# dojo-sim/ContactImplicitMPC.jl

Hardware: AMD Instinct MI355X
Metric: MPC steps/s (quadruped, H=40, fp64) (higher is better)
Workload: dtype f64

## Files before the change

contactimplicitmpc/jl_amd/csrc/cimpc_host.cpp:

```cpp
#include <hip/hip_runtime.h>

#include <algorithm>
#include <chrono>
#include <cmath>
#include <cstdio>
#include <cstdlib>
#include <cstring>
#include <string>
#include <vector>

#include "cimpc_internal.h"
#include "lin_table.h"
#include "newton_state.h"
#include "schedule_plan.h"

using namespace cimpc;

namespace {

thread_local std::string g_create_error;

enum ProfClass { PC_IP = 0, PC_KKT = 1, PC_RESID = 2, PC_OTHER = 3, PC_ASYNC = 4, PC_COUNT = 5 };

struct ProfRec {
// ... 385 lines not shown
    o->r_tol = 3.0e-4;
    o->beta_init = 1.0e-5;
    o->max_time = 0.0;
    o->kappa = 2.0e-4;
    o->max_iter = 5;
    o->kkt_backend = CIMPC_KKT_CONDENSED;
}

const char* cimpc_last_error(cimpc_handle h) { return h ? h->err.c_str() : g_create_error.c_str(); }

int cimpc_create(const cimpc_dims* dims, const cimpc_ip_opts* ip, const cimpc_newton_opts* nt,
                 int device, cimpc_handle* out) {
    if (!dims || !out) return fail(nullptr, CIMPC_ERR_INVALID, "null argument");
    *out = nullptr;
    const cimpc_dims& d = *dims;
    if (d.nq <= 0 || d.nu < 0 || d.nw < 0 || d.nc <= 0 || d.nb < 0 || d.H <= 0 || d.H_ref <= 0 ||
        d.B <= 0 || (d.mode != 0 && d.mode != 1))
        return fail(nullptr, CIMPC_ERR_INVALID, "invalid dimensions");
    int ndev = 0;
    if (hipGetDeviceCount(&ndev) != hipSuccess || ndev <= 0)
        return fail(nullptr, CIMPC_ERR_NO_DEVICE,
                    "no HIP device visible: this library has no CPU fallback");
    if (device < 0 || device >= ndev) return fail(nullptr, CIMPC_ERR_NO_DEVICE, "device index out of range");
    hipDeviceProp_t prop;
    if (hipGetDeviceProperties(&prop, device) != hipSuccess)
        return fail(nullptr, CIMPC_ERR_NO_DEVICE, "hipGetDeviceProperties failed");
    if (std::strncmp(prop.gcnArchName, "gfx950", 6) != 0)
        return fail(nullptr, CIMPC_ERR_NO_DEVICE,
                    std::string("device is ") + prop.gcnArchName + ", kernels are built for gfx950 only");
    if (hipSetDevice(device) != hipSuccess) return fail(nullptr, CIMPC_ERR_NO_DEVICE, "hipSetDevice failed");

    cimpc_ctx* h = new cimpc_ctx();
    h->dm = d;
    if (ip) h->ip = *ip; else cimpc_default_ip_opts(&h->ip);
    if (nt) h->nt = *nt; else cimpc_default_newton_opts(&h->nt);
    h->device = device;
    if (h->ip.max_time > 0.0 && h->ip.max_time < 1000.0) {
        if (h->ip.max_iter >= 128) { delete h; return fail(nullptr, CIMPC_ERR_INVALID, "ip max_time needs max_iter < 128 (the parked state packs both into one word)"); }
        int khz = 0;
        if (hipDeviceGetAttribute(&khz, hipDeviceAttributeWallClockRate, device) != hipSuccess || khz <= 0) {
            delete h;
            return fail(nullptr, CIMPC_ERR_HIP, "ip max_time: the device does not report hipDeviceAttributeWallClockRate");
        }
        h->ip_budget_ticks = std::max<long long>(1, (long long)std::llround(h->ip.max_time * 1.0e3 * (double)khz));
    }
    h->kn.read_environment();
    if (ip_kernel_info(&h->dm, &h->ki) != CIMPC_OK) {
        delete h;
        return fail(nullptr, CIMPC_ERR_INVALID,
                    "model dimensions outside the runtime-dimension kernel (nx, ny <= 64) and without a compiled set (built: pushbot, hopper_2D, hopper_3D, walledcartpole, particle, particle_2D, "
                    "quadruped, flamingo, centroidal_quadruped are built)");
    }
    h->nx = d.nq;
    h->ny = 2 * d.nc + d.nb;
    h->nz = d.nq + 4 * d.nc + 2 * d.nb;
    h->nth = 2 * d.nq + d.nu + d.nw + 2;
    h->nths = 2 * d.nq + d.nu;
    h->nd = d.mode ? d.nq + d.nc + d.nb : d.nq;
    h->nr = d.mode ? d.nq + d.nu + d.nc + d.nb : d.nq + d.nu;
    h->N = d.H * (h->nr + h->nd);
    if (hipStreamCreateWithFlags(&h->stream, hipStreamNonBlocking) != hipSuccess) {
        delete h;
        return fail(nullptr, CIMPC_ERR_HIP, "hipStreamCreate failed");
    }
    h->own_stream = true;
    h->knot_set.assign(d.H_ref, 0);
    h->h_tab.assign(h->ki.tab_size, 0.0);

    const size_t B = d.B, H = d.H;
    int rc = CIMPC_OK;
    {
        const size_t K = d.H_ref;
        const size_t evals = 1 + 7 * (size_t)std::max(1, h->nt.max_iter);
        h->a_cap = B * evals * ((H + K - 1) / K + 1);
        h->a_rq_cap = B * (2 + 3 * (size_t)std::max(1, h->nt.max_iter));
        h->a_kq_cap = B * (2 + 3 * (size_t)std::max(1, h->nt.max_iter));
        const size_t bytes = (K * h->a_cap + h->a_rq_cap + h->a_kq_cap) * sizeof(int);
        h->sched = plan_schedule(h->kn.sched, ScheduleFacts{d.B, d.H, d.H_ref, h->ki.G, newton_async_available(&d) && K <= 256 && bytes <= ((size_t)1 << 30)});
    }
    auto A = [&](auto** p, size_t n) { if (rc == CIMPC_OK) rc = dev_alloc(h, p, n); };
    A(&h->d_tab, (size_t)d.H_ref * h->ki.tab_size);
    {
        const size_t K = d.H_ref;
        const size_t cap = B * CS * ((H + K - 1) / K + 1);
        h->Q.K = (int)K; h->Q.cap = (int)cap; h->Q.par = 0;
        A(&h->Q.items, 2 * K * cap);
        h->ctl_ints = 3 * K * QPAD + 2 * 8 * CPAD;
        A(&h->Q.count, h->ctl_ints);
        if (rc == CIMPC_OK) { h->Q.head = h->Q.count + 2 * K * QPAD; h->d_ring = h->Q.count + 3 * K * QPAD; }
        A(&h->Q.done_count, B * CS);
        A(&h->d_window, B * (H + 2));
        h->Q.window = h->d_window;
    }
    A(&h->d_alt, B * d.nc);
    A(&h->d_zout, B * CS * H * h->nz);
    A(&h->d_Q, H * d.nq * d.nq);
    A(&h->d_R, H * d.nu * d.nu);
    A(&h->d_Qinv, H * d.nq * d.nq);
    A(&h->d_Rinv, H * d.nu * d.nu);
    A(&h->d_Cg, H * d.nc * d.nc);
    A(&h->d_Cb, H * d.nb * d.nb);
    A(&h->d_V, H * d.nq * d.nq);
    A(&h->d_qt, H * d.nq);
    A(&h->d_vt, H * d.nq);
    A(&h->d_q0, 2 * B * d.nq);
    if (rc == CIMPC_OK) h->d_q1 = h->d_q0 + B * d.nq;
    A(&h->d_result, 8 + B * (d.nu + 2));
    if (rc == CIMPC_OK && (hipHostMalloc((void**)&h->h_qin, (2 * B + 1) * d.nq * sizeof(double), hipHostMallocDefault) != hipSuccess ||
                           hipHostMalloc((void**)&h->h_result, (8 + B * (d.nu + 2)) * sizeof(double), hipHostMallocDefault) != hipSuccess))
        rc = CIMPC_ERR_HIP;
    A(&h->d_rhs, B * h->N);
    NewtonDev& S = h->S;
    S.dm = d;
    S.b0 = 0;
    S.nb_launch = d.B;
    S.nd = h->nd; S.nr = h->nr; S.nth = h->nth; S.nths = h->nths; S.N = h->N;
    const size_t BS = B * CS;
    for (TrajDev* T : {&S.traj, &S.cand, &S.ref}) {
        const size_t n = (T == &S.cand) ? BS : B;
        A(&T->q, n * (H + 2) * d.nq); A(&T->u, n * H * d.nu); A(&T->w, n * H * d.nw);
        A(&T->g, n * H * d.nc); A(&T->b, n * H * d.nb); A(&T->th, n * H * h->nth);
    }
    A(&S.nu, B * H * h->nd); A(&S.nu_cand, BS * H * h->nd); A(&S.d, BS * H * h->nd);
    A(&S.dz, BS * H * h->nths * h->nd); A(&S.dz_good, B * H * h->nths * h->nd); A(&h->d_good_src, B * H);
    S.dtn_ld = h->ki.generic ? 0 : h->ki.dtn_ld;
    if (S.dtn_ld > 0) A(&S.dtn, BS * H * (size_t)S.dtn_ld);
    A(&S.ip_status, BS * H); A(&S.ip_iters, BS * H); A(&S.pflag, BS * H); A(&S.cur_slot, B);
    A(&h->d_pstate, BS * H * (2 * (size_t)h->nx + 4 * (size_t)h->ny + 4));
    A(&S.res, B * h->N); A(&S.res_cand, BS * h->N); A(&S.delta, B * h->N);
    A(&S.r_norm, B); A(&S.r_cand, BS); A(&S.alpha, B); A(&S.beta, B);
    A(&S.ls_iter, B); A(&S.newton_l, B); A(&S.stage, B); A(&S.need_sweep, BS);
    A(&S.kkt_list, 2 * B);
    A(&S.slot_list, 2 * BS);
    A(&S.counters, 8 * CPAD);
    A(&S.stats, std::max<size_t>(B * 4, 64));
    A(&S.ro_sweeps, B); A(&S.ro_ip_iters, B); A(&S.ro_ip_fail, B); A(&S.nlog, B * NLOG * 4);
    A(&S.kkt_ws, B * H * (3 * (size_t)h->nd * h->nd + h->nd));
    A(&S.kkt_tw_xch, B * (3 * (size_t)h->nd * h->nd + 4 * h->nd));
    A(&S.kkt_tw_flags, B * 32);
    if (rc == CIMPC_OK && hipHostMalloc((void**)&h->h_counters, 8 * CPAD * sizeof(int)) != hipSuccess)
        rc = fail(h, CIMPC_ERR_HIP, "hipHostMalloc failed");
    if (rc != CIMPC_OK) {
        g_create_error = h->err;
        cimpc_destroy(h);
        return rc;
    }
    S.Q = h->d_Q; S.R = h->d_R; S.Qinv = h->d_Qinv; S.Rinv = h->d_Rinv; S.Cg = h->d_Cg; S.Cb = h->d_Cb;
    if (hipMemset(h->d_good_src, 0xFF, B * H * sizeof(int)) != hipSuccess || hipStreamSynchronize(nullptr) != hipSuccess) {
        g_create_error = "hipMemset failed"; cimpc_destroy(h); return CIMPC_ERR_HIP;
    }
    S.band_form = h->kn.banded_form;
    S.r_tol = h->nt.r_tol; S.beta_init = h->nt.beta_init; S.kappa = h->nt.kappa; S.max_iter = h->nt.max_iter;
    h->kp = h->kn.kkt;
    h->kp.kkt_overlap = h->sched.kkt_overlap;
    set_kkt_backend(h);
    S.spec_all = h->sched.spec_all; S.spec_first = h->sched.spec_first; S.spec_mid = h->sched.spec_mid;
    S.kkt_tw_nb = h->kn.kkt_tw_nb;
    S.kkt_tw_epoch = 0;
    S.kkt_tw_spins = h->kn.kkt_tw_spins > 0 ? h->kn.kkt_tw_spins : (1 << 21);
    {
        int* dv = nullptr;
        if (hipHostMalloc((void**)&h->h_twfail, 4 * sizeof(int), hipHostMallocMapped) != hipSuccess ||
            hipHostGetDevicePointer((void**)&dv, h->h_twfail, 0) != hipSuccess) {
            g_create_error = "mapped counter allocation failed"; cimpc_destroy(h); return CIMPC_ERR_HIP;
        }
        h->h_twfail[0] = 0;
        S.kkt_tw_fail = dv;
    }
    if (hipHostMalloc((void**)&h->h_ring, 32 * sizeof(int), hipHostMallocMapped) != hipSuccess ||
        hipHostGetDevicePointer((void**)&h->h_ring_dev, h->h_ring, 0) != hipSuccess) {
        g_create_error = "ring allocation failed"; cimpc_destroy(h); return CIMPC_ERR_HIP;
    }
    if (h->sched.async_on) {
        const size_t K = d.H_ref;
        if (dev_alloc(h, &h->a_items, K * h->a_cap) != CIMPC_OK || dev_alloc(h, &h->a_jobs, h->a_rq_cap + h->a_kq_cap) != CIMPC_OK ||
            dev_alloc(h, &h->a_ctrl, 2 * K * QPAD + 64 + 33 * 16) != CIMPC_OK || dev_alloc(h, &h->a_evals, B) != CIMPC_OK) {
            g_create_error = h->err; cimpc_destroy(h); return CIMPC_ERR_HIP;
        }
        if (h->kn.async_debug && dev_alloc(h, &h->a_dbg, 16) != CIMPC_OK) { g_create_error = h->err; cimpc_destroy(h); return CIMPC_ERR_HIP; }
        h->async_dirty = true;
    }
    {
        RoundStreams& r = h->rs;
        if (hipStreamCreateWithFlags(&r.st, hipStreamNonBlocking) != hipSuccess ||
            hipStreamCreateWithFlags(&r.st_kkt, hipStreamNonBlocking) != hipSuccess ||
            hipEventCreateWithFlags(&r.ev_join, hipEventDisableTiming) != hipSuccess ||
            hipEventCreateWithFlags(&r.ev_start, hipEventDisableTiming) != hipSuccess) {
            g_create_error = "stream creation failed"; cimpc_destroy(h); return CIMPC_ERR_HIP;
        }
    }
    *out = h;
    return CIMPC_OK;
}

int cimpc_destroy(cimpc_handle h) {
    if (!h) return CIMPC_ERR_INVALID;
    (void)hipSetDevice(h->device);
    if (h->stream) (void)hipStreamSynchronize(h->stream);
    for (auto& r : h->prof_recs) { (void)hipEventDestroy(r.a); (void)hipEventDestroy(r.b); }
    for (auto e : h->ev_pool) (void)hipEventDestroy(e);
    for (void* p : h->allocs) (void)hipFree(p);
    if (h->h_counters) (void)hipHostFree(h->h_counters);
    if (h->h_ring) (void)hipHostFree(h->h_ring);
    if (h->h_qin) (void)hipHostFree(h->h_qin);
    if (h->h_result) (void)hipHostFree(h->h_result);
    if (h->h_stage) (void)hipHostFree(h->h_stage);
    if (h->h_twfail) (void)hipHostFree(h->h_twfail);
    {
        RoundStreams& r = h->rs;
        if (r.st) { (void)hipStreamSynchronize(r.st); (void)hipStreamDestroy(r.st); }
        if (r.st_kkt) { (void)hipStreamSynchronize(r.st_kkt); (void)hipStreamDestroy(r.st_kkt); }
        if (r.ev_join) (void)hipEventDestroy(r.ev_join);
        if (r.ev_start) (void)hipEventDestroy(r.ev_start);
    }
    if (h->own_stream && h->stream) (void)hipStreamDestroy(h->stream);
    delete h;
    return CIMPC_OK;
}

int cimpc_set_stream(cimpc_handle h, void* hip_stream) {
    if (!h) return CIMPC_ERR_INVALID;
    (void)hipStreamSynchronize(h->stream);
    h->advance_pending = false;
// ... 187 lines not shown
static int rekey_out(cimpc_ctx* h) {
    if (h->dz_producer == 0 || !h->window_set) return CIMPC_OK;
    if (!h->d_dz_knot && dev_alloc(h, &h->d_dz_knot, (size_t)h->dm.B * h->dm.H_ref * h->nths * h->nd) != CIMPC_OK) return CIMPC_ERR_HIP;
    int rc = launch_dz_rekey(h->S, h->d_dz_knot, h->d_window, h->dz_producer == 1 ? 0 : 1, 0, h->stream);
    return rc == CIMPC_OK ? CIMPC_OK : fail(h, rc, "sensitivity archive launch failed");
}
static int rekey_in(cimpc_ctx* h) {
    if (h->dz_producer == 0 || !h->d_dz_knot) return CIMPC_OK;
    for (int which = 0; which < 2; ++which) {
        int rc = launch_dz_rekey(h->S, h->d_dz_knot, h->d_window, which, 1, h->stream);
        if (rc != CIMPC_OK) return fail(h, rc, "sensitivity restore launch failed");
    }
    return CIMPC_OK;
}

int cimpc_set_window(cimpc_handle h, const int* window) {
    if (!h || !window) return fail(h, CIMPC_ERR_INVALID, "null argument");
    const cimpc_dims& d = h->dm;
    const int B = d.B, H = d.H, K = d.H_ref;
    std::vector<int> w0((size_t)B * (H + 2));
    for (size_t k = 0; k < w0.size(); ++k) {
        const int t = window[k];
        if (t < 1 || t > K) return fail(h, CIMPC_ERR_INVALID, "window entry out of range (1-based knot index)");
        w0[k] = t - 1;
    }
    HIP_TRY(h, hipSetDevice(h->device));
    if (int dp = drain_pending(h); dp != CIMPC_OK) return dp;
    if (int rk = rekey_out(h); rk != CIMPC_OK) return rk;
    HIP_TRY(h, hipStreamSynchronize(h->stream));
    HIP_TRY(h, hipMemcpy(h->d_window, w0.data(), w0.size() * sizeof(int), hipMemcpyHostToDevice));
    if (int rk = rekey_in(h); rk != CIMPC_OK) return rk;
    HIP_TRY(h, hipStreamSynchronize(h->stream));
    h->window_set = true;
    h->gait_set = false;
    h->win_mirror = w0;
    return CIMPC_OK;
}

int cimpc_set_reference(cimpc_handle h, const double* q_ref, const double* u_ref,
                        const double* w_ref, const double* gamma_ref, const double* b_ref,
                        const double* theta_ref) {
    if (!h || !q_ref || !u_ref || !theta_ref) return fail(h, CIMPC_ERR_INVALID, "q_ref, u_ref, theta_ref are required");
    const cimpc_dims& d = h->dm;
    const size_t B = d.B, H = d.H;
    HIP_TRY(h, hipSetDevice(h->device));
    if (int dp = drain_pending(h); dp != CIMPC_OK) return dp;
    HIP_TRY(h, hipMemcpy(h->S.ref.q, q_ref, B * (H + 2) * d.nq * sizeof(double), hipMemcpyHostToDevice));
    HIP_TRY(h, hipMemcpy(h->S.ref.u, u_ref, B * H * d.nu * sizeof(double), hipMemcpyHostToDevice));
    if (w_ref) HIP_TRY(h, hipMemcpy(h->S.ref.w, w_ref, B * H * d.nw * sizeof(double), hipMemcpyHostToDevice));
    else {
        HIP_TRY(h, hipMemset(h->S.ref.w, 0, B * H * d.nw * sizeof(double)));
        HIP_TRY(h, hipStreamSynchronize(nullptr));
    }
    if (gamma_ref) HIP_TRY(h, hipMemcpy(h->S.ref.g, gamma_ref, B * H * d.nc * sizeof(double), hipMemcpyHostToDevice));
    if (b_ref) HIP_TRY(h, hipMemcpy(h->S.ref.b, b_ref, B * H * d.nb * sizeof(double), hipMemcpyHostToDevice));
    HIP_TRY(h, hipMemcpy(h->S.ref.th, theta_ref, B * H * h->nth * sizeof(double), hipMemcpyHostToDevice));
    h->reference_set = true;
    h->gait_set = false;
    return CIMPC_OK;
}

int cimpc_implicit_dynamics(cimpc_handle h, const double* q, const double* theta,
                            const double* gamma, const double* b, double* d_out, double* dz,
                            int* status, int* iters, double* z) {
    int rc = check_ready(h, false);
    if (rc != CIMPC_OK) return rc;
    if (!q || !theta) return fail(h, CIMPC_ERR_INVALID, "q and theta are required");
    const cimpc_dims& d = h->dm;
    const size_t B = d.B, H = d.H;
    if (d.mode == CIMPC_MODE_CONFIGURATIONFORCE && (!gamma || !b))
        return fail(h, CIMPC_ERR_INVALID, "gamma and b are required in configurationforce mode");
    HIP_TRY(h, hipSetDevice(h->device));
    if (int sy = sync_dz_stores(h, 2); sy != CIMPC_OK) return sy;
    h->dz_producer = 2;
    TrajDev& T = h->S.cand;
    auto up = [&](double* dst, const double* src, size_t row_doubles) {
        return hipMemcpy2DAsync(dst, CS * row_doubles * sizeof(double), src, row_doubles * sizeof(double),
                                row_doubles * sizeof(double), B, hipMemcpyHostToDevice, h->stream);
    };
    HIP_TRY(h, up(T.q, q, (H + 2) * d.nq));
    HIP_TRY(h, up(T.th, theta, H * h->nth));
    if (gamma) HIP_TRY(h, up(T.g, gamma, H * d.nc));
    if (b) HIP_TRY(h, up(T.b, b, H * d.nb));
    HIP_TRY(h, hipMemsetAsync(h->Q.count, 0, 2 * h->Q.K * QPAD * sizeof(int), h->stream));
    HIP_TRY(h, hipMemsetAsync(h->Q.head, 0, h->Q.K * QPAD * sizeof(int), h->stream));
    {
        NewtonDev Sk = h->S;
        Sk.WQ = h->Q; Sk.WQ.par = 0;
        rc = launch_enqueue_all(Sk, h->stream);
        if (rc != CIMPC_OK) return fail(h, rc, "enqueue launch failed");
    }
    for (int pass = 0; pass < 64; ++pass) {
        const int par = pass & 1;
        HIP_TRY(h, hipMemsetAsync(h->S.counters, 0, 8 * CPAD * sizeof(int), h->stream));
        rc = run_sweep(h, par, h->S.counters + 2 * CPAD, z ? h->d_zout : nullptr, h->stream);
        if (rc != CIMPC_OK) return rc;
        HIP_TRY(h, hipMemsetAsync(h->Q.count + (size_t)par * h->Q.K * QPAD, 0, h->Q.K * QPAD * sizeof(int), h->stream));
        HIP_TRY(h, hipMemsetAsync(h->Q.head, 0, h->Q.K * QPAD * sizeof(int), h->stream));
        HIP_TRY(h, hipMemcpyAsync(h->h_counters, h->S.counters + 2 * CPAD, sizeof(int), hipMemcpyDeviceToHost, h->stream));
        HIP_TRY(h, hipStreamSynchronize(h->stream));
        if (h->h_counters[0] == 0) break;
    }
    auto down = [&](void* dst, const void* src, size_t row_bytes) {
        return hipMemcpy2DAsync(dst, row_bytes, src, CS * row_bytes, row_bytes, B, hipMemcpyDeviceToHost, h->stream);
    };
    if (d_out) HIP_TRY(h, down(d_out, h->S.d, H * h->nd * sizeof(double)));
    if (dz) HIP_TRY(h, down(dz, h->S.dz, H * h->nths * h->nd * sizeof(double)));
    if (status) HIP_TRY(h, down(status, h->S.ip_status, H * sizeof(int)));
    if (iters) HIP_TRY(h, down(iters, h->S.ip_iters, H * sizeof(int)));
    if (z) HIP_TRY(h, down(z, h->d_zout, H * h->nz * sizeof(double)));
    HIP_TRY(h, hipStreamSynchronize(h->stream));
    return CIMPC_OK;
}

static int run_ip_callback(cimpc_handle h, int t, int n, int op, const double* z, const double* theta, const double* alt,
                           const double* r, double kappa, double reg, double* out) {
    if (!h || !z || !out || n <= 0) return fail(h, CIMPC_ERR_INVALID, "null argument");
    if (t < 1 || t > h->dm.H_ref) return fail(h, CIMPC_ERR_INVALID, "knot index out of range (1-based)");
    if (!h->knot_set[t - 1]) return fail(h, CIMPC_ERR_STATE, "set_linearization has not been called for this knot");
    if (h->ki.generic) return fail(h, CIMPC_ERR_INVALID, "B2 callbacks exist for the compiled lane-group models only");
    HIP_TRY(h, hipSetDevice(h->device));
    const size_t nz = h->nz, nth = h->nth, nc = h->dm.nc;
    const size_t naux = std::max(nz, nth);
    const size_t tot = (size_t)n * (2 * nz + naux + nc);
    double* buf = nullptr;
    HIP_TRY(h, hipMalloc((void**)&buf, tot * sizeof(double)));
    double* d_z = buf; double* d_out = buf + (size_t)n * nz; double* d_aux = d_out + (size_t)n * nz; double* d_alt = d_aux + (size_t)n * naux;
    auto done = [&](int rc) { (void)hipFree(buf); return rc; };
    if (hipMemcpy(d_z, z, (size_t)n * nz * sizeof(double), hipMemcpyHostToDevice) != hipSuccess) return done(fail(h, CIMPC_ERR_HIP, "upload failed"));
    const double* aux = op == 0 ? theta : r;
    if (!aux) return done(fail(h, CIMPC_ERR_INVALID, "null argument"));
    if (hipMemcpy(d_aux, aux, (size_t)n * (op == 0 ? nth : nz) * sizeof(double), hipMemcpyHostToDevice) != hipSuccess) return done(fail(h, CIMPC_ERR_HIP, "upload failed"));
    if (alt && hipMemcpy(d_alt, alt, (size_t)n * nc * sizeof(double), hipMemcpyHostToDevice) != hipSuccess) return done(fail(h, CIMPC_ERR_HIP, "upload failed"));
    IpCallbackArgs a{};
    a.tab = h->d_tab; a.knot = t - 1; a.n = n; a.op = op; a.z = d_z;
    a.theta = op == 0 ? d_aux : nullptr; a.alt = (op == 0 && alt) ? d_alt : nullptr; a.r = op == 1 ? d_aux : nullptr;
    a.kappa = kappa; a.reg = reg; a.out = d_out;
    (void)hipGetLastError();
    const int rc = launch_ip_callback(&h->dm, a, h->stream);
    if (rc != CIMPC_OK) return done(fail(h, rc, "callback launch failed"));
    if (hipStreamSynchronize(h->stream) != hipSuccess ||
        hipMemcpy(out, d_out, (size_t)n * nz * sizeof(double), hipMemcpyDeviceToHost) != hipSuccess) return done(fail(h, CIMPC_ERR_HIP, "callback kernel failed"));
    return done(CIMPC_OK);
}

int cimpc_ip_residual(cimpc_handle h, int t, int n, const double* z, const double* theta, const double* alt, double kappa, double* r) {
    return run_ip_callback(h, t, n, 0, z, theta, alt, nullptr, kappa, 0.0, r);
}

int cimpc_ip_linear_solve(cimpc_handle h, int t, int n, const double* z, const double* r, double reg, double* delta) {
    return run_ip_callback(h, t, n, 1, z, nullptr, nullptr, r, 0.0, reg, delta);
}

int cimpc_kkt_solve(cimpc_handle h, const double* r, double beta, double* delta) {
    int rc = check_ready(h, true);
    if (rc != CIMPC_OK) return rc;
    if (!r || !delta) return fail(h, CIMPC_ERR_INVALID, "null argument");
    const size_t n = (size_t)h->dm.B * h->N;
    HIP_TRY(h, hipSetDevice(h->device));
    HIP_TRY(h, hipMemcpyAsync(h->d_rhs, r, n * sizeof(double), hipMemcpyHostToDevice, h->stream));
    if ((rc = ensure_kkt_ws(h)) != CIMPC_OK) return rc;
    for (int attempt = 0; attempt < 2; ++attempt) {
        h->S.kkt_tw_epoch += 1;
        const int fails0 = *(volatile int*)h->h_twfail;
        prof_begin(h, PC_KKT);
        rc = run_kkt_stage(h, h->S, kkt_raw_args(h->d_rhs, beta, h->S.delta), KktSite{.kind = KktSite::Seam, .attempt = attempt, .B = h->dm.B},
                           nullptr, h->S.nb_launch, nullptr, h->stream);
        prof_end(h);
        if (rc != CIMPC_OK) return fail(h, rc, "kkt launch failed");
        HIP_TRY(h, hipMemcpyAsync(delta, h->S.delta, n * sizeof(double), hipMemcpyDeviceToHost, h->stream));
        HIP_TRY(h, hipStreamSynchronize(h->stream));
        const int fails1 = *(volatile int*)h->h_twfail;
        if (fails1 == fails0) break;
        h->n_kkt_tw_fallbacks += fails1 - fails0;
        h->twfail_seen = fails1;
    }
    return CIMPC_OK;
}

int cimpc_kkt_solve_rho(cimpc_handle h, const double* r, double rho, double* delta) {
    if (!h) return CIMPC_ERR_INVALID;
    if (!(rho >= 0.0) || !(h->nt.kappa > 0.0)) return fail(h, CIMPC_ERR_INVALID, "rho must be >= 0 (and kappa > 0)");
    const double Hk = (double)h->dm.H, kap = h->nt.kappa;
    auto f = [&](double b) { return Hk * b * kap; };
    double beta = rho / (Hk * kap), err = std::fabs(f(beta) - rho), lo = beta, hi = beta;
    for (int k = 0; k < 4 && err != 0.0; ++k) {
        lo = std::nextafter(lo, -HUGE_VAL); hi = std::nextafter(hi, HUGE_VAL);
        for (double c : {lo, hi}) { const double e = std::fabs(f(c) - rho); if (e < err) { err = e; beta = c; } }
    }
    return cimpc_kkt_solve(h, r, beta, delta);
}

int cimpc_newton_solve_dev(cimpc_handle h, const double* q0_dev, const double* q1_dev, int warm_start) {
    int rc = check_ready(h, true);
    if (rc != CIMPC_OK) return rc;
    if (!q0_dev || !q1_dev) return fail(h, CIMPC_ERR_INVALID, "null argument");
    HIP_TRY(h, hipSetDevice(h->device));
    if (int sy = sync_dz_stores(h, 1); sy != CIMPC_OK) return sy;
    h->dz_producer = 1;
    NewtonDev& S = h->S;
    const int tw_fail0 = *(volatile int*)h->h_twfail;
    h->twfail_seen = tw_fail0;
    const auto t0 = std::chrono::steady_clock::now();
    auto over_budget = [&]() {
        if (h->nt.max_time <= 0.0) return false;
        const double el = std::chrono::duration<double>(std::chrono::steady_clock::now() - t0).count();
        return el >= h->nt.max_time;
    };
    if (!h->external_stream) {
        HIP_TRY(h, hipEventRecord(h->rs.ev_start, h->stream));
        HIP_TRY(h, hipStreamWaitEvent(h->rs.st, h->rs.ev_start, 0));
    }
    HIP_TRY(h, hipMemsetAsync(S.stats, 0, (size_t)h->dm.B * 4 * sizeof(long long), h->external_stream ? h->stream : h->rs.st));
    auto finish_results = [&](hipStream_t st) -> int {
        if (launch_dz_commit(S, st) != CIMPC_OK) return fail(h, CIMPC_ERR_HIP, "sensitivity flush launch failed");
        int rf = launch_solve_finish(S, h->d_result, st);
        if (rf != CIMPC_OK) return fail(h, rf, "result kernel launch failed");
        HIP_TRY(h, hipMemcpyAsync(h->h_result, h->d_result, (8 + (size_t)h->dm.B * (h->dm.nu + 2)) * sizeof(double), hipMemcpyDeviceToHost, st));
        return CIMPC_OK;
    };
    auto run_async = [&](bool from_reset, long long rounds_before, int next_par = -1) -> int {
        IpQueues LQ = h->Q; LQ.par = next_par >= 0 ? next_par : (int)(rounds_before & 1);
        hipStream_t st = h->external_stream ? h->stream : h->rs.st;
        const size_t K = h->Q.K;
        if (h->async_dirty) {
            HIP_TRY(h, hipMemsetAsync(h->a_items, 0xFF, K * h->a_cap * sizeof(int), st));
            HIP_TRY(h, hipMemsetAsync(h->a_jobs, 0xFF, (h->a_rq_cap + h->a_kq_cap) * sizeof(int), st));
            h->async_dirty = false;
        }
        HIP_TRY(h, hipMemsetAsync(h->a_ctrl, 0, (2 * K * QPAD + 64 + 33 * 16) * sizeof(int), st));
        volatile int* hm = (volatile int*)h->h_ring;
        hm[3] = 0;
        NewtonDev Sk = S;
        Sk.b0 = 0; Sk.nb_launch = h->dm.B; Sk.counters = h->d_ring; Sk.counters_next = h->d_ring + 8 * CPAD;
        Sk.host_flag = h->h_ring_dev;
        if (!from_reset) Sk.spec_all = h->sched.spec_tail;
        Sk.WQ = h->Q; Sk.WQ.par = 0;
        Sk.WQ.items = h->a_items; Sk.WQ.cap = (int)h->a_cap;
        Sk.WQ.count = h->a_ctrl; Sk.WQ.head = h->a_ctrl + K * QPAD;
        AsyncQ& A = Sk.A;
        A.on = 1;
        int* c = h->a_ctrl + 2 * K * QPAD;
        A.rq_items = h->a_jobs; A.rq_head = c + 0; A.rq_tail = c + 16;
        A.kq_items = h->a_jobs + h->a_rq_cap; A.kq_head = c + 32; A.kq_tail = c + 48;
        A.n_done = c + 8;
        A.epoch = c + 64;
        A.evals_left = h->a_evals;
        A.abort_flag = (volatile int*)(h->h_ring_dev + 3);
        const int a_grid = from_reset ? h->sched.async_grid : h->sched.tail_grid;
        A.n_service = from_reset ? h->sched.async_service : h->sched.tail_service;
        A.idle_sleep = async_idle_sleep; A.idle_spins = async_idle_spins; A.wake_fan = async_wake_fan;
        A.dbg = h->a_dbg;
        if (h->a_dbg) HIP_TRY(h, hipMemsetAsync(h->a_dbg, 0, 16 * sizeof(long long), st));
        A.B = h->dm.B;
        const KktSite site{.kind = from_reset ? KktSite::Persistent : KktSite::HybridTail, .tw_off = *(volatile int*)h->h_twfail != tw_fail0,
                           .B = h->dm.B, .async_tail = h->sched.async_tail, .waves = std::min(h->sched.waves, 4)};
        A.kkt_tw = plan_kkt_stage(h, site) == KktForm::AsyncTwoJob ? 1 : 0;
        S.kkt_tw_epoch += h->nt.max_iter + 2;
        prof_begin(h, PC_OTHER, st);
        int rc2 = from_reset ? launch_reset(Sk, q0_dev, q1_dev, warm_start, st) : launch_async_handoff(Sk, LQ, st);
        prof_end(h, st);
        if (rc2 != CIMPC_OK) return fail(h, rc2, "reset / hand-off launch failed");
        IpParams p = make_ip_params(h, S.cand, 0, h->d_ring + 2 * CPAD, nullptr);
        if (S.dtn != nullptr) { p.nu = S.nu_cand; p.dtn = S.dtn; }
        p.Q = Sk.WQ;
        p.iter_cap = h->ip.max_iter + 1;
        p.A = A;
        long long solved_before = 0;
        if (h->prof_on && !from_reset) { long long sv[4]; if (int rs = read_stats(h, sv); rs != CIMPC_OK) return rs; solved_before = sv[1]; }
        prof_begin(h, PC_ASYNC, st);
        rc2 = launch_newton_async(&h->dm, p, Sk, std::min(h->sched.waves, 4), a_grid, st);
        prof_end(h, st);
        if (rc2 != CIMPC_OK) return fail(h, rc2, "asynchronous newton launch failed");
        if (int rf = finish_results(st); rf != CIMPC_OK) return rf;
        const double watchdog_s = h->kn.watchdog_s;
        const bool budget = h->nt.max_time > 0.0 && h->nt.max_time < 1.0e6;
        bool timed_out = false;
        const auto tw = std::chrono::steady_clock::now();
        long long polls = 0;
        while (hipStreamQuery(st) == hipErrorNotReady) {
            if (budget && over_budget()) { hm[3] = 1; h->async_dirty = true; break; }
            if ((++polls & 0x3FF) == 0 &&
                std::chrono::duration<double>(std::chrono::steady_clock::now() - tw).count() > watchdog_s) {
                hm[3] = 1; h->async_dirty = true; timed_out = true; break;
            }
        }
        HIP_TRY(h, hipStreamSynchronize(st));
        if (const int twf = *(volatile int*)h->h_twfail; twf != h->twfail_seen) { h->n_kkt_tw_fallbacks += twf - h->twfail_seen; h->twfail_seen = twf; }
        if (timed_out) return fail(h, CIMPC_ERR_HIP, "asynchronous solve: watchdog expired (no completion within CIMPC_ASYNC_WATCHDOG_S)");
        if (h->a_dbg) {
            long long dv[16];
            HIP_TRY(h, hipMemcpy(dv, h->a_dbg, sizeof(dv), hipMemcpyDeviceToHost));
            fprintf(stderr, "[cimpc async] WG-ms: other %.2f kkt %.2f resid %.2f ip %.2f | jobs: kkt %lld resid %lld serve %lld | grid %d service %d | group-trips %.2fM active %.1f%% | group-ms pop %.1f fence %.1f | pop: cas %lld spins %lld claim-ms %.1f wait-ms %.1f\n",
                    dv[0] * 1e-5, dv[1] * 1e-5, dv[2] * 1e-5, dv[3] * 1e-5, dv[9], dv[10], dv[11], h->sched.async_grid, h->sched.async_service, dv[5] * 1e-6, dv[5] ? 100.0 * dv[4] / dv[5] : 0.0, dv[6] * 1e-5, dv[7] * 1e-5, dv[12], dv[13], dv[14] * 1e-5, dv[15] * 1e-5);
        }
        const long long stv[4] = {(long long)h->h_result[0], (long long)h->h_result[1], (long long)h->h_result[2], (long long)h->h_result[3]};
        h->last_stats.sweeps = stv[0];
        h->last_stats.ip_solves = stv[1];
        h->last_stats.ip_iters = stv[2];
        h->last_stats.ip_failures = stv[3];
        h->last_stats.rounds = rounds_before + 1;
        h->last_stats.newton_iters = (long long)h->h_result[4];
        h->prof_ip_problems += solved_before;
        h->prof_async_problems += stv[1] - solved_before;
        if (from_reset) h->prof_kkt_systems += h->last_stats.newton_iters;
        return CIMPC_OK;
    };
    if ((rc = ensure_kkt_ws(h)) != CIMPC_OK) return rc;
    const SolvePath path = choose_solve_path(h->sched, h->kb);
    if (path == SolvePath::Persistent) return run_async(true, 0);
    const bool hybrid = path == SolvePath::Hybrid;
    const int round_limit = max_rounds(h->kn.sched, h->nt.max_iter, h->ip.max_iter);
    RoundStreams sb = h->rs;
    if (h->external_stream) sb.st = h->stream;
    long long launched = 0, completed = 0, rounds = 0;
    const bool dbg_rounds = h->kn.debug_rounds;
    int last_kkt = 0, last_sweep = h->dm.B, last_slots = h->dm.B, last_parked = 0, last_new_slots = h->dm.B;
    const bool ahead = round_ahead(h->sched, h->kb, warm_start != 0, h->nt.max_time > 0.0 && h->nt.max_time < 1.0e6);
    auto launch_round = [&](long long r, bool blind) -> int {
        const int slot = (int)(r & 1), par = (int)(r & 1);
        int* d_cnt = h->d_ring + 8 * CPAD * slot;
        S.kkt_tw_epoch += 1;
        const int tw_fails = *(volatile int*)h->h_twfail;
        if (tw_fails != h->twfail_seen) { h->n_kkt_tw_fallbacks += tw_fails - h->twfail_seen; h->twfail_seen = tw_fails; }
        const bool tw_off = tw_fails != tw_fail0;
        NewtonDev Sk = S;
        Sk.b0 = 0; Sk.nb_launch = h->dm.B; Sk.counters = d_cnt;
        Sk.counters_next = h->d_ring + 8 * CPAD * (slot ^ 1);
        Sk.host_flag = h->h_ring_dev + 8 * slot;
        Sk.A.n_done = hybrid ? h->a_ctrl + 2 * (size_t)h->Q.K * QPAD + 8 : nullptr;
        Sk.round_stamp = (int)(r + 1);
        Sk.WQ = h->Q; Sk.WQ.par = par;
        const bool kkt = (r > 0) && (blind || last_kkt > 0);
        const int n_kkt = blind ? h->dm.B : last_kkt;
        const int* n_kkt_dev = blind ? h->d_ring + 8 * CPAD * (slot ^ 1) + 1 * CPAD : nullptr;
        if (kkt) {
            const bool ov = h->kp.kkt_overlap;
            const KktSite site{.kind = ov ? KktSite::Overlapped : KktSite::Round, .n_kkt = n_kkt, .blind = blind,
                               .sweep_problems = (long long)last_new_slots * h->dm.H, .tw_off = tw_off, .B = h->dm.B};
            hipStream_t kst = ov ? sb.st_kkt : sb.st;
            if (!ov) Sk.kkt_same_round = 1;
            prof_begin(h, PC_KKT, kst);
            int rk = run_kkt_stage(h, Sk, kkt_newton_args(Sk), site, Sk.kkt_list + (size_t)(par ^ 1) * h->dm.B,
                                   ov ? last_kkt : n_kkt, ov ? nullptr : n_kkt_dev, kst);
            prof_end(h, kst);
            if (rk != CIMPC_OK) return fail(h, rk, "kkt launch failed");
            if (ov && hipEventRecord(sb.ev_join, sb.st_kkt) != hipSuccess) return fail(h, CIMPC_ERR_HIP, "join record failed");
        }
        const RoundPlan rp = plan_round(h->kn.sched, h->sched, h->ip.max_iter, kkt, blind, last_sweep, last_slots);
        const long long hint = blind ? -1 : (long long)last_slots * h->dm.H + last_parked;
        if (dbg_rounds && !blind) {
            std::vector<int> qc((size_t)h->Q.K * QPAD);
            (void)hipStreamSynchronize(sb.st); (void)hipStreamSynchronize(sb.st_kkt);
            if (hipMemcpy(qc.data(), h->Q.count + (size_t)par * h->Q.K * QPAD, qc.size() * sizeof(int), hipMemcpyDeviceToHost) == hipSuccess) {
                long long tot = 0;
                for (int k = 0; k < h->Q.K; ++k) tot += qc[(size_t)k * QPAD];
                fprintf(stderr, "[cimpc round %lld] sweep launch: %lld problems queued (host hint %lld)\n", r, tot, hint);
            }
        }
        int rr = run_sweep(h, par, d_cnt + 2 * CPAD, nullptr, sb.st, rp.cap, d_cnt + 3 * CPAD, true, hint);
        if (rr != CIMPC_OK) return rr;
        prof_begin(h, PC_RESID, sb.st);
        if (rp.split_join) {
            rr = launch_resid_decide(Sk, sb.st, rp.n_slots, 1);
            if (rr != CIMPC_OK) return fail(h, rr, "residual launch failed");
        }
        if (kkt && h->kp.kkt_overlap && hipStreamWaitEvent(sb.st, sb.ev_join, 0) != hipSuccess) return fail(h, CIMPC_ERR_HIP, "join failed");
        rr = launch_resid_decide(Sk, sb.st, rp.n_slots, rp.split_join ? 2 : 0);
        prof_end(h, sb.st);
        if (rr != CIMPC_OK) return fail(h, rr, "residual launch failed");
        return CIMPC_OK;
    };
    HIP_TRY(h, hipMemsetAsync(h->Q.count, 0, h->ctl_ints * sizeof(int), sb.st));
    if (hybrid) HIP_TRY(h, hipMemsetAsync(h->a_ctrl + 2 * (size_t)h->Q.K * QPAD, 0, 64 * sizeof(int), sb.st));
    ((volatile int*)h->h_ring)[2] = 0;
    ((volatile int*)h->h_ring)[10] = 0;
    {
        NewtonDev Sk = S;
        Sk.b0 = 0; Sk.nb_launch = h->dm.B; Sk.counters = h->d_ring;
        Sk.WQ = h->Q; Sk.WQ.par = 0;
        prof_begin(h, PC_OTHER, sb.st);
        rc = launch_reset(Sk, q0_dev, q1_dev, warm_start, sb.st);
        prof_end(h, sb.st);
        if (rc != CIMPC_OK) return fail(h, rc, "reset launch failed");
    }
    while (true) {
        if (completed >= round_limit) {
            (void)hipStreamSynchronize(sb.st); (void)hipStreamSynchronize(sb.st_kkt);
            return fail(h, CIMPC_ERR_STATE, "newton_solve: round limit reached with unfinished rollouts");
        }
        while (launched <= completed + (ahead ? 1 : 0)) {
            rc = launch_round(launched, launched > completed);
            if (rc != CIMPC_OK) return rc;
            ++launched;
        }
        {
            volatile int* hm = (volatile int*)h->h_ring + 8 * (completed & 1);
            const int want = (int)(completed + 1);
            long long spins = 0;
            while (hm[2] != want) {
                if ((++spins & 0xFFFFF) == 0 && hipStreamQuery(sb.st) != hipErrorNotReady && hm[2] != want)
                    return fail(h, CIMPC_ERR_HIP, "round finished without publishing its counters");
            }
        }
        volatile int* hr = (volatile int*)h->h_ring + 8 * (completed & 1);
        const int n_sweep = hr[0];
        last_sweep = n_sweep;
        last_kkt = hr[1];
        last_slots = hr[6];
        last_new_slots = hr[7];
        last_parked = hr[4];
        if (dbg_rounds) fprintf(stderr, "[cimpc round %lld] t %.3f ms: next sweep %d rollouts (%d evaluation slots), next kkt %d, parked %d, finished %d\n", completed,
                                1e3 * std::chrono::duration<double>(std::chrono::steady_clock::now() - t0).count(), n_sweep, last_slots, last_kkt, hr[4], hr[5]);
        h->prof_kkt_systems += last_kkt;
        ++completed;
        rounds = completed;
        if ((n_sweep == 0 && last_kkt == 0) || over_budget()) break;
        if (hybrid) {
            if (hand_over(h->sched, h->dm.B - hr[5])) {
                HIP_TRY(h, hipStreamSynchronize(sb.st));
                HIP_TRY(h, hipStreamSynchronize(sb.st_kkt));
                return run_async(false, rounds, (int)(rounds & 1));
            }
        }
    }
    HIP_TRY(h, hipStreamSynchronize(sb.st_kkt));
    if (int rf = finish_results(sb.st); rf != CIMPC_OK) return rf;
    HIP_TRY(h, hipStreamSynchronize(sb.st));
    const long long st[4] = {(long long)h->h_result[0], (long long)h->h_result[1], (long long)h->h_result[2], (long long)h->h_result[3]};
    h->last_stats.sweeps = st[0];
    h->last_stats.ip_solves = st[1];
    h->last_stats.ip_iters = st[2];
    h->last_stats.ip_failures = st[3];
    h->last_stats.rounds = rounds;
    h->last_stats.newton_iters = (long long)h->h_result[4];
    h->prof_ip_problems += st[1];
    return CIMPC_OK;
}

// ... 341 lines not shown
```

contactimplicitmpc/jl_amd/csrc/cimpc_internal.h:

```cpp
#pragma once
#include <hip/hip_runtime.h>
#include <stdint.h>

#include "../../../include/cimpc.h"

namespace cimpc {

constexpr int QPAD = 32;
constexpr int CPAD = 32;

struct IpQueues {
    int* items;
    int* count;
    int* head;
    int* done_count;
    const int* window;
    int cap, K, par;
};

struct AsyncQ {
    int on;
    int* rq_items;
    int* rq_head;
    int* rq_tail;
    int* kq_items;
    int* kq_head;
    int* kq_tail;
    int* evals_left;
    int* n_done;
    int* epoch;
    volatile int* abort_flag;
    long long* dbg;
    int n_service;
    int flags;
    int idle_sleep;
    int idle_spins;
    int wake_fan;
    int B;
    int kkt_tw;
};
constexpr int KJOB_SHIFT = 24, KJOB_MASK = (1 << KJOB_SHIFT) - 1;

__device__ __forceinline__ void xfence(int ) { __threadfence(); }
template <bool X>
__device__ __forceinline__ double xld(const double* p) { return *p; }
template <bool X>
__device__ __forceinline__ void xst(double* p, double v) { *p = v; }
template <bool X>
__device__ __forceinline__ void xst(int* p, int v) { *p = v; }

__device__ __forceinline__ int aload(const int* p) { return __hip_atomic_load(p, __ATOMIC_RELAXED, __HIP_MEMORY_SCOPE_AGENT); }
__device__ __forceinline__ void astore(int* p, int v) { __hip_atomic_store(p, v, __ATOMIC_RELAXED, __HIP_MEMORY_SCOPE_AGENT); }

__device__ __forceinline__ void aq_push(int* items, int* tail, int v) {
    const int pos = atomicAdd(tail, 1);
    astore(items + pos, v);
}
__device__ __forceinline__ int aq_pop(int* items, int* head, const int* tail, long long* dbg = nullptr,
                                      volatile int* abort_flag = nullptr) {
    const long long t0 = dbg ? wall_clock64() : 0;
    int h = aload(head);
    int cas = 0;
    while (true) {
        if (h >= aload(tail)) { if (dbg) { dbg[0] += cas; dbg[2] += wall_clock64() - t0; } return -1; }
        const int old = atomicCAS(head, h, h + 1);
        ++cas;
        if (old == h) break;
        h = old;
    }
    const long long t1 = dbg ? wall_clock64() : 0;
    int v, spins = 0;
    while ((v = aload(items + h)) < 0) {
        __builtin_amdgcn_s_sleep(1);
        if ((++spins & 0xFFFF) == 0 && abort_flag != nullptr && *abort_flag != 0) return -1;
    }
    astore(items + h, -1);
    if (dbg) { dbg[0] += cas; dbg[1] += spins; dbg[2] += t1 - t0; dbg[3] += wall_clock64() - t1; }
    return v;
}

__device__ __forceinline__ void wake_ip(const AsyncQ& A, int b) {
    for (int k = 0; k < A.wake_fan; ++k) atomicAdd(A.epoch + ((b + k * (16 / A.wake_fan)) & 15) * 16, 1);
}
__device__ __forceinline__ void wake_job(const AsyncQ& A, int b) {
    atomicAdd(A.epoch + 32 * 16, 1);
    atomicAdd(A.epoch + (16 + (b & 15)) * 16, 1);
}
__device__ __forceinline__ void push_kkt_job(const AsyncQ& A, int b) {
    if (A.kkt_tw) {
        const int pos = atomicAdd(A.kq_tail, 2);
        astore(A.kq_items + pos, b | (2 << KJOB_SHIFT));
        astore(A.kq_items + pos + 1, b | (1 << KJOB_SHIFT));
        atomicAdd(A.epoch + 32 * 16, 1);
        atomicAdd(A.epoch + (16 + (b & 15)) * 16, 1);
        atomicAdd(A.epoch + (16 + ((b + 1) & 15)) * 16, 1);
    } else {
        aq_push(A.kq_items, A.kq_tail, b);
        wake_job(A, b);
    }
}
__device__ __forceinline__ void wake_all(const AsyncQ& A) { for (int k = 0; k <= 32; ++k) atomicAdd(A.epoch + k * 16, 1); }

__device__ __forceinline__ int* qcount(const IpQueues& Q, int par, int k) { return Q.count + ((size_t)par * Q.K + k) * QPAD; }
__device__ __forceinline__ int* qhead(const IpQueues& Q, int k) { return Q.head + (size_t)k * QPAD; }

struct IpParams {
    const double* tab;
    IpQueues Q;
    int wpk;
    const double* q;
    const double* theta;
    const double* gam;
    const double* bfr;
    const double* alt;
    double* d;
    double* dz;
    const double* nu;
    double* dtn;
    int dtn_ld;
    int* status;
    int* iters;
    double* zout;
    int* pflag;
    double* pstate;
    int* pending_count;
    int iter_cap;
    int* drain_count;
    int drain_thresh, drain_min;
    int slots;
    int H;
    cimpc_ip_opts o;
    double kc_floor;
    double tau_floor;
    double reg_floor;
    long long budget_ticks;
    int generic_static;
    int direct;
    AsyncQ A;
};

struct IpCallbackArgs {
    const double* tab;
    int knot, n, op;
    const double* z;
    const double* theta;
    const double* alt;
    const double* r;
    double kappa, reg;
    double* out;
};

struct KernelInfo {
    int G;
    int lds_table;
    int lds_group;
    int tab_size;
    int dtn_ld;
    int adj;
    int generic;
};

struct LdsOptIn { size_t set[16] = {0}; };
inline int lds_opt_in(LdsOptIn& cache, const void* kernel, size_t lds) {
    if (lds <= 64 * 1024) return CIMPC_OK;
    int dev = 0;
    if (hipGetDevice(&dev) != hipSuccess) return CIMPC_ERR_HIP;
    dev &= 15;
    if (lds <= cache.set[dev]) return CIMPC_OK;
    if (hipFuncSetAttribute(kernel, hipFuncAttributeMaxDynamicSharedMemorySize, (int)lds) != hipSuccess) return CIMPC_ERR_HIP;
    cache.set[dev] = lds;
    return CIMPC_OK;
}
template <class Kern, class... Args>
int launch_lds(LdsOptIn& cache, Kern kernel, dim3 grid, dim3 block, size_t lds, hipStream_t s, Args... args) {
    if (lds_opt_in(cache, (const void*)kernel, lds) != CIMPC_OK) return CIMPC_ERR_HIP;
    hipLaunchKernelGGL(kernel, grid, block, lds, s, args...);
    return hipGetLastError() == hipSuccess ? CIMPC_OK : CIMPC_ERR_HIP;
}

int ip_kernel_info(const cimpc_dims* dm, KernelInfo* info);
int launch_ip_sweep(const cimpc_dims* dm, const IpParams& p, int waves, hipStream_t s);
int launch_ip_callback(const cimpc_dims* dm, const IpCallbackArgs& a, hipStream_t s);
bool ip_generic_available(const cimpc_dims* dm);
void ip_generic_info(const cimpc_dims* dm, KernelInfo* info);
int launch_ip_generic(const cimpc_dims* dm, const IpParams& p, hipStream_t s);

}
// ... 1 lines not shown
```

contactimplicitmpc/jl_amd/csrc/ip_generic.hip:

```cpp
#include <algorithm>
#include <cstdio>

#include "cimpc_internal.h"
#include "lin_table.h"
#include "newton_state.h"

namespace cimpc {

namespace {

constexpr int GW = 64;

__device__ __forceinline__ void wfence() {
    __builtin_amdgcn_fence(__ATOMIC_ACQ_REL, "wavefront");
    __builtin_amdgcn_wave_barrier();
}
__device__ __forceinline__ double uniform(double v) {
    const unsigned lo = (unsigned)__builtin_amdgcn_readfirstlane(__double2loint(v));
    const unsigned hi = (unsigned)__builtin_amdgcn_readfirstlane(__double2hiint(v));
    return __hiloint2double((int)hi, (int)lo);
}
__device__ __forceinline__ double wmax(double v) {
#pragma unroll
    for (int m = 32; m >= 1; m >>= 1) v = fmax(v, __shfl_xor(v, m, 64));
// ... 95 lines not shown
            wfence();
            if (l == k) { t = c / Rm[k * ld + k]; buf[0] = t; }
            wfence();
            const double xk = buf[0];
            if (vy && l < k) c = fma(-Rm[l * ld + k], xk, c);
        }
        return t;
    }

    __device__ double schur_solve(double u, double v, double& xs) {
        const double bq = matvec(L.oCAi, nx, vx ? u : 0.0);
        const double t = qr_solve(vy ? bq - v : 0.0);
        const double w = matvec(L.oDy1, ny, vy ? t : 0.0);
        const double ww = vx ? u + w : 0.0;
        xs = matvec(L.oAi, nx, ww);
        return t;
    }
    __device__ void linear_solve() {
        const double u = rdyn;
        const double v = vy ? (rrst - ry2 * rbil / y1r) : 0.0;
        const double t = schur_solve(u, v, Dx_);
        Dy1_ = vy ? -t : 0.0;
        Dy2_ = vy ? ((rbil - y2r * Dy1_) / y1r) : 0.0;
    }
    __device__ double step_length(double tau) const {
        double a = 1.0;
        if (vy && Dy1_ > 0.0) a = fmin(a, tau * y1 / Dy1_);
        if (vy && Dy2_ > 0.0) a = fmin(a, tau * y2 / Dy2_);
        return wmin(a);
    }
    __device__ bool iterate(const cimpc_ip_opts& o, double& reg, double& r_vio, double& k_vio) {
        reg = (k_vio < o.kappa_reg) ? k_vio * o.gamma_reg : 0.0;
        factorize(reg);
        linear_solve();
        const double a_aff = step_length(1.0);
        const double mu = wsum(vy ? y1 * y2 : 0.0) / (double)ny;
        const double mu_aff = wsum(vy ? (y1 - a_aff * Dy1_) * (y2 - a_aff * Dy2_) : 0.0) / (double)ny;
        double sg = fmin(fmax(mu_aff / mu, 0.0), 1.0);
        sg = sg * sg * sg;
        const double kc = fmax(sg * mu, o.kappa_tol / o.undercut);
        rbil = vy ? ((y1 * y2 - kc) + Dy1_ * Dy2_) : 0.0;
        linear_solve();
        const double vm = fmax(r_vio, k_vio);
        const double tau = fmax(1.0 - o.eps_min, 1.0 - vm * vm);
        const double alpha = step_length(tau);
        if (alpha < o.stall_alpha) return true;
        x -= alpha * Dx_;
        y1 = vy ? (y1 - alpha * Dy1_) : 1.0;
        y2 = vy ? (y2 - alpha * Dy2_) : 1.0;
        double k_c = 0.0, r_c = 0.0, back = alpha;
        for (int s = 1; s <= o.max_ls; ++s) {
            residual(0.0);
            k_c = k_violation();
            r_c = r_violation();
            if (r_c <= r_vio || k_c <= k_vio) break;
            back *= o.ls_scale;
            x += back * Dx_;
            y1 = vy ? (y1 + back * Dy1_) : 1.0;
            y2 = vy ? (y2 + back * Dy2_) : 1.0;
        }
        k_vio = k_c;
        r_vio = r_c;
        return false;
    }
};

struct GenDims { int nq, nu, nw, nc, nb, mode; };

}

__global__ __launch_bounds__(64) void ip_generic_kernel(IpParams p, GenDims gd) {
    extern __shared__ __attribute__((aligned(16))) double sm[];
    const int l = (int)threadIdx.x;
    const int nx = gd.nq, ny = 2 * gd.nc + gd.nb, nth = 2 * gd.nq + gd.nu + gd.nw + 2, nths = 2 * gd.nq + gd.nu;
    const int nz = gd.nq + 4 * gd.nc + 2 * gd.nb, nd = gd.mode ? gd.nq + gd.nc + gd.nb : gd.nq;
    Gen S(nx, ny, nth);
    S.nx = nx; S.ny = ny; S.nth = nth; S.nths = nths; S.nd = nd; S.nc = gd.nc; S.nb = gd.nb; S.nq = gd.nq; S.mode = gd.mode;
    S.ld = ny | 1;
    S.Qm = sm; S.Rm = sm + ny * S.ld; S.buf = S.Rm + ny * S.ld;
    double* dth = S.buf + GW;
    S.l = l; S.vx = l < nx; S.vy = l < ny;
    const LinLayout& L = S.L;
    const cimpc_ip_opts o = p.o;
    const int K = p.Q.K, par = p.Q.par, cap = p.Q.cap;
    const int PS = 2 * nx + 4 * ny + 4;
    for (int kk = 0; kk < K; ++kk) {
        const int knot = ((int)blockIdx.x + kk) % K;
        const int n = *qcount(p.Q, par, knot);
        if (n == 0) continue;
        const int* items = p.Q.items + ((size_t)par * K + knot) * cap;
        S.tab = p.tab + (size_t)knot * L.size;
        const double* tVec = S.tab + L.oVec;
        S.ry2 = tVec[LinLayout::V_RY2 * GW + l]; S.ry1d = tVec[LinLayout::V_RY1D * GW + l]; S.caibd = tVec[LinLayout::V_CAIBD * GW + l];
        S.rdyn0 = tVec[LinLayout::V_RDYN0 * GW + l]; S.rrst0 = tVec[LinLayout::V_RRST0 * GW + l];
        S.x0 = tVec[LinLayout::V_X0 * GW + l]; S.y10 = tVec[LinLayout::V_Y10 * GW + l]; S.y20 = tVec[LinLayout::V_Y20 * GW + l];
        int* head = qhead(p.Q, knot);
        const int G0 = (int)gridDim.x;
        int idx = p.generic_static ? (int)blockIdx.x : __builtin_amdgcn_readfirstlane(atomicAdd(head, l == 0 ? 1 : 0));
        for (; idx < n; idx = p.generic_static ? idx + G0 : __builtin_amdgcn_readfirstlane(atomicAdd(head, l == 0 ? 1 : 0))) {
            const int prob = items[idx];
            const int sb = prob / p.H, i = prob - sb * p.H;
            const size_t pi = (size_t)prob;
            wfence();
            for (int k = l; k < nth; k += GW) dth[k] = p.theta[pi * nth + k] - S.tab[L.oTh0 + k];
            wfence();
            {
                double a = 0.0, c = 0.0;
                for (int k = 0; k < nth; ++k) { const double dv = dth[k]; a = fma(S.T(L.oRthDyn, k), dv, a); c = fma(S.T(L.oRthRst, k), dv, c); }
                S.tthdyn = a; S.tthrst = c;
            }
            S.altl = (p.alt != nullptr && l < gd.nc) ? p.alt[(size_t)(sb / p.slots) * gd.nc + l] : 0.0;
            const double qinit = S.vx ? p.q[((size_t)sb * (p.H + 2) + (i + 2)) * gd.nq + l] : 0.0;
            S.x = qinit; S.y1 = 1.0; S.y2 = 1.0;
            S.residual(0.0);
            double r_vio = S.r_violation(), k_vio = S.k_violation(), reg = 0.0;
            int iters = 0;
            bool stalled = false;
            const long long t_solve0 = p.budget_ticks > 0 ? (long long)wall_clock64() : 0;
            while (!stalled && !(r_vio < o.r_tol && k_vio < o.kappa_tol) && iters < o.max_iter &&
                   !(p.budget_ticks > 0 && (long long)wall_clock64() - t_solve0 >= p.budget_ticks)) {
                ++iters;
                stalled = S.iterate(o, reg, r_vio, k_vio);
            }
            const int code = (!stalled && r_vio < o.r_tol && k_vio < o.kappa_tol) ? 1 : 0;
            if (l == 0) { p.status[pi] = code; p.iters[pi] = iters; p.pflag[pi] = 0; }
            if (S.vx) p.d[pi * nd + l] = S.x - qinit;
            if (gd.mode == CIMPC_MODE_CONFIGURATIONFORCE) {
                if (l < gd.nc) p.d[pi * nd + nx + l] = S.y1 - p.gam[pi * gd.nc + l];
                else if (l < gd.nc + gd.nb) p.d[pi * nd + nx + l] = S.y1 - p.bfr[pi * gd.nb + (l - gd.nc)];
            }
            if (p.zout != nullptr) {
                double* zo = p.zout + pi * nz;
                if (S.vx) zo[l] = S.x;
                if (S.vy) { zo[nx + l] = S.y1; zo[nx + ny + l] = S.y2; }
            }
            if (l == 0) {
                double* ps = p.pstate + pi * PS;
                ps[PS - 2] = reg;
            }
            if (code == 1) {
                S.factorize(fmax(reg, o.kappa_tol * o.gamma_reg));
                double* dzo = p.dz + pi * (size_t)(nths * nd);
                for (int c = 0; c < nths; ++c) {
                    const double u = S.vx ? S.T(L.oRthDyn, c) : 0.0;
                    const double v = S.vy ? S.T(L.oRthRst, c) : 0.0;
                    double xs;
                    const double t = S.schur_solve(u, v, xs);
                    if (S.vx) dzo[c * nd + l] = -xs;
                    if (gd.mode == CIMPC_MODE_CONFIGURATIONFORCE && l < gd.nc + gd.nb) dzo[c * nd + nx + l] = t;
                }
            }
            if (l == 0) atomicAdd(&p.Q.done_count[sb], 1);
        }
    }
}

bool ip_generic_available(const cimpc_dims* dm) {
    const int nx = dm->nq, ny = 2 * dm->nc + dm->nb;
    return nx >= 1 && ny >= 1 && nx <= GW && ny <= GW;
}
void ip_generic_info(const cimpc_dims* dm, KernelInfo* info) {
    const LinLayout L(dm->nq, 2 * dm->nc + dm->nb, 2 * dm->nq + dm->nu + dm->nw + 2, GW);
    info->G = GW;
    info->lds_table = 0;
    info->lds_group = 0;
    info->tab_size = L.size;
}
int launch_ip_generic(const cimpc_dims* dm, const IpParams& p, hipStream_t s) {
    if (!ip_generic_available(dm)) return CIMPC_ERR_INVALID;
    const int ny = 2 * dm->nc + dm->nb, nth = 2 * dm->nq + dm->nu + dm->nw + 2, ld = ny | 1;
    const size_t lds = (size_t)(2 * ny * ld + GW + nth + 8) * sizeof(double);
    static LdsOptIn optin;
    if (lds_opt_in(optin, (const void*)ip_generic_kernel, lds) != CIMPC_OK) return CIMPC_ERR_HIP;
    const int per_cu = (int)std::max<size_t>(1, std::min<size_t>(8, (160 * 1024) / std::max<size_t>(lds, 1)));
    const long long nprob = (long long)dm->B * CS * dm->H;
    const int grid = (int)std::max<long long>(1, std::min<long long>(nprob, 256ll * per_cu));
    const GenDims gd{dm->nq, dm->nu, dm->nw, dm->nc, dm->nb, dm->mode};
    hipLaunchKernelGGL(ip_generic_kernel, dim3(grid), dim3(64), lds, s, p, gd);
    return hipGetLastError() == hipSuccess ? CIMPC_OK : CIMPC_ERR_HIP;
}

}
```

contactimplicitmpc/jl_amd/csrc/ip_kernel_impl.h:

```cpp
#pragma once
#include "cimpc_internal.h"
#include "lane_group.h"
#include "lin_table.h"

#define CIMPC_SWEEP_PRIO 0

namespace cimpc {

#ifdef CIMPC_SWEEP_PROF
static __device__ unsigned long long g_sweep_prof[16];
#define SPROF_T() ((long long)__builtin_amdgcn_s_memtime())
#else
#define SPROF_T() 0ll
#endif

template <int NQ_, int NU_, int NW_, int NC_, int NB_, int MODE_, int WIDE_ = 0>
struct Model {
    static constexpr int NQ = NQ_, NU = NU_, NW = NW_, NC = NC_, NB = NB_, MODE = MODE_;
    static constexpr bool WIDE = WIDE_ != 0;
    using Wide = Model<NQ_, NU_, NW_, NC_, NB_, MODE_, 1>;
    static constexpr int NX = NQ, NY = 2 * NC + NB, NZ = NQ + 4 * NC + 2 * NB;
    static constexpr int NTH = 2 * NQ + NU + NW + 2, NTHS = 2 * NQ + NU;
    static constexpr int ND = MODE ? NQ + NC + NB : NQ;
    static constexpr int G = (NX <= 16 && NY <= 16) ? 16 : (NX <= 32 && NY <= 32) ? 32 : 64;
// ... 663 lines not shown
                        constexpr int j = decltype(jc)::value;
                        const double g0 = g[j * G + (l & 15)], g1 = g[j * G + 16 + ((l & 15) < NY - 16 ? (l & 15) : 0)];
                        Dpp16::chain2<16, 0, 8>(a[j], g0, [&](auto kc) { return A2[decltype(kc)::value]; });
                        Dpp16::chain2<NY - 16, 0, 8>(a[j], g1, [&](auto kc) { return A2[16 + decltype(kc)::value]; });
                    });
                } else
                static_for<0, NY>([&](auto kc) {
                    constexpr int k = decltype(kc)::value;
                    static_for<0, N>([&](auto jc) { constexpr int j = decltype(jc)::value; a[j][k & 1] = fma(A2[k], g[j * G + k], a[j][k & 1]); });
                });
                static_for<0, N>([&](auto jc) {
                    constexpr int j = decltype(jc)::value;
                    const double mx = -(a[j][0] + a[j][1]);
                    if (vx) xst<ASYNC>(dzo + (c0 + cc + j) * ND + lg, mx);
                    if (want && vx) scr[(cc + j) * ND + l] = mx;
                });
            };
            int cc = 0;
#pragma unroll 1
            for (; cc + CB <= n; cc += CB) columns(std::integral_constant<int, CB>{}, cc);
#pragma unroll 1
            for (; cc < n; ++cc) columns(std::integral_constant<int, 1>{}, cc);
            if (want) {
                wave_lds_fence();
                const double* col = scr + (l < n ? l : 0) * ND;
                double s_ = 0.0;
                static_for<0, NX>([&](auto kc) { constexpr int k = decltype(kc)::value; s_ = fma(col[k], LG::template bcast<k>(nux), s_); });
                if (l < n) xst<ASYNC>(p.dtn + pi * (size_t)M::DTN_LD + c0 + lg, s_);
                wave_lds_fence();
            }
        }
        problem_done<ASYNC>(p, prob / p.H, l, part == 0);
        return;
    }
    constexpr int ILP2 = ILP > 2 ? ILP - 1 : 1;
    const bool narrow = nparts > 1 && (hi - lo) % ILP != 0;
#pragma unroll 1
    for (int c0 = lo; c0 < hi; c0 += CH) {
        const int n = hi - c0 < CH ? hi - c0 : CH;
        int cc = 0;
        if (!narrow) {
#pragma unroll 1
            for (; cc + ILP <= n; cc += ILP) {
                if constexpr (G != 16) column_n(c0 + cc, cc);
                else static_for<0, ILP>([&](auto jc) { column(c0 + cc + decltype(jc)::value, cc + decltype(jc)::value); });
            }
        }
        if constexpr (ILP2 > 1) {
#pragma unroll 1
            for (; cc + ILP2 <= n; cc += ILP2) {
                static_for<0, ILP2>([&](auto jc) { column(c0 + cc + decltype(jc)::value, cc + decltype(jc)::value); });
            }
        }
        if constexpr (ILP2 > 2) {
            if (cc + ILP2 - 1 <= n) {
                static_for<0, ILP2 - 1>([&](auto jc) { column(c0 + cc + decltype(jc)::value, cc + decltype(jc)::value); });
                cc += ILP2 - 1;
            }
        }
        for (; cc < n; ++cc) column(c0 + cc, cc);
        if (want) {
            wave_lds_fence();
            const double* col = scr + (l < n ? l : 0) * ND;
            double s_ = 0.0;
            static_for<0, NX>([&](auto kc) { constexpr int k = decltype(kc)::value; s_ = fma(col[k], LG::template bcast<k>(nux), s_); });
            if constexpr (M::MODE == CIMPC_MODE_CONFIGURATIONFORCE)
                static_for<0, NC + NB>([&](auto kc) { constexpr int k = decltype(kc)::value; s_ = fma(col[NX + k], LG::template bcast<k>(nuy), s_); });
            if (l < n) xst<ASYNC>(p.dtn + pi * (size_t)M::DTN_LD + c0 + lg, s_);
            wave_lds_fence();
        }
    }
    problem_done<ASYNC>(p, prob / p.H, l, part == 0);
}

#define CIMPC_PICK_MAXK 256
constexpr int PICK_MAXK = CIMPC_PICK_MAXK;
__device__ __forceinline__ int pick_knot(const IpParams& p, int* s_rem, int* s_total, int* s_knot, int tid, int wg, int nwg) {
    const int K = p.Q.K, par = p.Q.par;
    if (tid == 0) *s_total = 0;
    __syncthreads();
    {
        int part = 0;
        for (int k = tid; k < K; k += (int)blockDim.x) {
            int rem = aload(qcount(p.Q, par, k)) - aload(qhead(p.Q, k));
            rem = rem > 0 ? rem : 0;
            if (k < PICK_MAXK) s_rem[k] = rem;
            part += rem;
        }
        if (part > 0) atomicAdd(s_total, part);
    }
    __syncthreads();
    if (tid == 0) {
        const int total = *s_total;
        int pick = -1;
        if (total > 0) {
            const long long target = ((long long)wg * total) / (long long)nwg;
            long long acc = 0;
            for (int k = 0; k < K; ++k) {
                const int rem = k < PICK_MAXK ? s_rem[k] : max(0, aload(qcount(p.Q, par, k)) - aload(qhead(p.Q, k)));
                if (rem > 0) { pick = k; acc += rem; if (acc > target) break; }
            }
        }
        *s_knot = pick;
    }
    __syncthreads();
    return *s_knot;
}

template <class M, bool ASYNC>
__device__ __forceinline__ void serve_knot(const IpParams& p, double* smem, int knot, int tid, [[maybe_unused]] long long* sp = nullptr) {
    constexpr int NX = M::NX, NY = M::NY, NTH = M::NTH, ND = M::ND, G = M::G;
    constexpr int NC = M::NC, NB = M::NB;
    constexpr LinLayout L(NX, NY, NTH, G, M::NTHS, M::ADJ);
    constexpr int PS = 2 * NX + 4 * NY + 4;
    double* tab = smem;
    const int K = p.Q.K, cap = p.Q.cap, par = p.Q.par;
    const int grp = tid / G;
    const int l = tid % G;
    double* Rst = smem + L.hot + (size_t)grp * M::LDS_GROUP;
    double* dth = Rst;
    constexpr int GPW = 64 / G;
    static_assert(M::SENS_MAX >= 2 * GPW, "the wave's list holds a trip's worth of problems plus one trip of new arrivals");
    const int gw = (tid & 63) / G;
    int* backlog = reinterpret_cast<int*>(smem + L.hot + (size_t)(grp - gw) * M::LDS_GROUP + M::TILE);
    int nback = 0;
    const bool vx = l < NX, vy = l < NY;
    const cimpc_ip_opts o = p.o;
    long long* tbase = reinterpret_cast<long long*>(smem + L.hot + (size_t)grp * M::LDS_GROUP + M::TILE + M::SENS_MAX / 2);
    const bool timed = p.budget_ticks > 0;

    [[maybe_unused]] const long long sp_t0 = SPROF_T();
    const int n = ASYNC ? 1 : *qcount(p.Q, par, knot);
    stage_table<M>(tab, p.tab, knot, tid);
    __syncthreads();
#ifdef CIMPC_SWEEP_PROF
    if (sp) sp[2] += SPROF_T() - sp_t0;
#endif
    const int* items = p.Q.items + ((size_t)par * K + knot) * cap;
    int* head = qhead(p.Q, knot);
    [[maybe_unused]] const int* tailp = qcount(p.Q, par, knot);
    IpSolver<M> S;
    const double* ctab = (L.hot == L.size) ? tab : p.tab + (size_t)knot * L.size;
    S.bind(tab, Rst, l, ctab);
    bool have = false, exhausted = false, stalled = false;
    int prob = 0, iters = 0, done_here = 0;
    [[maybe_unused]] int idle_trips = 0, dbg_trips = 0, dbg_act = 0;
    [[maybe_unused]] long long dbg_tpop = 0, dbg_tfence = 0;
    [[maybe_unused]] long long dbg_pop[4] = {0, 0, 0, 0};
    [[maybe_unused]] const bool dbg_on = ASYNC && p.A.dbg != nullptr;
    double reg = 0.0, r_vio = 0.0, k_vio = 0.0, qinit = 0.0;
    [[maybe_unused]] int drain_raw = 0;

    while (true) {
        [[maybe_unused]] const long long sp_a = SPROF_T();
        [[maybe_unused]] bool draining = false;
        int lg = l;
        asm volatile("" : "+v"(lg));
        if constexpr (!ASYNC) {
            if (p.drain_count != nullptr) {
                draining = __builtin_amdgcn_readfirstlane(drain_raw) >= p.drain_thresh;
                drain_raw = aload(p.drain_count);
            }
        }
        bool push = false;
        long long t_used = 0;
        if (timed) t_used = (long long)wall_clock64() - *tbase;
        if (have) {
            int code = -1;
            if (stalled) code = 0;
            else if (r_vio < o.r_tol && k_vio < o.kappa_tol) code = 1;
            else if (iters >= o.max_iter || (timed && t_used >= p.budget_ticks)) code = 0;
            else if (done_here >= p.iter_cap || (!ASYNC && draining && done_here >= p.drain_min)) code = 2;
            if (code >= 0) {
                const size_t pi = (size_t)prob;
                const int sb = prob / p.H;
                double* ps = p.pstate + pi * PS;
                if (code == 2) {
                    if (vx) { ps[lg] = S.x; ps[NX + 2 * NY + lg] = S.rdyn; }
                    if (vy) { ps[NX + lg] = S.y1; ps[NX + NY + lg] = S.y2; ps[2 * NX + 2 * NY + lg] = S.rrst; ps[2 * NX + 3 * NY + lg] = S.rbil; }
                    if (l == 0) {
                        ps[PS - 4] = r_vio; ps[PS - 3] = k_vio; ps[PS - 2] = reg; ps[PS - 1] = (double)((long long)iters + (timed ? t_used * 128 : 0));
                        p.pflag[pi] = 1;
                        const int pos = atomicAdd(qcount(p.Q, par ^ 1, knot), 1);
                        p.Q.items[((size_t)(par ^ 1) * K + knot) * cap + pos] = prob;
                        atomicAdd(p.pending_count, 1);
                    }
                } else {
                    if (l == 0) { xst<ASYNC>(p.status + pi, code); xst<ASYNC>(p.iters + pi, iters); }
                    if (vx) xst<ASYNC>(p.d + pi * ND + lg, S.x - qinit);
                    if constexpr (M::MODE == CIMPC_MODE_CONFIGURATIONFORCE) {
                        if (l < NC) xst<ASYNC>(p.d + pi * ND + NX + lg, S.y1 - xld<ASYNC>(p.gam + pi * NC + lg));
                        else if (l < NC + NB) xst<ASYNC>(p.d + pi * ND + NX + lg, S.y1 - xld<ASYNC>(p.bfr + pi * NB + (lg - NC)));
                    }
                    if (p.zout != nullptr) {
                        double* zo = p.zout + pi * M::NZ;
                        if (vx) zo[lg] = S.x;
                        if (vy) { zo[NX + lg] = S.y1; zo[NX + NY + lg] = S.y2; }
                    }
                    if (code == 1) {
                        if (vx) ps[lg] = S.x;
                        if (vy) { ps[NX + lg] = S.y1; ps[NX + NY + lg] = S.y2; }
                        if (l == 0) ps[PS - 2] = reg;
                        push = true;
                    } else {
                        {
                            const long long t0 = dbg_on ? wall_clock64() : 0;
                            problem_done<ASYNC>(p, sb, l);
                            if (dbg_on) dbg_tfence += wall_clock64() - t0;
                        }
                    }
                }
                have = false;
            }
        }
        {
            const unsigned long long pm = __ballot((push && l == 0) ? 1 : 0);
            if (pm != 0ull) {
                if (push && l == 0) backlog[nback + __popcll(pm & ((1ull << (tid & 63)) - 1ull))] = prob;
                nback += __popcll(pm);
            }
        }
        [[maybe_unused]] const long long sp_b = SPROF_T();
        if (!have && (!exhausted || (ASYNC && (++idle_trips & 7) == 0))) {
            int idx = 0, item = 0;
            if constexpr (ASYNC) {
                const long long tq0 = dbg_on ? wall_clock64() : 0;
                if (l == 0) item = aq_pop(const_cast<int*>(items), head, tailp, p.A.dbg ? dbg_pop : nullptr, p.A.abort_flag);
                item = group_bcast0<G>(item);
                idx = item < 0 ? n : 0;
                const long long tq1 = dbg_on ? wall_clock64() : 0;
                if (item >= 0) xfence(p.A.flags);
                if (dbg_on) { dbg_tpop += tq1 - tq0; dbg_tfence += wall_clock64() - tq1; }
            } else {
                if (l == 0) idx = atomicAdd(head, 1);
                idx = group_bcast0<G>(idx);
            }
            if (idx < n) {
                prob = ASYNC ? item : items[idx];
                const int sb = prob / p.H, i = prob - sb * p.H;
                const size_t pi = (size_t)prob;
                const double* th = p.theta + pi * NTH;
                constexpr int NTC = (NTH + G - 1) / G;
                double thv[NTC];
                static_for<0, NTC>([&](auto jc) {
                    constexpr int j = decltype(jc)::value;
                    const int k = lg + j * G;
                    thv[j] = xld<ASYNC>(th + (k < NTH ? k : 0));
                });
                const double alt_in = (p.alt != nullptr && l < NC) ? p.alt[(size_t)(sb / p.slots) * NC + lg] : 0.0;
                const double* qrow = p.q + ((size_t)sb * (p.H + 2) + (i + 2)) * M::NQ;
                const double q_in = vx ? xld<ASYNC>(qrow + lg) : 0.0;
                const int parked_in = p.pflag[pi];
                static_for<0, NTC>([&](auto jc) {
                    constexpr int j = decltype(jc)::value;
                    const int k = l + j * G;
                    if (k < NTH) dth[k] = thv[j] - ctab[L.oTh0 + k];
                });
                wave_lds_fence();
                {
                    double a0 = 0.0, a1 = 0.0, c0 = 0.0, c1 = 0.0;
                    if constexpr (G == 16) {
                        constexpr int CHK = 8;
                        static_for<0, (NTH + CHK - 1) / CHK>([&](auto cc) {
                            constexpr int k0 = decltype(cc)::value * CHK, n = NTH - k0 < CHK ? NTH - k0 : CHK;
                            double dv[n], od[n], orr[n];
                            static_for<0, n>([&](auto jc) {
                                constexpr int j = decltype(jc)::value;
                                dv[j] = dth[k0 + j]; od[j] = ctab[L.oRthDyn + (k0 + j) * G + l]; orr[j] = ctab[L.oRthRst + (k0 + j) * G + l];
                            });
                            pin_values(dv); pin_values(od); pin_values(orr);
                            static_for<0, n>([&](auto jc) {
                                constexpr int j = decltype(jc)::value;
                                if constexpr (((k0 + j) & 1) == 0) { a0 = fma(od[j], dv[j], a0); c0 = fma(orr[j], dv[j], c0); }
                                else { a1 = fma(od[j], dv[j], a1); c1 = fma(orr[j], dv[j], c1); }
                            });
                        });
                    } else {
                        int k = 0;
                        for (; k + 1 < NTH; k += 2) {
                            const double d0 = dth[k], d1 = dth[k + 1];
                            a0 = fma(ctab[L.oRthDyn + k * G + l], d0, a0);
                            c0 = fma(ctab[L.oRthRst + k * G + l], d0, c0);
                            a1 = fma(ctab[L.oRthDyn + (k + 1) * G + l], d1, a1);
                            c1 = fma(ctab[L.oRthRst + (k + 1) * G + l], d1, c1);
                        }
                        for (; k < NTH; ++k) {
                            const double d0 = dth[k];
                            a0 = fma(ctab[L.oRthDyn + k * G + l], d0, a0);
                            c0 = fma(ctab[L.oRthRst + k * G + l], d0, c0);
                        }
                    }
                    S.tthdyn = a0 + a1;
                    S.tthrst = c0 + c1;
                }
                S.altl = alt_in;
                qinit = q_in;
                const double* ps = p.pstate + pi * PS;
                if (parked_in == 1) {
                    S.x = vx ? ps[lg] : 0.0;
                    S.y1 = vy ? ps[NX + lg] : 1.0;
                    S.y2 = vy ? ps[NX + NY + lg] : 1.0;
                    S.rdyn = vx ? ps[NX + 2 * NY + lg] : 0.0;
                    S.rrst = vy ? ps[2 * NX + 2 * NY + lg] : 0.0;
                    S.rbil = vy ? ps[2 * NX + 3 * NY + lg] : 0.0;
                    r_vio = ps[PS - 4]; k_vio = ps[PS - 3]; reg = ps[PS - 2];
                    const long long it_word = (long long)ps[PS - 1];
                    iters = timed ? (int)(it_word & 127) : (int)it_word;
                    if (timed && l == 0) *tbase = (long long)wall_clock64() - (it_word >> 7);
                    wave_lds_fence();
                    if (l == 0) p.pflag[pi] = 0;
                } else {
                    S.x = qinit; S.y1 = 1.0; S.y2 = 1.0;
                    S.residual(0.0);
                    r_vio = S.r_violation();
                    k_vio = S.k_violation();
                    iters = 0;
                    reg = 0.0;
                    if (timed && l == 0) *tbase = (long long)wall_clock64();
                }
                if (timed) wave_lds_fence();
                done_here = 0;
                stalled = false;
                have = true;
#ifdef CIMPC_SWEEP_PROF
                if (sp) sp[8] += 1;
#endif
            } else {
                exhausted = true;
            }
        }
        [[maybe_unused]] const long long sp_c = SPROF_T();
#ifdef CIMPC_SWEEP_PROF
        if (sp) { sp[3] += sp_b - sp_a; sp[4] += sp_c - sp_b; }
#endif
        if (dbg_on) { dbg_trips += 1; dbg_act += have ? 1 : 0; }
        const bool any_ip = __any(have ? 1 : 0);
        if (!any_ip && nback == 0) break;
        const bool sens_trip = !any_ip || nback >= GPW || (ASYNC && nback > 0 && __any(have ? 0 : 1));
        if (!sens_trip) {
            if (have && !(r_vio < o.r_tol && k_vio < o.kappa_tol) && iters < o.max_iter && done_here < p.iter_cap) {
                ++done_here;
                ++iters;
                stalled = S.iterate(o, p.kc_floor, p.tau_floor, reg, r_vio, k_vio);
            }
        } else {
            int take, part = 0, nparts = 1;
            if (nback >= GPW) { take = nback - 1 - gw; nback -= GPW; }
            else {
                if (nback == 1) { take = 0; part = gw; nparts = GPW; }
                else if (GPW == 4 && nback == 2) { take = gw >> 1; part = gw & 1; nparts = 2; }
                else take = gw < nback ? gw : -1;
                nback = 0;
            }
            wave_lds_fence();
            if (take >= 0) {
                const double sx = S.x, sy1 = S.y1, sy2 = S.y2, sd = S.rdyn, sr = S.rrst, sb_ = S.rbil, st = S.tthdyn, su = S.tthrst, sa = S.altl;
                const int pr = backlog[take];
                sensitivities<M, ASYNC>(p, S, tab, pr, l, part, nparts);
                S.x = sx; S.y1 = sy1; S.y2 = sy2; S.rdyn = sd; S.rrst = sr; S.rbil = sb_; S.tthdyn = st; S.tthrst = su; S.altl = sa;
            }
        }
#ifdef CIMPC_SWEEP_PROF
        if (sp) { const long long sp_d = SPROF_T(); if (sens_trip) { sp[6] += sp_d - sp_c; sp[10] += 1; } else { sp[5] += sp_d - sp_c; sp[9] += 1; } }
#endif
    }
    if constexpr (ASYNC) {
        if (p.A.dbg != nullptr && l == 0) {
            atomicAdd((unsigned long long*)p.A.dbg + 4, (unsigned long long)dbg_act);
            atomicAdd((unsigned long long*)p.A.dbg + 5, (unsigned long long)dbg_trips);
            atomicAdd((unsigned long long*)p.A.dbg + 6, (unsigned long long)dbg_tpop);
            atomicAdd((unsigned long long*)p.A.dbg + 7, (unsigned long long)dbg_tfence);
            for (int k = 0; k < 4; ++k) atomicAdd((unsigned long long*)p.A.dbg + 12 + k, (unsigned long long)dbg_pop[k]);
        }
    }
}

#define CIMPC_SWEEP_OCC 2
#define CIMPC_SWEEP_THREADS 256
template <class M>
__global__ __launch_bounds__(M::G == 16 ? CIMPC_SWEEP_THREADS : (M::WIDE ? 512 : 256), M::G == 16 ? CIMPC_SWEEP_OCC : 1) void ip_queue_kernel(IpParams p) {
    extern __shared__ __attribute__((aligned(16))) double smem[];
    __shared__ int s_knot, s_total, s_rem[PICK_MAXK];
    const int tid = (int)threadIdx.x;
    __builtin_amdgcn_s_setprio(CIMPC_SWEEP_PRIO);
    [[maybe_unused]] long long sp[12] = {0, 0, 0, 0, 0, 0, 0, 0, 0, 0, 0, 0};
    [[maybe_unused]] const long long sp_life = SPROF_T();
    if (p.direct) {
        const int knot = (int)blockIdx.x;
        if (knot < p.Q.K && aload(qcount(p.Q, p.Q.par, knot)) > 0) serve_knot<M, false>(p, smem, knot, tid, sp);
        return;
    }
    while (true) {
        [[maybe_unused]] const long long sp_t = SPROF_T();
        __syncthreads();
        const int knot = pick_knot(p, s_rem, &s_total, &s_knot, tid, (int)blockIdx.x, (int)gridDim.x);
#ifdef CIMPC_SWEEP_PROF
        sp[1] += SPROF_T() - sp_t;
#endif
        if (knot < 0) {
            if (tid == 0 && p.drain_count != nullptr) atomicAdd(p.drain_count, 1);
            break;
        }
        serve_knot<M, false>(p, smem, knot, tid, sp);
    }
#ifdef CIMPC_SWEEP_PROF
    if ((tid & 63) == 0) {
        sp[0] = SPROF_T() - sp_life; sp[7] = 1;
        for (int k = 0; k < 11; ++k) atomicAdd(&g_sweep_prof[k], (unsigned long long)sp[k]);
    }
#endif
}

template <class M>
__global__ __launch_bounds__(64) void ip_callback_kernel(IpCallbackArgs a) {
    constexpr int NX = M::NX, NY = M::NY, NTH = M::NTH, G = M::G;
    constexpr LinLayout L(NX, NY, NTH, G, M::NTHS, M::ADJ);
    extern __shared__ __attribute__((aligned(16))) double smem[];
    const int tid = (int)threadIdx.x, grp = tid / G, l = tid % G;
    double* tab = smem;
    double* Rst = smem + L.size + (size_t)grp * M::LDS_GROUP;
    stage_table<M>(tab, a.tab, a.knot, tid);
    __syncthreads();
    const int prob = (int)blockIdx.x * (64 / G) + grp;
    const bool live = prob < a.n;
    const size_t pi = (size_t)(live ? prob : 0);
    IpSolver<M> S;
    S.bind(tab, Rst, l);
    const bool vx = S.vx, vy = S.vy;
    const double* z = a.z + pi * M::NZ;
    S.x = vx ? z[l] : 0.0;
    S.y1 = vy ? z[NX + l] : 1.0;
    S.y2 = vy ? z[NX + NY + l] : 1.0;
    double* out = a.out + pi * M::NZ;
    if (a.op == 0) {
        const double* th = a.theta + pi * NTH;
        double td[2] = {0.0, 0.0}, tr[2] = {0.0, 0.0};
        for (int k = 0; k < NTH; ++k) {
            const double dk = th[k] - tab[L.oTh0 + k];
            td[k & 1] = fma(tab[L.oRthDyn + k * G + l], dk, td[k & 1]);
            tr[k & 1] = fma(tab[L.oRthRst + k * G + l], dk, tr[k & 1]);
        }
        S.tthdyn = td[0] + td[1]; S.tthrst = tr[0] + tr[1];
        S.altl = (a.alt != nullptr && l < M::NC) ? a.alt[pi * M::NC + l] : 0.0;
        S.residual(a.kappa);
        if (live && vx) out[l] = S.rdyn;
        if (live && vy) { out[NX + l] = S.rrst; out[NX + NY + l] = S.rbil; }
    } else {
        const double* r = a.r + pi * M::NZ;
        S.rdyn = vx ? r[l] : 0.0;
        S.rrst = vy ? r[NX + l] : 0.0;
        S.rbil = vy ? r[NX + NY + l] : 0.0;
        S.factorize(a.reg);
        S.linear_solve();
        if (live && vx) out[l] = S.Dx_;
        if (live && vy) { out[NX + l] = S.Dy1_; out[NX + NY + l] = S.Dy2_; }
    }
}

template <class M>
int launch_callback(const IpCallbackArgs& a, hipStream_t s) {
    constexpr LinLayout L(M::NX, M::NY, M::NTH, M::G, M::NTHS, M::ADJ);
    const int ppw = 64 / M::G;
    const size_t lds = (size_t)(L.size + ppw * M::LDS_GROUP) * sizeof(double);
    static LdsOptIn optin;
    if (lds_opt_in(optin, (const void*)ip_callback_kernel<M>, lds) != CIMPC_OK) return CIMPC_ERR_HIP;
    hipLaunchKernelGGL((ip_callback_kernel<M>), dim3((a.n + ppw - 1) / ppw), dim3(64), lds, s, a);
    return hipGetLastError() == hipSuccess ? CIMPC_OK : CIMPC_ERR_HIP;
}

template <class M>
int launch_model(const IpParams& p, int waves, hipStream_t s) {
    constexpr LinLayout L(M::NX, M::NY, M::NTH, M::G, M::NTHS, M::ADJ);
    if (waves < 1 || waves > (M::G == 16 ? CIMPC_SWEEP_THREADS : 512) / 64 || waves == 3) return CIMPC_ERR_INVALID;
    const int ppw = 64 / M::G;
    const size_t lds = (size_t)(L.hot + waves * ppw * M::LDS_GROUP) * sizeof(double);
    const int grid = p.wpk;
    if constexpr (M::G == 64) { if (waves > 4) return CIMPC_ERR_INVALID; }
    if constexpr (M::G == 32) {
        if (waves > 4) {
            using MW = typename M::Wide;
            constexpr LinLayout LW(MW::NX, MW::NY, MW::NTH, MW::G, MW::NTHS, MW::ADJ);
            const size_t lds_w = (size_t)(LW.size + waves * ppw * MW::LDS_GROUP) * sizeof(double);
            static LdsOptIn optin_w;
            if (lds_opt_in(optin_w, (const void*)ip_queue_kernel<MW>, lds_w) != CIMPC_OK) return CIMPC_ERR_HIP;
            hipLaunchKernelGGL((ip_queue_kernel<MW>), dim3(grid), dim3(64 * waves), lds_w, s, p);
            return hipGetLastError() == hipSuccess ? CIMPC_OK : CIMPC_ERR_HIP;
// ... 93 lines not shown
```

contactimplicitmpc/jl_amd/csrc/newton_async_impl.h:

```cpp
#pragma once
#include <algorithm>
#include <cstddef>
#include <map>
#include "ip_kernel_impl.h"
#ifdef CIMPC_KKT_PROF
#undef CIMPC_KKT_PROF
#endif
#include "newton_impl.h"

namespace cimpc {

struct AsyncArgs {
    IpParams p;
    NewtonDev S;
};

template <class T, size_t OFFSET>
__device__ __forceinline__ T uniform_arg(unsigned long long v) {
    T out;
#if defined(__HIP_DEVICE_COMPILE__)
    const unsigned lo = __builtin_amdgcn_readfirstlane((unsigned)v);
    const unsigned hi = __builtin_amdgcn_readfirstlane((unsigned)(v >> 32));
    const unsigned long long u = (((unsigned long long)hi << 32) | lo) + OFFSET;
    __builtin_memcpy(&out, (const __attribute__((address_space(4))) T*)u, sizeof(T));
#else
    (void)v;
#endif
    return out;
}
__device__ __forceinline__ NewtonDev uniform_state(unsigned long long v) { return uniform_arg<NewtonDev, offsetof(AsyncArgs, S)>(v); }
template <int NQ, int NU>
__device__ __noinline__ void async_kkt_job(unsigned long long ka, int b, double* smem, int tid) {
    const NewtonDev S = uniform_state(ka);
    if ((int)blockDim.x >= 192) {
        if (tid < 192) {
            const KktArgs K{S.res, S.delta, S.beta, 0.0, S.stage, 0};
            kkt_body<NQ, NU, WaveSync, 3>(S, K, b, smem, tid & 63, tid >> 6);
        } else {
            for (int k = 0; k < S.dm.H + 4; ++k) __syncthreads();
        }
        __threadfence_block();
        __syncthreads();
        start_line_search<BlockSync>(S, b, 2, tid, (int)blockDim.x);
    } else if ((int)blockDim.x >= 128) {
        const KktArgs K{S.res, S.delta, S.beta, 0.0, S.stage, 2};
        kkt_body<NQ, NU, WaveSync, 2>(S, K, b, smem, tid & 63, tid >> 6);
    } else if (tid < 64) {
        const KktArgs K{S.res, S.delta, S.beta, 0.0, S.stage, 2};
        kkt_body<NQ, NU, WaveSync>(S, K, b, smem, tid);
    }
}
template <int NQ, int NU, int TW>
__device__ __noinline__ void async_kkt_tw_job(unsigned long long ka, int b, double* smem, int tid) {
    NewtonDev S = uniform_state(ka);
    S.kkt_tw_epoch += 1 + __builtin_amdgcn_readfirstlane(S.newton_l[b]);
    constexpr int TL = kkt_tld<NQ, NU>();
    const int H = S.dm.H;
    const int msp = kkt_tw_split(H, S.kkt_tw_nb, TL > 16, false);
    const int NS = TW == 1 ? msp + 2 : (H - msp - 2) + 2;
    if (tid < 192) {
        const KktArgs K{S.res, S.delta, S.beta, 0.0, S.stage, 0};
        kkt_body<NQ, NU, WaveSync, 3, false, TW>(S, K, b, smem, tid & 63, tid >> 6);
    } else {
        for (int k = 0; k < NS + 8; ++k) __syncthreads();
    }
    __syncthreads();
    const int last = (int)smem[KKT_TW_TILES * TL * TL + 11 * (TL <= 16 ? 16 : 32)];
    if (last == 0) return;
    __threadfence();
    int* xfl = S.kkt_tw_flags + (size_t)b * KKT_TW_FLAGS;
    if (__builtin_amdgcn_readfirstlane(aload(xfl + 3)) == S.kkt_tw_epoch) {
        if (tid == 0) { aq_push(S.A.kq_items, S.A.kq_tail, b | (3 << KJOB_SHIFT)); wake_job(S.A, b); }
        return;
    }
    start_line_search<BlockSync>(S, b, 2, tid, (int)blockDim.x);
}
template <int NQ, int NU>
__device__ __noinline__ void async_resid_job(unsigned long long ka, int b, double* red, double* rc, int* sh) {
    const NewtonDev S = uniform_state(ka);
    resid_decide_body<NQ, NU, false, true>(S, b, red, rc, sh);
}

template <class M>
__device__ __noinline__ void async_serve_job(unsigned long long ka, double* smem, int knot, int tid) {
    const IpParams p = uniform_arg<IpParams, offsetof(AsyncArgs, p)>(ka);
    serve_knot<M, true>(p, smem, knot, tid);
}

template <class M>
__global__ __launch_bounds__(256, (M::G == 16 ? 2 : 1)) void newton_async_kernel(AsyncArgs args) {
    const IpParams& p = args.p;
    const unsigned long long ka = (unsigned long long)__builtin_amdgcn_kernarg_segment_ptr();
    static_assert(M::MODE == CIMPC_MODE_CONFIGURATION, "the KKT stage implements :configuration");
    constexpr int NQ = M::NQ, NU = M::NU;
    extern __shared__ __attribute__((aligned(16))) double smem[];
    __shared__ int s_knot, s_total, s_rem[PICK_MAXK], s_job[2], s_epoch[2];
    __shared__ double rc[CS];
    __shared__ int sh[4];
    const int tid = (int)threadIdx.x;
    const AsyncQ& A = p.A;
    const bool service = (int)blockIdx.x < A.n_service;
    const int nwork = max(1, (int)gridDim.x - A.n_service), wg = max(0, (int)blockIdx.x - A.n_service);
    unsigned trip = 0;
    long long tk = wall_clock64();
    auto account = [&](int slot) {
        if (tid == 0 && A.dbg != nullptr) {
            const long long tn = wall_clock64();
            atomicAdd((unsigned long long*)A.dbg + slot, (unsigned long long)(tn - tk));
            atomicAdd((unsigned long long*)A.dbg + 8 + slot, 1ull);
            tk = tn;
        }
    };
    while (true) {
        __syncthreads();
        if (tid == 0) {
            int type = 0, job = -1;
            s_epoch[0] = aload(A.epoch + ((int)blockIdx.x & 15) * 16);
            s_epoch[1] = aload(A.epoch + (service ? 32 : 16 + ((int)blockIdx.x & 15)) * 16);
            if ((trip++ & 31u) == 31u && *A.abort_flag != 0) {
                type = 3;
            } else if ((job = aq_pop(A.kq_items, A.kq_head, A.kq_tail, nullptr, A.abort_flag)) >= 0) {
                type = 1;
            } else if ((job = aq_pop(A.rq_items, A.rq_head, A.rq_tail, nullptr, A.abort_flag)) >= 0) {
                type = 2;
            }
            s_job[0] = type; s_job[1] = job;
        }
        __syncthreads();
        const int type = s_job[0], job = s_job[1];
        if (type == 3) break;
        if (type == 1) {
            xfence(A.flags);
            account(0);
            const int kind = job >> KJOB_SHIFT, jb = job & KJOB_MASK;
            if constexpr (kkt_tld<NQ, NU>() == 16) {
                if ((kind == 1 || kind == 2) && (int)blockDim.x >= 256) {
                    if (kind == 2) async_kkt_tw_job<NQ, NU, 2>(ka, jb, smem, tid);
                    else async_kkt_tw_job<NQ, NU, 1>(ka, jb, smem, tid);
                    __syncthreads();
                    account(1);
                    continue;
                }
            }
            async_kkt_job<NQ, NU>(ka, jb, smem, tid);
            __syncthreads();
            account(1);
            continue;
        }
        if (type == 2) {
            xfence(A.flags);
            account(0);
            async_resid_job<NQ, NU>(ka, job, smem, rc, sh);
            __syncthreads();
            account(2);
            continue;
        }
        if (!service) {
            const int knot = pick_knot(p, s_rem, &s_total, &s_knot, tid, wg, nwork);
            if (knot >= 0) {
                account(0);
                async_serve_job<M>(ka, smem, knot, tid);
                __syncthreads();
                account(3);
                continue;
            }
        }
        if (tid == 0) {
            int leave = aload(A.n_done) >= A.B;
            const int* wi = A.epoch + ((int)blockIdx.x & 15) * 16;
// ... 53 lines not shown
```

contactimplicitmpc/jl_amd/csrc/newton_impl.h:

```cpp
#pragma once
#include "lane_group.h"
#include "newton_state.h"

namespace cimpc {

struct BlockSync { static __device__ __forceinline__ void sync() { __syncthreads(); } };
struct WaveSync {
    static __device__ __forceinline__ void sync() {
        __builtin_amdgcn_fence(__ATOMIC_SEQ_CST, "workgroup");
        __builtin_amdgcn_wave_barrier();
    }
};

__device__ __forceinline__ void theta_update(const NewtonDev& S, const TrajDev& T, int b, int i,
                                             int tid, int nthreads) {
    const cimpc_dims& m = S.dm;
    double* th = T.th + ((size_t)b * m.H + i) * S.nth;
    const double* q = T.q + ((size_t)b * (m.H + 2) + i) * m.nq;
    const double* u = T.u + ((size_t)b * m.H + i) * m.nu;
    const double* w = T.w + ((size_t)b * m.H + i) * m.nw;
    for (int k = tid; k < 2 * m.nq; k += nthreads) th[k] = q[k];
    for (int k = tid; k < m.nu; k += nthreads) th[2 * m.nq + k] = u[k];
    for (int k = tid; k < m.nw; k += nthreads) th[2 * m.nq + m.nu + k] = w[k];
}

__device__ __forceinline__ void copy_n(double* dst, const double* src, int n, int tid, int nt) {
    for (int k = tid; k < n; k += nt) dst[k] = src[k];
}

__device__ __forceinline__ double ls_alpha(int iter) { return ldexp(1.0, -iter); }

__device__ __forceinline__ void list_slot(const NewtonDev& S, size_t sb, int par, int pos = -1) {
    if (S.slot_list == nullptr) return;
    if (pos < 0) pos = atomicAdd(&S.counters[4 * CPAD], 1);
    if (pos >= S.dm.B * CS) __builtin_trap();
    S.slot_list[(size_t)par * S.dm.B * CS + pos] = (int)sb;
}

__device__ __forceinline__ void enqueue_eval(const NewtonDev& S, size_t sb, int b, int par, int tid, int nt, int list_pos = -1) {
    const int H = S.dm.H, K = S.WQ.K;
    for (int k = tid; k < H; k += nt) {
        const int t = S.WQ.window[(size_t)b * (H + 2) + k];
        const int pos = atomicAdd(qcount(S.WQ, par, t), 1);
        S.WQ.items[((size_t)par * K + t) * S.WQ.cap + pos] = (int)(sb * H + k);
    }
    if (tid == 0) {
        S.WQ.done_count[sb] = 0;
        S.need_sweep[sb] = 1;
        list_slot(S, sb, par, list_pos);
    }
}

__device__ __forceinline__ void enqueue_evals(const NewtonDev& S, size_t sb, int n, int b, int par, int tid, int nt, int mark = 1) {
    const int H = S.dm.H, K = S.WQ.K;
    for (int k = tid; k < H; k += nt) {
        const int t = S.WQ.window[(size_t)b * (H + 2) + k];
        const int pos = atomicAdd(qcount(S.WQ, par, t), n);
        int* it = S.WQ.items + ((size_t)par * K + t) * S.WQ.cap + pos;
        for (int c = 0; c < n; ++c) it[c] = (int)((sb + c) * H + k);
    }
    if (tid == 0) {
        int pos = 0;
        if (S.slot_list != nullptr) pos = atomicAdd(&S.counters[4 * CPAD], n);
        atomicAdd(&S.counters[5 * CPAD], n);
        if (pos + n > S.dm.B * CS) __builtin_trap();
        for (int c = 0; c < n; ++c) {
            S.WQ.done_count[sb + c] = 0;
            S.need_sweep[sb + c] = mark;
            if (S.slot_list != nullptr) S.slot_list[(size_t)par * S.dm.B * CS + pos + c] = (int)(sb + c);
        }
    }
}

template <class Sync>
__device__ __forceinline__ void enqueue_eval_async(const NewtonDev& S, size_t sb0, int first, int nslots, int b, int tid, int nt) {
    const int H = S.dm.H;
    if (tid == 0) {
        for (int c = 0; c < CS; ++c) {
            const bool on = c >= first && c < first + nslots;
            if (on) S.WQ.done_count[sb0 + c] = 0;
            S.need_sweep[sb0 + c] = on;
        }
        astore(S.A.evals_left + b, nslots);
    }
    xfence(S.A.flags);
    Sync::sync();
    for (int e = tid; e < nslots * H; e += nt) {
        const int c = first + e / H, k = e % H;
        const int t = S.WQ.window[(size_t)b * (H + 2) + k];
        aq_push(S.WQ.items + (size_t)t * S.WQ.cap, qcount(S.WQ, 0, t), (int)((sb0 + c) * H + k));
    }
    Sync::sync();
    if (tid == 0) wake_ip(S.A, b);
}

template <class Sync>
__device__ __forceinline__ void apply_step(const NewtonDev& S, const TrajDev& dst, double* nu_dst_base, size_t di, int b,
                           double alpha, int tid, int nt) {
    const cimpc_dims& m = S.dm;
    const int H = m.H, nq = m.nq, nu = m.nu, nr = S.nr, nd = S.nd;
    const double* D = S.delta + (size_t)b * S.N;
    const bool cf = m.mode == CIMPC_MODE_CONFIGURATIONFORCE;
    const int oq_in_block = cf ? nu + m.nc + m.nb : nu;
    for (int k = tid; k < H * nq; k += nt) {
        const int t = k / nq, c = k - t * nq;
        dst.q[(di * (H + 2) + t + 2) * nq + c] =
            S.traj.q[((size_t)b * (H + 2) + t + 2) * nq + c] - alpha * D[t * nr + oq_in_block + c];
    }
    for (int k = tid; k < 2 * nq; k += nt)
        dst.q[di * (H + 2) * nq + k] = S.traj.q[(size_t)b * (H + 2) * nq + k];
    for (int k = tid; k < H * nu; k += nt) {
        const int t = k / nu, c = k - t * nu;
        dst.u[(di * H + t) * nu + c] = S.traj.u[((size_t)b * H + t) * nu + c] - alpha * D[t * nr + c];
    }
    if (cf) {
        for (int k = tid; k < H * m.nc; k += nt) {
            const int t = k / m.nc, c = k - t * m.nc;
            dst.g[(di * H + t) * m.nc + c] = S.traj.g[((size_t)b * H + t) * m.nc + c] - alpha * D[t * nr + nu + c];
        }
        for (int k = tid; k < H * m.nb; k += nt) {
            const int t = k / m.nb, c = k - t * m.nb;
            dst.b[(di * H + t) * m.nb + c] = S.traj.b[((size_t)b * H + t) * m.nb + c] - alpha * D[t * nr + nu + m.nc + c];
        }
    }
    for (int k = tid; k < H * nd; k += nt)
        nu_dst_base[di * H * nd + k] = S.nu[(size_t)b * H * nd + k] - alpha * D[H * nr + k];
    Sync::sync();
    {
        const int nth = S.nth, nw = m.nw;
        for (int k = tid; k < H * nth; k += nt) {
            const int t = k / nth, c = k - t * nth;
            double v;
            if (c < 2 * nq) v = dst.q[(di * (H + 2) + t) * nq + c];
            else if (c < 2 * nq + nu) v = dst.u[(di * H + t) * nu + (c - 2 * nq)];
            else if (c < 2 * nq + nu + nw) v = S.traj.w[((size_t)b * H + t) * nw + (c - 2 * nq - nu)];
            else v = S.traj.th[((size_t)b * H + t) * nth + c];
            dst.th[(di * H + t) * nth + c] = v;
        }
    }
    Sync::sync();
}

template <int UN>
__device__ __forceinline__ void copy_rows(double* __restrict__ dst, const double* __restrict__ src, int n, int tid, int nt) {
    for (int e0 = tid; e0 < n; e0 += UN * nt) {
        double v[UN];
        static_for<0, UN>([&](auto jc) { constexpr int j = decltype(jc)::value; const int e = e0 + j * nt; v[j] = src[e < n ? e : 0]; });
// ... 18 lines not shown
template <class Sync>
__device__ __forceinline__ void apply_steps(const NewtonDev& S, size_t sb_first, int it_first, int count, int b, int tid, int nt) {
    const cimpc_dims& m = S.dm;
    const int H = m.H, nq = m.nq, nu = m.nu, nw = m.nw, nr = S.nr, nd = S.nd, nth = S.nth;
    const bool cf = m.mode == CIMPC_MODE_CONFIGURATIONFORCE;
    const int oq = cf ? nu + m.nc + m.nb : nu;
    const double* __restrict__ D = S.delta + (size_t)b * S.N;
    const double* __restrict__ tq = S.traj.q + (size_t)b * (H + 2) * nq;
    const double* __restrict__ tu = S.traj.u + (size_t)b * H * nu;
    const double* __restrict__ tw = S.traj.w + (size_t)b * H * nw;
    const double* __restrict__ tth = S.traj.th + (size_t)b * H * nth;
    const double* __restrict__ tnu = S.nu + (size_t)b * H * nd;
    double* __restrict__ cq = S.cand.q + sb_first * (H + 2) * nq;
    double* __restrict__ cu = S.cand.u + sb_first * H * nu;
    double* __restrict__ cth = S.cand.th + sb_first * H * nth;
    double* __restrict__ cnu = S.nu_cand + sb_first * H * nd;
    auto put = [&](double* dst, size_t stride, int k, double base, double dl, bool moves) {
        for (int c = 0; c < count; ++c) dst[(size_t)c * stride + k] = moves ? fma(-ls_alpha(it_first + c), dl, base) : base;
    };
    auto rows = [&](auto unc, int n, auto&& src, auto&& sink) {
        constexpr int UN = decltype(unc)::value;
        for (int e0 = tid; e0 < n; e0 += UN * nt) {
            double base[UN], dl[UN]; bool mv[UN];
            static_for<0, UN>([&](auto jc) { constexpr int j = decltype(jc)::value; const int e = e0 + j * nt; src(e < n ? e : 0, base[j], dl[j], mv[j]); });
            static_for<0, UN>([&](auto jc) { constexpr int j = decltype(jc)::value; const int e = e0 + j * nt; if (e < n) sink(e, base[j], dl[j], mv[j]); });
        }
    };
    const size_t sth = (size_t)H * nth;
    rows(std::integral_constant<int, 3>{}, (H + 2) * nq, [&](int k, double& base, double& dl, bool& mv) {
        const int j = k / nq, c = k - j * nq;
        base = tq[k]; mv = j >= 2; dl = D[mv ? (j - 2) * nr + oq + c : 0];
    }, [&](int k, double base, double dl, bool mv) {
        const int j = k / nq, c = k - j * nq;
        put(cq, (size_t)(H + 2) * nq, k, base, dl, mv);
        if (j < H) put(cth, sth, j * nth + c, base, dl, mv);
        if (j >= 1 && j <= H) put(cth, sth, (j - 1) * nth + nq + c, base, dl, mv);
    });
    rows(std::integral_constant<int, 2>{}, H * nu, [&](int k, double& base, double& dl, bool& mv) {
        const int t = k / nu, c = k - t * nu;
        base = tu[k]; dl = D[t * nr + c]; mv = true;
    }, [&](int k, double base, double dl, bool mv) {
        const int t = k / nu, c = k - t * nu;
        put(cu, (size_t)H * nu, k, base, dl, mv);
        put(cth, sth, t * nth + 2 * nq + c, base, dl, mv);
    });
    if (cf) {
        const double* __restrict__ tg = S.traj.g + (size_t)b * H * m.nc;
        const double* __restrict__ tb = S.traj.b + (size_t)b * H * m.nb;
        for (int k = tid; k < H * m.nc; k += nt) { const int t = k / m.nc, c = k - t * m.nc; put(S.cand.g + sb_first * H * m.nc, (size_t)H * m.nc, k, tg[k], D[t * nr + nu + c], true); }
        for (int k = tid; k < H * m.nb; k += nt) { const int t = k / m.nb, c = k - t * m.nb; put(S.cand.b + sb_first * H * m.nb, (size_t)H * m.nb, k, tb[k], D[t * nr + nu + m.nc + c], true); }
    }
    rows(std::integral_constant<int, 3>{}, H * nd, [&](int k, double& base, double& dl, bool& mv) { base = tnu[k]; dl = D[H * nr + k]; mv = true; },
         [&](int k, double base, double dl, bool mv) { put(cnu, (size_t)H * nd, k, base, dl, mv); });
    const int o_w = 2 * nq + nu, o_c = o_w + nw, n_c = nth - o_c;
    rows(std::integral_constant<int, 1>{}, H * nw, [&](int k, double& base, double& dl, bool& mv) { base = tw[k]; dl = 0.0; mv = false; },
         [&](int k, double base, double dl, bool mv) { const int t = k / nw; put(cth, sth, t * nth + o_w + (k - t * nw), base, dl, mv); });
    if (n_c > 0)
        rows(std::integral_constant<int, 1>{}, H * n_c, [&](int k, double& base, double& dl, bool& mv) { const int t = k / n_c; base = tth[t * nth + o_c + (k - t * n_c)]; dl = 0.0; mv = false; },
             [&](int k, double base, double dl, bool mv) { const int t = k / n_c; put(cth, sth, t * nth + o_c + (k - t * n_c), base, dl, mv); });
    Sync::sync();
}

template <class Sync>
__device__ __forceinline__ void start_line_search(const NewtonDev& S, int b, int mode, int lane, int nt) {
    const size_t sb0 = (size_t)b * CS;
    int n = 1;
    {
        const int prev = S.ls_iter[b];
        if (S.newton_l[b] == 0) n = S.spec_first;
        else if (prev >= S.spec_all) n = 7;
        else if (prev >= S.spec_mid) n = 3;
        n = (n >= 7) ? 7 : (n >= 3) ? 3 : 1;
    }
    Sync::sync();
    apply_steps<Sync>(S, sb0, 0, n, b, lane, nt);
    if (lane == 0) { S.alpha[b] = 1.0; S.ls_iter[b] = 0; S.stage[b] = (n == 7) ? STAGE_LS7 : (n == 3) ? STAGE_LS3 : STAGE_LS0; }
    if (mode == 2) {
        enqueue_eval_async<Sync>(S, sb0, 0, n, b, lane, nt);
    } else {
        const int par = (S.kkt_same_round == 1) ? S.WQ.par : (S.WQ.par ^ 1);
        enqueue_evals(S, sb0, n, b, par, lane, nt, S.kkt_same_round == 0 ? 2 : 1);
        if (lane == 0) {
            for (int c = n; c < CS; ++c) S.need_sweep[sb0 + c] = 0;
            if (S.kkt_same_round == 0) atomicAdd(&S.counters[0 * CPAD], 1);
        }
    }
}


__device__ __forceinline__ const double* dz_eff(const NewtonDev& S, int b, int it, int i) {
    const int H = S.dm.H;
    const size_t sb0 = (size_t)b * CS, blk = (size_t)S.nths * S.nd;
    int s = it;
    while (s >= 0 && S.ip_status[(sb0 + s) * H + i] == 0) --s;
    return s >= 0 ? S.dz + ((sb0 + s) * H + i) * blk : S.dz_good + ((size_t)b * H + i) * blk;
}

template <int NQ, int NU, bool CF>
__device__ double slot_residual(const NewtonDev& S, size_t sb, int b, const int* eff, int tid, int nt, double* absr = nullptr) {
    const cimpc_dims& m = S.dm;
    const int nq = NQ > 0 ? NQ : m.nq, nu = NQ > 0 ? NU : m.nu;
    constexpr bool cf = CF;
    const int H = m.H, nc = m.nc, nb = m.nb, nr = S.nr;
    const int nd = cf ? nq + nc + nb : nq;
    const int oq_in_block = cf ? nu + nc + nb : nu;
    double* r = S.res_cand + sb * S.N;
    const double* nuc = S.nu_cand + sb * H * nd;
    const int it = (int)(sb - (size_t)b * CS);
    const size_t blk = (size_t)(2 * nq + nu) * nd, sb0 = (size_t)b * CS;
    auto dzp = [&](int i) -> const double* {
        if (eff == nullptr) return dz_eff(S, b, it, i);
        const int s_ = eff[i];
        return s_ >= 0 ? S.dz + ((sb0 + s_) * H + i) * blk : S.dz_good + ((size_t)b * H + i) * blk;
    };
    if constexpr (NQ > 0 && !CF) {
        if (absr != nullptr && S.V == nullptr) {
            constexpr int nrc = NQ + NU, JM = NQ > NU ? NQ : NU;
            const double* dtn = S.dtn; const int dld = S.dtn_ld;
            const double* cu = S.cand.u + sb * H * NU; const double* ru = S.ref.u + (size_t)b * H * NU;
            const double* cqp = S.cand.q + sb * (H + 2) * NQ; const double* rqp = S.ref.q + (size_t)b * (H + 2) * NQ;
            const double* dd = S.d + sb * H * NQ;
            for (int j = tid; j < H * JM; j += nt) {
                const bool on_u = j < H * NU;
                const int ju = on_u ? j : 0, iu = ju / NU, cu_ = ju - iu * NU;
                const double* Rm = S.R + (size_t)iu * NU * NU + cu_; const double* uu = cu + iu * NU; const double* ur = ru + iu * NU;
                const bool ownu = dtn != nullptr && eff != nullptr && eff[iu] == it;
                const double* A0 = dzp(iu) + (size_t)(2 * NQ + cu_) * NQ; const double* nv = nuc + iu * NQ;
                const bool on_q = j < H * NQ;
                const int jq = on_q ? j : 0, i = jq / NQ, cq = jq - i * NQ;
                const int i1 = min(i + 1, H - 1), i2 = min(i + 2, H - 1);
                const double* Qm = S.Q + (size_t)i * NQ * NQ + cq; const double* qq = cqp + (i + 2) * NQ; const double* qr = rqp + (i + 2) * NQ;
                const bool own1 = dtn != nullptr && eff != nullptr && eff[i1] == it, own2 = dtn != nullptr && eff != nullptr && eff[i2] == it;
                const double* A1 = dzp(i1) + (size_t)(NQ + cq) * NQ; const double* n1 = nuc + i1 * NQ;
                const double* A2 = dzp(i2) + (size_t)cq * NQ; const double* n2 = nuc + i2 * NQ;
                double rv[NU], du_[NU], qv[NQ], dq_[NQ];
#pragma unroll
                for (int k = 0; k < NU; ++k) { rv[k] = Rm[k * NU]; du_[k] = uu[k] - ur[k]; }
#pragma unroll
                for (int k = 0; k < NQ; ++k) { qv[k] = Qm[k * NQ]; dq_[k] = qq[k] - qr[k]; }
                const double nui = nuc[i * NQ + cq];
                const double dv = dd[jq];
                double su, s1, s2;
                if (dtn != nullptr) {
                    su = dtn[((size_t)sb * H + iu) * dld + 2 * NQ + cu_]; s1 = dtn[((size_t)sb * H + i1) * dld + NQ + cq]; s2 = dtn[((size_t)sb * H + i2) * dld + cq];
                }
                auto dot = [&](const double* A, const double* n_) { double a_ = 0.0;
#pragma unroll
                    for (int k = 0; k < NQ; ++k) a_ = fma(A[k], n_[k], a_);
                    return a_; };
                if (!ownu) su = dot(A0, nv);
                if (!own1) s1 = dot(A1, n1);
                if (!own2) s2 = dot(A2, n2);
                double vu = 0.0, vq = 0.0;
#pragma unroll
                for (int k = 0; k < NU; ++k) vu = fma(rv[k], du_[k], vu);
                vu += su;
#pragma unroll
                for (int k = 0; k < NQ; ++k) vq = fma(qv[k], dq_[k], vq);
                vq -= nui;
                if (i + 1 < H) vq += s1;
                if (i + 2 < H) vq += s2;
                if (on_u) { r[iu * nrc + cu_] = vu; absr[iu * nrc + cu_] = fabs(vu); }
                if (on_q) { r[i * nrc + NU + cq] = vq; absr[i * nrc + NU + cq] = fabs(vq); r[H * nrc + jq] = dv; absr[H * nrc + jq] = fabs(dv); }
            }
            return 0.0;
        }
    }
// ... 32 lines not shown
                    for (int k = 0; k < nq; ++k)
                        v = fma(Vi[cq + k * nq], qq[k] - qq[k - nq] - (cf ? 0.0 : vt[k]), v);
                    if (i + 1 < H) {
                        const double* Vn = Vi + nq * nq;
                        for (int k = 0; k < nq; ++k)
                            v = fma(-Vn[cq + k * nq], qq[k + nq] - qq[k] - (cf ? 0.0 : vt[k + nq]), v);
                    }
                }
                v -= nuc[i * nd + cq];
                if (i + 1 < H) {
                    const double* A1 = dzp(i + 1) + (size_t)(nq + cq) * nd;
                    double s = 0.0;
#pragma unroll
                    for (int k = 0; k < nq; ++k) s = fma(A1[k], nuc[(i + 1) * nd + k], s);
                    for (int k = nq; k < nd; ++k) s = fma(A1[k], nuc[(i + 1) * nd + k], s);
                    v += s;
                }
                if (i + 2 < H) {
                    const double* A2 = dzp(i + 2) + (size_t)cq * nd;
                    double s = 0.0;
#pragma unroll
                    for (int k = 0; k < nq; ++k) s = fma(A2[k], nuc[(i + 2) * nd + k], s);
                    for (int k = nq; k < nd; ++k) s = fma(A2[k], nuc[(i + 2) * nd + k], s);
                    v += s;
                }
            } else if (c < nu + nc) {
                const int cg = c - nu;
                const double* Cm = S.Cg + (size_t)i * nc * nc;
                const double* gg = S.cand.g + (sb * H + i) * nc;
                const double* gr = S.ref.g + ((size_t)b * H + i) * nc;
                for (int k = 0; k < nc; ++k) v = fma(Cm[cg + k * nc], gg[k] - gr[k], v);
                v -= nuc[i * nd + nq + cg];
            } else {
                const int cb = c - nu - nc;
                const double* Cm = S.Cb + (size_t)i * nb * nb;
                const double* bb = S.cand.b + (sb * H + i) * nb;
                const double* br = S.ref.b + ((size_t)b * H + i) * nb;
                for (int k = 0; k < nb; ++k) v = fma(Cm[cb + k * nb], bb[k] - br[k], v);
                v -= nuc[i * nd + nq + nc + cb];
            }
        }
        r[e] = v;
        if (absr != nullptr) absr[e] = fabs(v);
        else part += fabs(v);
    }
    return part;
}

#ifdef CIMPC_RESID_PROF
static __device__ unsigned long long g_resid_prof[4][16];
struct ResidProf {
    long long t0, t, acc[13]; int k;
    __device__ ResidProf(int k_) : k(k_) { t0 = t = wall_clock64(); for (int j = 0; j < 13; ++j) acc[j] = 0; }
    __device__ void mark(int j) { const long long n = wall_clock64(); acc[j] += n - t; t = n; }
    __device__ ~ResidProf() {
        if (threadIdx.x != 0) return;
        const long long te = wall_clock64();
        atomicAdd(&g_resid_prof[k][0], 1ull);
        for (int j = 1; j < 13; ++j) if (acc[j]) atomicAdd(&g_resid_prof[k][j], (unsigned long long)acc[j]);
        atomicAdd(&g_resid_prof[k][13], (unsigned long long)(te - t0));
        atomicMax(&g_resid_prof[k][14], (unsigned long long)(te - t0));
        if (te - t0 > 3000) {
            atomicAdd(&g_resid_prof[2 + k][0], 1ull);
            for (int j = 1; j < 13; ++j) if (acc[j]) atomicAdd(&g_resid_prof[2 + k][j], (unsigned long long)acc[j]);
            atomicAdd(&g_resid_prof[2 + k][13], (unsigned long long)(te - t0));
        }
    }
};
#define RPROF_BEGIN(k) ResidProf rprof_(k);
#define RPROF(j) rprof_.mark(j);
#else
#define RPROF_BEGIN(k)
#define RPROF(j)
#endif
constexpr int SLOT_ABS_MAX = 6144;
template <int NQ, int NU, bool CF, bool ASYNC, int SPLIT = 0>
__device__ __forceinline__ void resid_decide_body(const NewtonDev& S, int b, double* red, double* rc, int* sh) {
    const cimpc_dims& m = S.dm;
    const int tid = threadIdx.x, nt = blockDim.x;
    const int H = m.H;
    const size_t sb0 = (size_t)b * CS;
    if (!ASYNC && blockIdx.x == 0) {
        const int K = S.WQ.K, par = S.WQ.par;
        for (int k = tid; k < K; k += nt) { *qcount(S.WQ, par, k) = 0; *qhead(S.WQ, k) = 0; }
        if (tid < 8) S.counters_next[tid * CPAD] = 0;
    }
    RPROF_BEGIN(1)
    int pre_dc = H, pre_ns = 0;
    double pre_rc = 0.0;
    if constexpr (SPLIT == 2) {
        if (tid < CS) { pre_dc = S.WQ.done_count[sb0 + tid]; pre_ns = S.need_sweep[sb0 + tid]; pre_rc = S.r_cand[sb0 + tid]; }
    }
    const int stage = S.stage[b];
    if (stage == STAGE_DONE || stage == STAGE_KKT) return;
    const int ncand = (stage == STAGE_LS1) ? 2 : (stage == STAGE_LS2) ? 4 : (stage == STAGE_LS7) ? 7 : (stage == STAGE_LS3) ? 3 : 1;
    const int it0 = (stage == STAGE_LS1) ? 1 : (stage == STAGE_LS2) ? 3 : 0;
    if constexpr (SPLIT == 2) {
        const bool mine = tid >= it0 && tid < it0 + ncand;
        if (!__syncthreads_or(tid == it0 && pre_ns != 0)) return;
        if (__syncthreads_or(tid == it0 && pre_ns == 2)) {
            if (mine) S.need_sweep[sb0 + tid] = 1;
            return;
        }
        if (__syncthreads_or(mine && pre_dc < H)) {
            if (tid == 0) atomicAdd(&S.counters[0 * CPAD], 1);
            if (mine) list_slot(S, sb0 + tid, S.WQ.par ^ 1);
            return;
        }
        if (mine) rc[tid - it0] = pre_rc;
    } else {
        if (S.need_sweep[sb0 + it0] == 0) return;
        if constexpr (!ASYNC) {
            if (S.need_sweep[sb0 + it0] == 2) {
                __syncthreads();
                if (tid < ncand) S.need_sweep[sb0 + it0 + tid] = 1;
                return;
            }
        }
        if constexpr (!ASYNC) {
            int pend = 0;
            if (tid < ncand) pend = (S.WQ.done_count[sb0 + it0 + tid] < H);
            if (__syncthreads_or(pend)) {
                if (tid == 0) atomicAdd(&S.counters[0 * CPAD], 1);
                return;
            }
        }
    }
    int& s_act = sh[0]; int& s_slot = sh[1]; int& s_iter = sh[2];
    constexpr int EFF_H = 128;
    __shared__ int eff[(SPLIT ? 1 : CS) * EFF_H];
    const bool use_eff = H <= EFF_H;
    auto resolve_eff = [&](int c, int* row) {
        for (int i = tid; i < H && use_eff; i += nt) {
            int s_ = it0 + c;
            while (s_ >= 0 && S.ip_status[(sb0 + s_) * H + i] == 0) --s_;
            row[i] = s_;
        }
    };
    if constexpr (SPLIT == 2) {
        __syncthreads();
    } else {
        constexpr int CT = 256;
        for (int c = 0; c < ncand; ++c) resolve_eff(c, eff + c * EFF_H);
        __syncthreads();
        double* absr = red + CS * CT;
        for (int c = 0; c < ncand; ++c) {
            slot_residual<NQ, NU, CF>(S, sb0 + it0 + c, b, use_eff ? eff + c * EFF_H : nullptr, tid, nt, absr);
            __syncthreads();
            for (int j = tid; j < CT; j += nt) {
                double part = 0.0;
                for (int e = j; e < S.N; e += CT) part += absr[e];
                red[c * CT + j] = part;
            }
            __syncthreads();
        }
        for (int st = CT / 2; st > 0; st >>= 1) {
            for (int j = tid; j < st; j += nt)
                for (int c = 0; c < ncand; ++c) red[c * CT + j] += red[c * CT + j + st];
            __syncthreads();
        }
        if (tid < ncand) { rc[tid] = red[tid * CT]; S.r_cand[sb0 + it0 + tid] = red[tid * CT]; }
        __syncthreads();
    }
    RPROF(1)
    if (tid == 0) {
        int act = 2, slot = 0, iter = 0;
        if (stage == STAGE_INIT) {
            act = 0;
        } else {
            const double rn2 = S.r_norm[b] * S.r_norm[b];
            for (int c = 0; c < ncand; ++c) {
                const double a = ls_alpha(it0 + c);
                if (!(rc[c] * rc[c] >= (1.0 - 0.001 * a) * rn2)) { act = 1; slot = c; iter = it0 + c; break; }
            }
            if (act == 2 && (stage == STAGE_LS2 || stage == STAGE_LS7)) {
                act = 1; slot = ncand - 1; iter = 7;
            }
        }
        s_act = act; s_slot = slot; s_iter = iter;
    }
    __syncthreads();
    RPROF(2)
    {
        const int nref = (s_act == 1 && s_iter <= 6) ? s_slot + 1 : ncand;
        int its = 0, fails = 0, its_ref = 0, fails_ref = 0;
        for (int k = tid; k < ncand * H; k += nt) {
            const int it = S.ip_iters[(sb0 + it0) * H + k], fl = (S.ip_status[(sb0 + it0) * H + k] == 0);
            its += it; fails += fl;
            if (k < nref * H) { its_ref += it; fails_ref += fl; }
        }
        for (int o = 32; o > 0; o >>= 1) {
            its += __shfl_xor(its, o, 64); fails += __shfl_xor(fails, o, 64);
            its_ref += __shfl_xor(its_ref, o, 64); fails_ref += __shfl_xor(fails_ref, o, 64);
        }
        if ((tid & 63) == 0) {
            double* w = red + 4 * (tid >> 6);
            w[0] = (double)its; w[1] = (double)fails; w[2] = (double)its_ref; w[3] = (double)fails_ref;
        }
        __syncthreads();
        if (tid == 0) {
            long long t_its = 0, t_fails = 0, t_its_ref = 0, t_fails_ref = 0;
            for (int w = 0; w < (nt + 63) / 64; ++w) {
                t_its += (long long)red[4 * w]; t_fails += (long long)red[4 * w + 1];
                t_its_ref += (long long)red[4 * w + 2]; t_fails_ref += (long long)red[4 * w + 3];
            }
            S.ro_sweeps[b] += nref;
            S.ro_ip_iters[b] += (int)t_its_ref;
            S.ro_ip_fail[b] += (int)t_fails_ref;
            long long* st = S.stats + (size_t)b * 4;
            st[0] += ncand; st[1] += (long long)ncand * H; st[2] += (long long)t_its; st[3] += t_fails;
        }
    }
    __syncthreads();
    RPROF(3)
    const int act = s_act, slot = s_slot, iter = s_iter;
    if (act == 2) {
        const int nstage = (stage == STAGE_LS0) ? STAGE_LS1 : STAGE_LS2;
        const int it1 = (nstage == STAGE_LS1) ? 1 : 3, nn = (nstage == STAGE_LS1) ? 2 : 4;
        if constexpr (ASYNC) {
            apply_steps<BlockSync>(S, sb0 + it1, it1, nn, b, tid, nt);
            if (tid == 0) S.stage[b] = nstage;
            enqueue_eval_async<BlockSync>(S, sb0, it1, nn, b, tid, nt);
            return;
        }
        if (tid == 0) for (int c = 0; c < CS; ++c) S.need_sweep[sb0 + c] = 0;
        __syncthreads();
        apply_steps<BlockSync>(S, sb0 + it1, it1, nn, b, tid, nt);
        RPROF(4)
        enqueue_evals(S, sb0 + it1, nn, b, S.WQ.par ^ 1, tid, nt);
        RPROF(5)
        if (tid == 0) {
            S.stage[b] = nstage;
            atomicAdd(&S.counters[0 * CPAD], 1);
        }
        return;
    }
    const double alpha = ls_alpha(iter);
    if (act == 1) {
        if (iter <= 6) accept_candidate<BlockSync>(S, sb0 + it0 + slot, b, tid, nt);
        else apply_step<BlockSync>(S, S.traj, S.nu, (size_t)b, b, alpha, tid, nt);
    }
    RPROF(6)
    {
        double* rr = S.res + (size_t)b * S.N;
        const double* r = S.res_cand + (sb0 + it0 + slot) * S.N;
        for (int e = tid; e < S.N; e += nt) rr[e] = r[e];
    }
    RPROF(7)
    {
        const int blk = S.nths * S.nd, ita = it0 + slot;
        double* good = S.dz_good + (size_t)b * H * blk;
        {
        if constexpr (SPLIT == 2) {
            resolve_eff(slot, eff);
            __syncthreads();
        }
        bool lazy_commit = false;
        if constexpr (!ASYNC) lazy_commit = S.good_src != nullptr && use_eff;
        if (lazy_commit) {
            const int* ef = eff + (SPLIT ? 0 : slot * EFF_H);
            for (int i = tid; i < H; i += nt) S.good_src[(size_t)b * H + i] = ef[i];
        } else if (use_eff && (blk & 1) == 0) {
            const int* ef = eff + (SPLIT ? 0 : slot * EFF_H);
            const int hb = blk / 2;
            constexpr int UN = 13;
            for (int e0 = tid; e0 < H * hb; e0 += UN * nt) {
                typedef double v2d __attribute__((ext_vector_type(2)));
                v2d v[UN]; int dst[UN];
                static_for<0, UN>([&](auto jc) {
                    constexpr int j = decltype(jc)::value;
                    const int e = e0 + j * nt, ec = e < H * hb ? e : 0, i = ec / hb, s_ = ef[i];
                    dst[j] = (e < H * hb && s_ >= 0) ? i * blk + 2 * (ec - i * hb) : -1;
                    v[j] = reinterpret_cast<const v2d*>(S.dz + ((sb0 + (s_ >= 0 ? s_ : 0)) * H + i) * (size_t)blk)[ec - i * hb];
                });
                static_for<0, UN>([&](auto jc) {
                    constexpr int j = decltype(jc)::value;
                    if (dst[j] >= 0) *reinterpret_cast<v2d*>(good + dst[j]) = v[j];
                });
            }
        } else {
            for (int e = tid; e < H * blk; e += nt) {
                const int i = e / blk;
                good[e] = dz_eff(S, b, ita, i)[e - i * blk];
            }
        }
        }
    }
    RPROF(8)
    if (tid == 0) {
        const double rn = rc[slot];
        if (act == 1 && S.nlog != nullptr && S.newton_l[b] < NLOG) {
            double* e = S.nlog + ((size_t)b * NLOG + S.newton_l[b]) * 4;
            e[0] = alpha; e[1] = S.r_norm[b] / (double)S.N; e[2] = rn / (double)S.N; e[3] = (double)iter;
        }
        S.r_norm[b] = rn;
        S.cur_slot[b] = it0 + slot;
        S.alpha[b] = alpha;
        S.ls_iter[b] = iter;
        int l = S.newton_l[b];
        if (act == 1) {
            l += 1;
            S.newton_l[b] = l;
            const double be = S.beta[b];
            S.beta[b] = (iter > 6) ? fmin(be * 1.3, 1.0e2) : fmax(1.0e1, be / 1.3);
        }
        const bool done = (l >= S.max_iter) || (rn / (double)S.N < S.r_tol);
        for (int c = 0; c < CS; ++c) S.need_sweep[sb0 + c] = 0;
        if (done) {
            S.stage[b] = STAGE_DONE;
            if (!ASYNC && S.A.n_done != nullptr) atomicAdd(S.A.n_done, 1);
        } else {
            S.stage[b] = STAGE_KKT;
            if constexpr (!ASYNC) {
                const int pos = atomicAdd(&S.counters[1 * CPAD], 1);
                if (S.kkt_list != nullptr) S.kkt_list[(size_t)S.WQ.par * m.B + pos] = b;
            }
// ... 4 lines not shown
        xfence(S.A.flags);
        __syncthreads();
        if (tid == 0) {
            if (sh[3]) {
                if (atomicAdd(S.A.n_done, 1) == S.A.B - 1) wake_all(S.A);
            } else {
                push_kkt_job(S.A, b);
            }
        }
    }
}

#define CIMPC_KKT_PRIO 2
#define CIMPC_RESID_THREADS 256
#define CIMPC_SLOT_THREADS 256
template <int NQ, int NU, bool CF>
__global__ __launch_bounds__(CIMPC_SLOT_THREADS) void resid_slot_kernel(NewtonDev S, const int* list) {
    constexpr int CT = 256, EFF_H = 128;
    extern __shared__ __attribute__((aligned(16))) double red[];
    __shared__ int eff[EFF_H];
    const int tid = threadIdx.x, nt = blockDim.x, H = S.dm.H;
    RPROF_BEGIN(0)
    int my, b;
    if (list != nullptr) {
        const int e = list[blockIdx.x];
        b = e / CS; my = e - b * CS;
    } else {
        my = (int)blockIdx.x / S.nb_launch; b = (int)blockIdx.x - my * S.nb_launch + S.b0;
    }
    const size_t sb0 = (size_t)b * CS, sb = sb0 + my;
    const bool use_eff = H <= EFF_H;
    const int ns_my = S.need_sweep[sb];
    const int stage = S.stage[b];
    const int dc = tid < CS ? S.WQ.done_count[sb0 + tid] : H;
    const int nsl = tid < CS ? S.need_sweep[sb0 + tid] : 0;
    int eff_i = -1;
    if (use_eff && tid < H) {
#pragma unroll
        for (int s_ = 0; s_ < CS; ++s_) {
            const int ok = (s_ <= my) ? S.ip_status[(sb0 + s_) * H + tid] : 0;
            if (ok != 0) eff_i = s_;
        }
    }
    if (ns_my != 1 || stage == STAGE_DONE || stage == STAGE_KKT) return;
    const int ncand = (stage == STAGE_LS1) ? 2 : (stage == STAGE_LS2) ? 4 : (stage == STAGE_LS7) ? 7 : (stage == STAGE_LS3) ? 3 : 1;
    const int it0 = (stage == STAGE_LS1) ? 1 : (stage == STAGE_LS2) ? 3 : 0;
    if (my < it0 || my >= it0 + ncand) return;
    const bool mine = tid >= it0 && tid < it0 + ncand;
    if (__syncthreads_or((tid == it0 && nsl != 1) || (mine && dc < H))) return;
    if (use_eff && tid < H) eff[tid] = eff_i;
    __syncthreads();
    RPROF(1)
    if (S.N <= SLOT_ABS_MAX) {
        double* absr = red + CT;
        slot_residual<NQ, NU, CF>(S, sb, b, use_eff ? eff : nullptr, tid, nt, absr);
        __syncthreads();
        RPROF(2)
        if (tid < CT) {
            double part = 0.0;
            for (int e = tid; e < S.N; e += CT) part += absr[e];
            red[tid] = part;
        }
    } else {
        const double part = tid < CT ? slot_residual<NQ, NU, CF>(S, sb, b, use_eff ? eff : nullptr, tid, CT) : 0.0;
        if (tid < CT) red[tid] = part;
    }
    __syncthreads();
    for (int st = CT / 2; st > 0; st >>= 1) {
        if (tid < st) red[tid] += red[tid + st];
        __syncthreads();
    }
    if (tid == 0) S.r_cand[sb] = red[0];
    RPROF(3)
}
template <int NQ, int NU, bool CF, bool SINGLE = false>
__global__ __launch_bounds__(CIMPC_RESID_THREADS) void resid_decide_kernel(NewtonDev S) {
    extern __shared__ __attribute__((aligned(16))) double red[];
    __shared__ double rc[CS];
    __shared__ int sh[4];
    resid_decide_body<NQ, NU, CF, false, SINGLE ? 0 : 2>(S, (int)blockIdx.x + S.b0, red, rc, sh);
    __syncthreads();
    if (threadIdx.x == 0) {
        __threadfence();
        const int ticket = atomicAdd(&S.counters[7 * CPAD], 1);
        if (ticket == (int)gridDim.x - 1) {
            const int n_sweep = atomicAdd(&S.counters[0 * CPAD], 0), n_kkt = atomicAdd(&S.counters[1 * CPAD], 0);
            volatile int* hm = S.host_flag;
            hm[0] = n_sweep;
            hm[1] = n_kkt;
            hm[4] = atomicAdd(&S.counters[2 * CPAD], 0);
            hm[6] = atomicAdd(&S.counters[4 * CPAD], 0);
            hm[7] = atomicAdd(&S.counters[5 * CPAD], 0);
            hm[5] = S.A.n_done != nullptr ? atomicAdd(S.A.n_done, 0) : 0;
            __threadfence_system();
            hm[2] = S.round_stamp;
            __threadfence_system();
        }
    }
}

__device__ __forceinline__ const double* kkt_dz(const NewtonDev& S, const KktArgs& K, int b, int H, int nths, int nd) {
    if (K.dz_override) return K.dz_override + (size_t)b * H * nths * nd;
    return K.stage ? S.dz_good + (size_t)b * H * nths * nd : S.dz + (size_t)b * CS * H * nths * nd;
}

__device__ __forceinline__ void lds_sync() { __syncthreads(); }

constexpr int KKT_TILES = 21;

template <int NQ, int NU>
__global__ __launch_bounds__(64) void kkt_kernel_scalar(NewtonDev S, KktArgs K) {
    constexpr int LD = ((NQ > NU ? NQ : NU) + 3) & ~3;
    const cimpc_dims& m = S.dm;
    const int b = blockIdx.x + S.b0, lane = threadIdx.x;
    if (K.stage != nullptr && K.stage[b] != STAGE_KKT) return;
    constexpr int nq = NQ, nu = NU, nd = NQ, nr = NQ + NU, nths = 2 * NQ + NU;
    const int H = m.H;
    constexpr int T2D = LD * LD;
    extern __shared__ __attribute__((aligned(16))) double sm[];
    double* A0 = sm;
    double* A1 = A0 + T2D;
    double* A2 = A1 + T2D;
    double* A1p = A2 + T2D;
    double* T0 = A1p + T2D;
    double* T1 = T0 + T2D;
    double* T2 = T1 + T2D;
    double* Y0 = T2 + T2D;
    double* Y1 = Y0 + T2D;
    double* Y2 = Y1 + T2D;
    double* Lc = Y2 + T2D;
    double* Lbuf[3] = {Lc + T2D, Lc + 2 * T2D, Lc + 3 * T2D};
    double* L1buf[2] = {Lc + 4 * T2D, Lc + 5 * T2D};
    double* L2c = Lc + 6 * T2D;
    double* Qbuf[3] = {Lc + 7 * T2D, Lc + 8 * T2D, Lc + 9 * T2D};
    double* Ri = Lc + 10 * T2D;
    double* vec = sm + KKT_TILES * T2D;
    double* bet = vec;
    double* ybuf[3] = {vec + LD, vec + 2 * LD, vec + 3 * LD};
    double* rpu = vec + 4 * LD;
    double* rpq[3] = {vec + 5 * LD, vec + 6 * LD, vec + 7 * LD};
    double* tv = vec + 8 * LD;
    const double* rb = K.r + (size_t)b * S.N;
    const double beta = K.beta ? K.beta[b] : K.beta_scalar;
    const double rho = (double)H * beta * S.kappa;
    const double* dzb = kkt_dz(S, K, b, H, nths, nd);
    constexpr int n2 = nd * nd;
    double* ws = S.kkt_ws + (size_t)b * H * (3 * n2 + nd);
    const int oq = nu;

    constexpr int PF_DZ = (nd * nths + 63) / 64, PF_Q = (nq * nq + 63) / 64, PF_R = (nu * nu + 63) / 64;
    double pf_dz[PF_DZ], pf_q[PF_Q], pf_r[PF_R], pf_rp = 0.0, pf_rd = 0.0;
    auto prefetch = [&](int i) {
        if (i >= H) return;
        const double* dzi = dzb + (size_t)i * nths * nd;
#pragma unroll
        for (int j = 0; j < PF_DZ; ++j) { const int k = lane + 64 * j; pf_dz[j] = (k < nd * nths) ? dzi[k] : 0.0; }
#pragma unroll
        for (int j = 0; j < PF_Q; ++j) { const int k = lane + 64 * j; pf_q[j] = (k < nq * nq) ? S.Qinv[(size_t)i * nq * nq + k] : 0.0; }
#pragma unroll
        for (int j = 0; j < PF_R; ++j) { const int k = lane + 64 * j; pf_r[j] = (k < nu * nu) ? S.Rinv[(size_t)i * nu * nu + k] : 0.0; }
        pf_rp = (lane < nr) ? rb[i * nr + lane] : 0.0;
        pf_rd = (lane < nd) ? rb[H * nr + i * nd + lane] : 0.0;
    };
#ifdef CIMPC_KKT_PROF
    long long pt[16] = {0}; long long tp = clock64();
#define KPROF(j) { const long long tn = clock64(); pt[j] += tn - tp; tp = tn; }
#else
#define KPROF(j)
#endif
    prefetch(0);
    for (int i = 0; i < H; ++i) {
        double* Li = Lbuf[i % 3];      double* Li1 = Lbuf[(i + 2) % 3];  double* Li2 = Lbuf[(i + 1) % 3];
        double* L1c = L1buf[i % 2];    double* L1p = L1buf[(i + 1) % 2];
        double* Qi0 = Qbuf[i % 3];     double* Qi1 = Qbuf[(i + 2) % 3];  double* Qi2 = Qbuf[(i + 1) % 3];
        double* yc = ybuf[i % 3];      double* y1 = ybuf[(i + 2) % 3];   double* y2 = ybuf[(i + 1) % 3];
// ... 1185 lines not shown
```

contactimplicitmpc/jl_amd/csrc/newton_kernels.hip:

```cpp
#include <cstdlib>
#ifdef CIMPC_KKT_PROF
#define CIMPC_KKT_WPROF
#endif
#include "newton_impl.h"

namespace cimpc {

__global__ __launch_bounds__(256) void reset_kernel(NewtonDev S, const double* q0,
                                                    const double* q1, int warm) {
    const cimpc_dims& m = S.dm;
    const int b = blockIdx.x + S.b0, tid = threadIdx.x, nt = blockDim.x;
    const int H = m.H;
    const size_t oq = (size_t)b * (H + 2) * m.nq;
    const size_t sb0 = (size_t)b * CS;
    if (!warm) {
        for (int k = tid; k < H * S.nd; k += nt) {
            S.nu[(size_t)b * H * S.nd + k] = 0.0;
        }
        copy_n(S.traj.q + oq, S.ref.q + oq, (H + 2) * m.nq, tid, nt);
        copy_n(S.traj.u + (size_t)b * H * m.nu, S.ref.u + (size_t)b * H * m.nu, H * m.nu, tid, nt);
        copy_n(S.traj.w + (size_t)b * H * m.nw, S.ref.w + (size_t)b * H * m.nw, H * m.nw, tid, nt);
        copy_n(S.traj.g + (size_t)b * H * m.nc, S.ref.g + (size_t)b * H * m.nc, H * m.nc, tid, nt);
        copy_n(S.traj.b + (size_t)b * H * m.nb, S.ref.b + (size_t)b * H * m.nb, H * m.nb, tid, nt);
        copy_n(S.traj.th + (size_t)b * H * S.nth, S.ref.th + (size_t)b * H * S.nth, H * S.nth, tid, nt);
// ... 146 lines not shown
    double* D = K.delta + (size_t)b * N;
    const double* r = K.r + (size_t)b * N;
    if (M.corr != nullptr) {
        const double* c = M.corr + (size_t)b * N;
        for (int e = tid; e < N; e += nt) D[e] += c[e];
        __syncthreads();
    }
    const double beta = K.beta ? K.beta[b] : K.beta_scalar;
    const double rho = (double)H * beta * S.kappa;
    const double* dzb = kkt_dz(S, K, b, H, S.nths, S.nd);
    double* res = M.res + (size_t)b * N;
    double mr = 0.0, mres = 0.0;
    for (int e = tid; e < N; e += nt) {
        const double v = r[e] - kkt_apply_row(S, dzb, D, rho, e);
        res[e] = v;
        mr = fmax(mr, fabs(r[e]));
        mres = (v == v) ? fmax(mres, fabs(v)) : HUGE_VAL;
    }
    red[tid] = mr; red[256 + tid] = mres;
    __syncthreads();
    for (int st = nt / 2; st > 0; st >>= 1) {
        if (tid < st) { red[tid] = fmax(red[tid], red[tid + st]); red[256 + tid] = fmax(red[256 + tid], red[256 + tid + st]); }
        __syncthreads();
    }
    const bool ok = red[256] <= M.tol * fmax(1.0, red[0]);
    __syncthreads();
    if (ok) {
        if (tid == 0) M.flag[b] = 0;
        if (K.finish) {
            __threadfence_block();
            start_line_search<BlockSync>(S, b, 1, tid, nt);
        }
    } else if (M.last && tid == 0 && M.n_fallback != nullptr) {
        atomicAdd(M.n_fallback, 1);
    }
}
size_t kkt_mixed_workspace_doubles(const NewtonDev& S) { return 2 * (size_t)S.dm.B * S.N + (size_t)S.dm.B; }
bool kkt_mixed_available(const NewtonDev& S) {
    return S.dm.mode == CIMPC_MODE_CONFIGURATION && S.V == nullptr && S.dm.nq <= 24 && S.dm.nu <= 24 && S.dm.H <= 96;
}
static int launch_kkt_mixed(const NewtonDev& S, const KktArgs& K0, double* ws, int* n_fallback, hipStream_t s) {
    const size_t BN = (size_t)S.dm.B * S.N;
    double* corr = ws; double* res = ws + BN;
    int* flag = reinterpret_cast<int*>(ws + 2 * BN);
    hipLaunchKernelGGL(kkt_mixed_init_kernel, dim3((S.nb_launch + 255) / 256), dim3(256), 0, s, S, K0, flag);
    KktArgs P = K0; P.finish = 0; P.only_flag = flag;
    int rc = launch_kkt_condensed(S, P, KktForm::PerRollout, true, nullptr, S.nb_launch, nullptr, s);
    if (rc != CIMPC_OK) return rc;
    constexpr int CORRECTIONS = 4;
    for (int k = 0; k <= CORRECTIONS; ++k) {
        MixArgs M{flag, k == 0 ? nullptr : corr, res, 1.0e-9, k == CORRECTIONS ? 1 : 0, n_fallback};
        hipLaunchKernelGGL(kkt_mixed_check_kernel, dim3(S.nb_launch), dim3(256), 0, s, S, K0, M);
        if (k == CORRECTIONS) break;
        KktArgs Pk = P; Pk.r = res; Pk.delta = corr;
        rc = launch_kkt_condensed(S, Pk, KktForm::PerRollout, true, nullptr, S.nb_launch, nullptr, s);
        if (rc != CIMPC_OK) return rc;
    }
    KktArgs F = K0; F.only_flag = flag;
    rc = launch_kkt_condensed(S, F, KktForm::PerRollout, false, nullptr, S.nb_launch, nullptr, s);
    if (rc != CIMPC_OK) return rc;
    return hipGetLastError() == hipSuccess ? CIMPC_OK : CIMPC_ERR_HIP;
}

#ifdef CIMPC_RESID_PROF
extern "C" int cimpc_debug_resid_prof(unsigned long long* out32) {
    unsigned long long z[64] = {0};
    if (hipMemcpyFromSymbol(out32, HIP_SYMBOL(cimpc::g_resid_prof), sizeof(z)) != hipSuccess) return -1;
    return hipMemcpyToSymbol(HIP_SYMBOL(cimpc::g_resid_prof), z, sizeof(z)) == hipSuccess ? 0 : -1;
}
#endif
__global__ __launch_bounds__(64) void enqueue_all_kernel(NewtonDev S) {
    const int b = blockIdx.x + S.b0;
    enqueue_eval(S, (size_t)b * CS, b, S.WQ.par, threadIdx.x, 64, b - S.b0);
    if (threadIdx.x == 0) S.cur_slot[b] = 0;
    for (int k = threadIdx.x; k < S.dm.H; k += 64) S.pflag[(size_t)b * CS * S.dm.H + k] = 0;
}
int launch_enqueue_all(const NewtonDev& S, hipStream_t s) {
    hipLaunchKernelGGL(enqueue_all_kernel, dim3(S.nb_launch), dim3(64), 0, s, S);
    return hipGetLastError() == hipSuccess ? CIMPC_OK : CIMPC_ERR_HIP;
}
__global__ __launch_bounds__(64) void async_handoff_kernel(NewtonDev S, IpQueues LQ) {
    const int i = blockIdx.x, tid = threadIdx.x;
    if (i < S.WQ.K) {
        const int n = *qcount(LQ, LQ.par, i);
        const int* src = LQ.items + ((size_t)LQ.par * LQ.K + i) * LQ.cap;
        int* dst = S.WQ.items + (size_t)i * S.WQ.cap;
        for (int k = tid; k < n; k += 64) dst[k] = src[k];
        if (tid == 0) *qcount(S.WQ, 0, i) = n;
    }
    if (i < S.dm.B && tid == 0) {
        const int b = i, stage = S.stage[b];
        if (stage == STAGE_DONE) {
            atomicAdd(S.A.n_done, 1);
        } else if (stage == STAGE_KKT) {
            push_kkt_job(S.A, b);
        } else {
            const size_t sb0 = (size_t)b * CS;
            int n = 0;
            for (int c = 0; c < CS; ++c) n += (S.need_sweep[sb0 + c] != 0 && S.WQ.done_count[sb0 + c] < S.dm.H);
            S.A.evals_left[b] = n;
        }
    }
}
int launch_async_handoff(const NewtonDev& S, const IpQueues& LQ, hipStream_t s) {
    const int grid = S.dm.B > S.WQ.K ? S.dm.B : S.WQ.K;
    hipLaunchKernelGGL(async_handoff_kernel, dim3(grid), dim3(64), 0, s, S, LQ);
    return hipGetLastError() == hipSuccess ? CIMPC_OK : CIMPC_ERR_HIP;
}
__global__ __launch_bounds__(64) void mpc_advance_kernel(NewtonDev S, int* window, const double* stride, int H_ref) {
    const cimpc_dims& m = S.dm;
    const int b = blockIdx.x, c = threadIdx.x, H = m.H, nq = m.nq, nth = S.nth;
    auto rot = [&](double* a, int rows, int n) {
        if (c >= n) return;
        const double first = a[c];
        for (int t = 0; t + 1 < rows; ++t) a[(size_t)t * n + c] = a[(size_t)(t + 1) * n + c];
        a[(size_t)(rows - 1) * n + c] = first;
    };
    double* q = S.ref.q + (size_t)b * (H + 2) * nq;
    double* th = S.ref.th + (size_t)b * H * nth;
    rot(q, H + 2, nq);
    rot(S.ref.u + (size_t)b * H * m.nu, H, m.nu);
    rot(S.ref.w + (size_t)b * H * m.nw, H, m.nw);
    rot(S.ref.g + (size_t)b * H * m.nc, H, m.nc);
    rot(S.ref.b + (size_t)b * H * m.nb, H, m.nb);
    rot(th, H, nth);
    __syncthreads();
    if (c < nq) {
        q[(size_t)H * nq + c] = q[c] + stride[c];
        q[(size_t)(H + 1) * nq + c] = q[nq + c] + stride[c];
    }
    __syncthreads();
    if (c < nq) {
        for (int tau = H - 2; tau <= H; ++tau) {
            if (tau < 1) continue;
            th[(size_t)(tau - 1) * nth + c] = q[(size_t)(tau - 1) * nq + c];
            th[(size_t)(tau - 1) * nth + nq + c] = q[(size_t)tau * nq + c];
        }
    }
    for (int i = c; i < H + 2; i += 64) {
        int* w = window + (size_t)b * (H + 2) + i;
        *w = (*w + 1) % H_ref;
    }
}
__global__ __launch_bounds__(128) void gait_window_kernel(NewtonDev S, GaitDev G, int* window, int advance) {
    const cimpc_dims& m = S.dm;
    const int b = blockIdx.x, tid = threadIdx.x, nt = blockDim.x, H = m.H, nq = m.nq, nth = S.nth, Hr = G.H_ref;
    const int k = G.phase[b] + advance;
    __syncthreads();
    if (tid == 0) G.phase[b] = k;
    double* q = S.ref.q + (size_t)b * (H + 2) * nq;
    double* th = S.ref.th + (size_t)b * H * nth;
    for (int e = tid; e < (H + 2) * nq; e += nt) {
        const int i = e / nq, c = e - i * nq, a = k + i;
        const int lap = a >= 1 ? (a - 1) / Hr : 0, j = a >= 1 ? (a - 1) - lap * Hr + 1 : 0;
        q[e] = (k == 0 && a == Hr + 1) ? G.q[(size_t)a * nq + c]
                                       : (lap ? G.q[(size_t)j * nq + c] + (double)lap * G.stride[c] : G.q[(size_t)j * nq + c]);
    }
    auto rows = [&](double* dst, const double* src, int n) {
        for (int e = tid; e < H * n; e += nt) {
            const int i = e / n, c = e - i * n;
            dst[e] = src[(size_t)((k + i) % Hr) * n + c];
        }
    };
    rows(S.ref.u + (size_t)b * H * m.nu, G.u, m.nu);
    rows(S.ref.w + (size_t)b * H * m.nw, G.w, m.nw);
    rows(S.ref.g + (size_t)b * H * m.nc, G.g, m.nc);
    rows(S.ref.b + (size_t)b * H * m.nb, G.b, m.nb);
    rows(th, G.th, nth);
    __syncthreads();
    for (int e = tid; e < H * 2 * nq; e += nt) {
// ... 29 lines not shown
    const size_t stride_b = which == 0 ? H * blk : (size_t)CS * H * blk;
    hipLaunchKernelGGL(dz_rekey_kernel, dim3(S.dm.B * S.dm.H), dim3(128), 0, s, base, stride_b, blk, knot, window, S.dm.H, S.dm.H_ref, (int)blk, dir);
    return hipGetLastError() == hipSuccess ? CIMPC_OK : CIMPC_ERR_HIP;
}
int launch_reset(const NewtonDev& S, const double* q0, const double* q1, int warm, hipStream_t s) {
    hipLaunchKernelGGL(reset_kernel, dim3(S.nb_launch), dim3(256), 0, s, S, q0, q1, warm);
    return hipGetLastError() == hipSuccess ? CIMPC_OK : CIMPC_ERR_HIP;
}
template <int NQ, int NU, bool CF>
static int launch_resid_m(const NewtonDev& S, hipStream_t s, int n_slots, int phase) {
    const size_t lds2 = (size_t)2 * CIMPC_RESID_THREADS * sizeof(double);
    if (n_slots == -1) {
        const size_t lds1 = (size_t)(CS * 256 + S.N) * sizeof(double);
        if (lds1 <= 64 * 1024) {
            if (phase == 1) return CIMPC_OK;
            hipLaunchKernelGGL((resid_decide_kernel<NQ, NU, CF, true>), dim3(S.nb_launch), dim3(CIMPC_RESID_THREADS), lds1, s, S);
            return hipGetLastError() == hipSuccess ? CIMPC_OK : CIMPC_ERR_HIP;
        }
    }
    const int* list = (n_slots >= 0 && S.slot_list != nullptr) ? S.slot_list + (size_t)S.WQ.par * S.dm.B * CS : nullptr;
    const int grid = list != nullptr ? n_slots : S.nb_launch * CS;
    const size_t lds = (size_t)(256 + (S.N <= SLOT_ABS_MAX ? S.N : 0)) * sizeof(double);
    if (grid > 0 && phase != 2) hipLaunchKernelGGL((resid_slot_kernel<NQ, NU, CF>), dim3(grid), dim3(CIMPC_SLOT_THREADS), lds, s, S, list);
    if (phase != 1) hipLaunchKernelGGL((resid_decide_kernel<NQ, NU, CF, false>), dim3(S.nb_launch), dim3(CIMPC_RESID_THREADS), lds2, s, S);
    return hipGetLastError() == hipSuccess ? CIMPC_OK : CIMPC_ERR_HIP;
}
template <int NQ, int NU>
static int launch_resid_t(const NewtonDev& S, hipStream_t s, int n_slots, int phase) {
    return S.dm.mode == CIMPC_MODE_CONFIGURATIONFORCE ? launch_resid_m<NQ, NU, true>(S, s, n_slots, phase) : launch_resid_m<NQ, NU, false>(S, s, n_slots, phase);
}
__global__ __launch_bounds__(256) void solve_finish_kernel(NewtonDev S, double* out) {
    __shared__ double red[5][256];
    const int tid = threadIdx.x, B = S.dm.B, H = S.dm.H, nu = S.dm.nu, w = nu + 2;
    double acc[5] = {0.0, 0.0, 0.0, 0.0, 0.0};
    for (int b = tid; b < B; b += 256) {
        for (int k = 0; k < 4; ++k) acc[k] += (double)S.stats[(size_t)b * 4 + k];
        acc[4] += (double)S.newton_l[b];
        double* o = out + 8 + (size_t)b * w;
        for (int k = 0; k < nu; ++k) o[k] = S.traj.u[(size_t)b * H * nu + k];
        o[nu] = (double)S.newton_l[b];
        o[nu + 1] = S.r_norm[b];
    }
    for (int k = 0; k < 5; ++k) red[k][tid] = acc[k];
    __syncthreads();
    for (int st = 128; st > 0; st >>= 1) {
        if (tid < st) for (int k = 0; k < 5; ++k) red[k][tid] += red[k][tid + st];
        __syncthreads();
    }
    if (tid < 5) out[tid] = red[tid][0];
}
__global__ __launch_bounds__(256) void dz_commit_kernel(NewtonDev S) {
    const int b = blockIdx.x, i = blockIdx.y, tid = threadIdx.x, H = S.dm.H;
    const int blk = S.nths * S.nd;
    const int s_ = S.good_src[(size_t)b * H + i];
    if (s_ < 0) return;
    double* good = S.dz_good + ((size_t)b * H + i) * blk;
    const double* slot = S.dz + (((size_t)b * CS + s_) * H + i) * blk;
    for (int e = tid; e < blk; e += 256) good[e] = slot[e];
    __syncthreads();
    if (tid == 0) S.good_src[(size_t)b * H + i] = -1;
}
int launch_dz_commit(const NewtonDev& S, hipStream_t s) {
    if (S.good_src == nullptr) return CIMPC_OK;
    hipLaunchKernelGGL(dz_commit_kernel, dim3(S.dm.B, S.dm.H), dim3(256), 0, s, S);
    return hipGetLastError() == hipSuccess ? CIMPC_OK : CIMPC_ERR_HIP;
}
bool kkt_mfma_available(const NewtonDev& S) {
    const int nq = S.dm.nq, nu = S.dm.nu;
    if (S.dm.mode != CIMPC_MODE_CONFIGURATION || nq > 24 || nu > 24) return false;
#define X(q, u) if (nq == q && nu == u) return S.dm.H <= kkt_max_h<q, u>();
    CIMPC_NQNU(X)
#undef X
    return false;
}
bool kkt_packed_available(const NewtonDev& S) {
    return S.dm.mode == CIMPC_MODE_CONFIGURATION && S.kkt_list != nullptr && S.dm.nq <= 24 && S.dm.nu <= 24 && S.dm.H <= 96 && kkt_condensed_available(S);
}
int launch_solve_finish(const NewtonDev& S, double* out, hipStream_t s) {
    hipLaunchKernelGGL(solve_finish_kernel, dim3(1), dim3(256), 0, s, S, out);
    return hipGetLastError() == hipSuccess ? CIMPC_OK : CIMPC_ERR_HIP;
}
__global__ void queue_recycle_kernel(IpQueues Q, int par) {
    const int k = (int)(blockIdx.x * blockDim.x + threadIdx.x);
    if (k < Q.K) { *qcount(Q, par, k) = 0; *qhead(Q, k) = 0; }
}
int launch_queue_recycle(const IpQueues& Q, int par, hipStream_t s) {
    hipLaunchKernelGGL(queue_recycle_kernel, dim3((Q.K + 255) / 256), dim3(256), 0, s, Q, par);
    return hipGetLastError() == hipSuccess ? CIMPC_OK : CIMPC_ERR_HIP;
}
int launch_resid_decide(const NewtonDev& S, hipStream_t s, int n_slots, int phase) {
    const int nq = S.dm.nq, nu = S.dm.nu;
#define X(q, u) if (nq == q && nu == u) return launch_resid_t<q, u>(S, s, n_slots, phase);
    CIMPC_NQNU(X)
#undef X
    return launch_resid_t<0, 0>(S, s, n_slots, phase);
}
struct CfReduce { double* dzq; double* r2; double* d2; };
__global__ __launch_bounds__(256) void cf_reduce_pre_kernel(NewtonDev S, KktArgs K, CfReduce W) {
    const int b = blockIdx.x + S.b0, tid = threadIdx.x, nt = blockDim.x;
    if (K.stage != nullptr && K.stage[b] != STAGE_KKT) return;
    const int nq = S.dm.nq, nu = S.dm.nu, ny = S.dm.nc + S.dm.nb, H = S.dm.H, nr = S.nr, nd = S.nd, nths = S.nths;
    const int nr2 = nu + nq, N2 = H * (nr2 + nq);
    const double* dz = kkt_dz(S, K, b, H, nths, nd);
    const double* r = K.r + (size_t)b * S.N;
    double* dzq = W.dzq + (size_t)b * H * nths * nq;
    double* r2 = W.r2 + (size_t)b * N2;
    for (int e = tid; e < H * nths * nq; e += nt) {
        const int ic = e / nq, rr = e - ic * nq;
        dzq[e] = dz[(size_t)ic * nd + rr];
    }
    auto dot_y = [&](int i, int c) {
        const double* col = dz + ((size_t)i * nths + c) * nd + nq;
        const double* ry = r + (size_t)i * nr + nu;
        double acc = 0.0;
        for (int k = 0; k < ny; ++k) acc = fma(col[k], ry[k], acc);
        return acc;
    };
    for (int e = tid; e < H * nr2; e += nt) {
        const int j = e / nr2, k = e - j * nr2;
        double v;
        if (k < nu) v = r[(size_t)j * nr + k] + dot_y(j, 2 * nq + k);
        else {
            const int cq = k - nu;
            v = r[(size_t)j * nr + nu + ny + cq];
            if (j + 1 < H) v += dot_y(j + 1, nq + cq);
            if (j + 2 < H) v += dot_y(j + 2, cq);
        }
        r2[e] = v;
    }
    for (int e = tid; e < H * nq; e += nt) {
        const int i = e / nq, k = e - i * nq;
        r2[(size_t)H * nr2 + e] = r[(size_t)H * nr + (size_t)i * nd + k];
    }
}

__global__ __launch_bounds__(256) void cf_reduce_post_kernel(NewtonDev S, KktArgs K, CfReduce W) {
    const int b = blockIdx.x + S.b0, tid = threadIdx.x, nt = blockDim.x;
    if (K.stage != nullptr && K.stage[b] != STAGE_KKT) return;
    const int nq = S.dm.nq, nu = S.dm.nu, nc = S.dm.nc, nbb = S.dm.nb, ny = nc + nbb, H = S.dm.H, nr = S.nr, nd = S.nd, nths = S.nths;
    const int nr2 = nu + nq, N2 = H * (nr2 + nq);
    const double* dz = kkt_dz(S, K, b, H, nths, nd);
    const double* r = K.r + (size_t)b * S.N;
    const double* d2 = W.d2 + (size_t)b * N2;
    double* D = K.delta + (size_t)b * S.N;
    const double beta = K.beta ? K.beta[b] : K.beta_scalar;
    const double rho = (double)H * beta * S.kappa;
    for (int e = tid; e < H * nr2; e += nt) {
        const int j = e / nr2, k = e - j * nr2;
        D[(size_t)j * nr + (k < nu ? k : ny + k)] = d2[e];
    }
    for (int e = tid; e < H * nq; e += nt) {
        const int i = e / nq, k = e - i * nq;
        D[(size_t)H * nr + (size_t)i * nd + k] = d2[(size_t)H * nr2 + e];
    }
    for (int e = tid; e < H * ny; e += nt) {
        const int i = e / ny, k = e - i * ny;
        double s = 0.0;
        for (int c = 0; c < nths; ++c) {
            double x;
            if (c < nq) x = i >= 2 ? d2[(size_t)(i - 2) * nr2 + nu + c] : 0.0;
            else if (c < 2 * nq) x = i >= 1 ? d2[(size_t)(i - 1) * nr2 + nu + (c - nq)] : 0.0;
            else x = d2[(size_t)i * nr2 + (c - 2 * nq)];
            s = fma(dz[((size_t)i * nths + c) * nd + nq + k], x, s);
        }
        D[(size_t)i * nr + nu + k] = s + rho * r[(size_t)i * nr + nu + k] - r[(size_t)H * nr + (size_t)i * nd + nq + k];
    }
    __syncthreads();
    for (int e = tid; e < H * ny; e += nt) {
        const int i = e / ny, k = e - i * ny;
        double g = 0.0;
// ... 77 lines not shown
```

Measured before the change: 75900.

## Shard per-knot work queues and round counters to reduce atomic contention

Splits each per-knot IP work queue into QS shards keyed by batch index, so enqueue atomics from different problems hit different counters. Consumers build a prefix map across shards and translate flat indices into shard slices. Round counters (sweep, new-eval, completion ticket) are also sharded, with a two-level ticket for the last-block election. This targets contention on hot atomics, at the cost of extra reads per dequeue, more memsets, and more complex indexing.

```diff
diff --git a/contactimplicitmpc/jl_amd/csrc/cimpc_host.cpp b/contactimplicitmpc/jl_amd/csrc/cimpc_host.cpp
--- a/contactimplicitmpc/jl_amd/csrc/cimpc_host.cpp
+++ b/contactimplicitmpc/jl_amd/csrc/cimpc_host.cpp
@@ -491,12 +491,13 @@
     A(&h->d_tab, (size_t)d.H_ref * h->ki.tab_size);
     {
         const size_t K = d.H_ref;
-        const size_t cap = B * CS * ((H + K - 1) / K + 1);
+        const size_t scap = ((B + QS - 1) / QS) * CS * ((H + K - 1) / K + 1), cap = QS * scap;
         h->Q.K = (int)K; h->Q.cap = (int)cap; h->Q.par = 0;
+        h->Q.shards = QS; h->Q.scap = (int)scap;
         A(&h->Q.items, 2 * K * cap);
-        h->ctl_ints = 3 * K * QPAD + 2 * 8 * CPAD;
+        h->ctl_ints = (2 * QS + 1) * K * QPAD + 2 * RC * CPAD;
         A(&h->Q.count, h->ctl_ints);
-        if (rc == CIMPC_OK) { h->Q.head = h->Q.count + 2 * K * QPAD; h->d_ring = h->Q.count + 3 * K * QPAD; }
+        if (rc == CIMPC_OK) { h->Q.head = h->Q.count + 2 * QS * K * QPAD; h->d_ring = h->Q.head + K * QPAD; }
         A(&h->Q.done_count, B * CS);
         A(&h->d_window, B * (H + 2));
         h->Q.window = h->d_window;
@@ -541,13 +542,13 @@
     A(&S.ls_iter, B); A(&S.newton_l, B); A(&S.stage, B); A(&S.need_sweep, BS);
     A(&S.kkt_list, 2 * B);
     A(&S.slot_list, 2 * BS);
-    A(&S.counters, 8 * CPAD);
+    A(&S.counters, RC * CPAD);
     A(&S.stats, std::max<size_t>(B * 4, 64));
     A(&S.ro_sweeps, B); A(&S.ro_ip_iters, B); A(&S.ro_ip_fail, B); A(&S.nlog, B * NLOG * 4);
     A(&S.kkt_ws, B * H * (3 * (size_t)h->nd * h->nd + h->nd));
     A(&S.kkt_tw_xch, B * (3 * (size_t)h->nd * h->nd + 4 * h->nd));
     A(&S.kkt_tw_flags, B * 32);
-    if (rc == CIMPC_OK && hipHostMalloc((void**)&h->h_counters, 8 * CPAD * sizeof(int)) != hipSuccess)
+    if (rc == CIMPC_OK && hipHostMalloc((void**)&h->h_counters, RC * CPAD * sizeof(int)) != hipSuccess)
         rc = fail(h, CIMPC_ERR_HIP, "hipHostMalloc failed");
     if (rc != CIMPC_OK) {
         g_create_error = h->err;
@@ -901,7 +902,7 @@
     HIP_TRY(h, up(T.th, theta, H * h->nth));
     if (gamma) HIP_TRY(h, up(T.g, gamma, H * d.nc));
     if (b) HIP_TRY(h, up(T.b, b, H * d.nb));
-    HIP_TRY(h, hipMemsetAsync(h->Q.count, 0, 2 * h->Q.K * QPAD * sizeof(int), h->stream));
+    HIP_TRY(h, hipMemsetAsync(h->Q.count, 0, 2 * (size_t)h->Q.K * QS * QPAD * sizeof(int), h->stream));
     HIP_TRY(h, hipMemsetAsync(h->Q.head, 0, h->Q.K * QPAD * sizeof(int), h->stream));
     {
         NewtonDev Sk = h->S;
@@ -911,10 +912,10 @@
     }
     for (int pass = 0; pass < 64; ++pass) {
         const int par = pass & 1;
-        HIP_TRY(h, hipMemsetAsync(h->S.counters, 0, 8 * CPAD * sizeof(int), h->stream));
+        HIP_TRY(h, hipMemsetAsync(h->S.counters, 0, RC * CPAD * sizeof(int), h->stream));
         rc = run_sweep(h, par, h->S.counters + 2 * CPAD, z ? h->d_zout : nullptr, h->stream);
         if (rc != CIMPC_OK) return rc;
-        HIP_TRY(h, hipMemsetAsync(h->Q.count + (size_t)par * h->Q.K * QPAD, 0, h->Q.K * QPAD * sizeof(int), h->stream));
+        HIP_TRY(h, hipMemsetAsync(h->Q.count + (size_t)par * h->Q.K * QS * QPAD, 0, (size_t)h->Q.K * QS * QPAD * sizeof(int), h->stream));
         HIP_TRY(h, hipMemsetAsync(h->Q.head, 0, h->Q.K * QPAD * sizeof(int), h->stream));
         HIP_TRY(h, hipMemcpyAsync(h->h_counters, h->S.counters + 2 * CPAD, sizeof(int), hipMemcpyDeviceToHost, h->stream));
         HIP_TRY(h, hipStreamSynchronize(h->stream));
@@ -1051,11 +1052,12 @@
         volatile int* hm = (volatile int*)h->h_ring;
         hm[3] = 0;
         NewtonDev Sk = S;
-        Sk.b0 = 0; Sk.nb_launch = h->dm.B; Sk.counters = h->d_ring; Sk.counters_next = h->d_ring + 8 * CPAD;
+        Sk.b0 = 0; Sk.nb_launch = h->dm.B; Sk.counters = h->d_ring; Sk.counters_next = h->d_ring + RC * CPAD;
         Sk.host_flag = h->h_ring_dev;
         if (!from_reset) Sk.spec_all = h->sched.spec_tail;
         Sk.WQ = h->Q; Sk.WQ.par = 0;
         Sk.WQ.items = h->a_items; Sk.WQ.cap = (int)h->a_cap;
+        Sk.WQ.shards = 1; Sk.WQ.scap = (int)h->a_cap;
         Sk.WQ.count = h->a_ctrl; Sk.WQ.head = h->a_ctrl + K * QPAD;
         AsyncQ& A = Sk.A;
         A.on = 1;
@@ -1138,21 +1140,21 @@
     const bool ahead = round_ahead(h->sched, h->kb, warm_start != 0, h->nt.max_time > 0.0 && h->nt.max_time < 1.0e6);
     auto launch_round = [&](long long r, bool blind) -> int {
         const int slot = (int)(r & 1), par = (int)(r & 1);
-        int* d_cnt = h->d_ring + 8 * CPAD * slot;
+        int* d_cnt = h->d_ring + RC * CPAD * slot;
         S.kkt_tw_epoch += 1;
         const int tw_fails = *(volatile int*)h->h_twfail;
         if (tw_fails != h->twfail_seen) { h->n_kkt_tw_fallbacks += tw_fails - h->twfail_seen; h->twfail_seen = tw_fails; }
         const bool tw_off = tw_fails != tw_fail0;
         NewtonDev Sk = S;
         Sk.b0 = 0; Sk.nb_launch = h->dm.B; Sk.counters = d_cnt;
-        Sk.counters_next = h->d_ring + 8 * CPAD * (slot ^ 1);
+        Sk.counters_next = h->d_ring + RC * CPAD * (slot ^ 1);
         Sk.host_flag = h->h_ring_dev + 8 * slot;
         Sk.A.n_done = hybrid ? h->a_ctrl + 2 * (size_t)h->Q.K * QPAD + 8 : nullptr;
         Sk.round_stamp = (int)(r + 1);
         Sk.WQ = h->Q; Sk.WQ.par = par;
         const bool kkt = (r > 0) && (blind || last_kkt > 0);
         const int n_kkt = blind ? h->dm.B : last_kkt;
-        const int* n_kkt_dev = blind ? h->d_ring + 8 * CPAD * (slot ^ 1) + 1 * CPAD : nullptr;
+        const int* n_kkt_dev = blind ? h->d_ring + RC * CPAD * (slot ^ 1) + 1 * CPAD : nullptr;
         if (kkt) {
             const bool ov = h->kp.kkt_overlap;
             const KktSite site{.kind = ov ? KktSite::Overlapped : KktSite::Round, .n_kkt = n_kkt, .blind = blind,
@@ -1169,11 +1171,11 @@
         const RoundPlan rp = plan_round(h->kn.sched, h->sched, h->ip.max_iter, kkt, blind, last_sweep, last_slots);
         const long long hint = blind ? -1 : (long long)last_slots * h->dm.H + last_parked;
         if (dbg_rounds && !blind) {
-            std::vector<int> qc((size_t)h->Q.K * QPAD);
+            std::vector<int> qc((size_t)h->Q.K * QS * QPAD);
             (void)hipStreamSynchronize(sb.st); (void)hipStreamSynchronize(sb.st_kkt);
-            if (hipMemcpy(qc.data(), h->Q.count + (size_t)par * h->Q.K * QPAD, qc.size() * sizeof(int), hipMemcpyDeviceToHost) == hipSuccess) {
+            if (hipMemcpy(qc.data(), h->Q.count + (size_t)par * h->Q.K * QS * QPAD, qc.size() * sizeof(int), hipMemcpyDeviceToHost) == hipSuccess) {
                 long long tot = 0;
-                for (int k = 0; k < h->Q.K; ++k) tot += qc[(size_t)k * QPAD];
+                for (int k = 0; k < h->Q.K * QS; ++k) tot += qc[(size_t)k * QPAD];
                 fprintf(stderr, "[cimpc round %lld] sweep launch: %lld problems queued (host hint %lld)\n", r, tot, hint);
             }
         }
diff --git a/contactimplicitmpc/jl_amd/csrc/cimpc_internal.h b/contactimplicitmpc/jl_amd/csrc/cimpc_internal.h
--- a/contactimplicitmpc/jl_amd/csrc/cimpc_internal.h
+++ b/contactimplicitmpc/jl_amd/csrc/cimpc_internal.h
@@ -8,6 +8,12 @@
 
 constexpr int QPAD = 32;
 constexpr int CPAD = 32;
+#ifndef CIMPC_QUEUE_SHARDS
+#define CIMPC_QUEUE_SHARDS 8
+#endif
+constexpr int QS = CIMPC_QUEUE_SHARDS;
+static_assert(QS >= 1 && QS <= 16, "CIMPC_QUEUE_SHARDS: 1 .. 16");
+constexpr int RC_TICKET = 8, RC_NEW = 8 + QS, RC_SWEEP = 8 + 2 * QS, RC = 8 + 3 * QS;
 
 struct IpQueues {
     int* items;
@@ -16,6 +22,7 @@
     int* done_count;
     const int* window;
     int cap, K, par;
+    int shards, scap;
 };
 
 struct AsyncQ {
@@ -101,8 +108,40 @@
 }
 __device__ __forceinline__ void wake_all(const AsyncQ& A) { for (int k = 0; k <= 32; ++k) atomicAdd(A.epoch + k * 16, 1); }
 
-__device__ __forceinline__ int* qcount(const IpQueues& Q, int par, int k) { return Q.count + ((size_t)par * Q.K + k) * QPAD; }
+__device__ __forceinline__ int qshard(const IpQueues& Q, int b) { return Q.shards > 1 ? b % Q.shards : 0; }
+__device__ __forceinline__ int* qcount(const IpQueues& Q, int par, int k, int s = 0) {
+    return Q.count + (((size_t)par * Q.K + k) * Q.shards + s) * QPAD;
+}
+__device__ __forceinline__ int* qslice(const IpQueues& Q, int par, int k, int s = 0) {
+    return Q.items + ((size_t)par * Q.K + k) * Q.cap + (size_t)s * Q.scap;
+}
 __device__ __forceinline__ int* qhead(const IpQueues& Q, int k) { return Q.head + (size_t)k * QPAD; }
+__device__ __forceinline__ int qtotal(const IpQueues& Q, int par, int k) {
+    int n = 0;
+    for (int s = 0; s < Q.shards; ++s) n += aload(qcount(Q, par, k, s));
+    return n;
+}
+__device__ __forceinline__ int* qreserve(const IpQueues& Q, int par, int k, int b, int n) {
+    const int s = qshard(Q, b);
+    const int pos = atomicAdd(qcount(Q, par, k, s), n);
+    if (pos + n > Q.scap) __builtin_trap();
+    return qslice(Q, par, k, s) + pos;
+}
+__device__ __forceinline__ int qmap_build(const IpQueues& Q, int par, int k, int* m) {
+    int cnt[QS];
+#pragma unroll
+    for (int s = 0; s < QS; ++s) cnt[s] = aload(qcount(Q, par, k, s));
+    int pre = 0;
+#pragma unroll
+    for (int s = 0; s < QS; ++s) { m[s] = pre; m[QS + s] = s * Q.scap - pre; pre += cnt[s]; }
+    return pre;
+}
+__device__ __forceinline__ int qmap_at(const int* m, int idx) {
+    int off = m[QS];
+#pragma unroll
+    for (int s = 1; s < QS; ++s) off = idx >= m[s] ? m[QS + s] : off;
+    return idx + off;
+}
 
 struct IpParams {
     const double* tab;
diff --git a/contactimplicitmpc/jl_amd/csrc/ip_generic.hip b/contactimplicitmpc/jl_amd/csrc/ip_generic.hip
--- a/contactimplicitmpc/jl_amd/csrc/ip_generic.hip
+++ b/contactimplicitmpc/jl_amd/csrc/ip_generic.hip
@@ -201,13 +201,14 @@
     S.l = l; S.vx = l < nx; S.vy = l < ny;
     const LinLayout& L = S.L;
     const cimpc_ip_opts o = p.o;
-    const int K = p.Q.K, par = p.Q.par, cap = p.Q.cap;
+    const int K = p.Q.K, par = p.Q.par;
     const int PS = 2 * nx + 4 * ny + 4;
     for (int kk = 0; kk < K; ++kk) {
         const int knot = ((int)blockIdx.x + kk) % K;
-        const int n = *qcount(p.Q, par, knot);
+        int qmap[2 * QS];
+        const int n = qmap_build(p.Q, par, knot, qmap);
         if (n == 0) continue;
-        const int* items = p.Q.items + ((size_t)par * K + knot) * cap;
+        const int* items = qslice(p.Q, par, knot);
         S.tab = p.tab + (size_t)knot * L.size;
         const double* tVec = S.tab + L.oVec;
         S.ry2 = tVec[LinLayout::V_RY2 * GW + l]; S.ry1d = tVec[LinLayout::V_RY1D * GW + l]; S.caibd = tVec[LinLayout::V_CAIBD * GW + l];
@@ -217,7 +218,7 @@
         const int G0 = (int)gridDim.x;
         int idx = p.generic_static ? (int)blockIdx.x : __builtin_amdgcn_readfirstlane(atomicAdd(head, l == 0 ? 1 : 0));
         for (; idx < n; idx = p.generic_static ? idx + G0 : __builtin_amdgcn_readfirstlane(atomicAdd(head, l == 0 ? 1 : 0))) {
-            const int prob = items[idx];
+            const int prob = items[qmap_at(qmap, idx)];
             const int sb = prob / p.H, i = prob - sb * p.H;
             const size_t pi = (size_t)prob;
             wfence();
diff --git a/contactimplicitmpc/jl_amd/csrc/ip_kernel_impl.h b/contactimplicitmpc/jl_amd/csrc/ip_kernel_impl.h
--- a/contactimplicitmpc/jl_amd/csrc/ip_kernel_impl.h
+++ b/contactimplicitmpc/jl_amd/csrc/ip_kernel_impl.h
@@ -769,7 +769,7 @@
     {
         int part = 0;
         for (int k = tid; k < K; k += (int)blockDim.x) {
-            int rem = aload(qcount(p.Q, par, k)) - aload(qhead(p.Q, k));
+            int rem = qtotal(p.Q, par, k) - aload(qhead(p.Q, k));
             rem = rem > 0 ? rem : 0;
             if (k < PICK_MAXK) s_rem[k] = rem;
             part += rem;
@@ -784,7 +784,7 @@
             const long long target = ((long long)wg * total) / (long long)nwg;
             long long acc = 0;
             for (int k = 0; k < K; ++k) {
-                const int rem = k < PICK_MAXK ? s_rem[k] : max(0, aload(qcount(p.Q, par, k)) - aload(qhead(p.Q, k)));
+                const int rem = k < PICK_MAXK ? s_rem[k] : max(0, qtotal(p.Q, par, k) - aload(qhead(p.Q, k)));
                 if (rem > 0) { pick = k; acc += rem; if (acc > target) break; }
             }
         }
@@ -795,13 +795,14 @@
 }
 
 template <class M, bool ASYNC>
-__device__ __forceinline__ void serve_knot(const IpParams& p, double* smem, int knot, int tid, [[maybe_unused]] long long* sp = nullptr) {
+__device__ __forceinline__ void serve_knot(const IpParams& p, double* smem, int knot, int tid, [[maybe_unused]] int* qmap,
+                                           [[maybe_unused]] long long* sp = nullptr) {
     constexpr int NX = M::NX, NY = M::NY, NTH = M::NTH, ND = M::ND, G = M::G;
     constexpr int NC = M::NC, NB = M::NB;
     constexpr LinLayout L(NX, NY, NTH, G, M::NTHS, M::ADJ);
     constexpr int PS = 2 * NX + 4 * NY + 4;
     double* tab = smem;
-    const int K = p.Q.K, cap = p.Q.cap, par = p.Q.par;
+    const int par = p.Q.par;
     const int grp = tid / G;
     const int l = tid % G;
     double* Rst = smem + L.hot + (size_t)grp * M::LDS_GROUP;
@@ -817,13 +818,15 @@
     const bool timed = p.budget_ticks > 0;
 
     [[maybe_unused]] const long long sp_t0 = SPROF_T();
-    const int n = ASYNC ? 1 : *qcount(p.Q, par, knot);
+    if constexpr (!ASYNC) { if (tid == 0) qmap[2 * QS] = qmap_build(p.Q, par, knot, qmap); }
     stage_table<M>(tab, p.tab, knot, tid);
     __syncthreads();
+    int n = 1;
+    if constexpr (!ASYNC) n = qmap[2 * QS];
 #ifdef CIMPC_SWEEP_PROF
     if (sp) sp[2] += SPROF_T() - sp_t0;
 #endif
-    const int* items = p.Q.items + ((size_t)par * K + knot) * cap;
+    const int* items = qslice(p.Q, par, knot);
     int* head = qhead(p.Q, knot);
     [[maybe_unused]] const int* tailp = qcount(p.Q, par, knot);
     IpSolver<M> S;
@@ -868,8 +871,7 @@
                     if (l == 0) {
                         ps[PS - 4] = r_vio; ps[PS - 3] = k_vio; ps[PS - 2] = reg; ps[PS - 1] = (double)((long long)iters + (timed ? t_used * 128 : 0));
                         p.pflag[pi] = 1;
-                        const int pos = atomicAdd(qcount(p.Q, par ^ 1, knot), 1);
-                        p.Q.items[((size_t)(par ^ 1) * K + knot) * cap + pos] = prob;
+                        *qreserve(p.Q, par ^ 1, knot, sb / p.slots, 1) = prob;
                         atomicAdd(p.pending_count, 1);
                     }
                 } else {
@@ -923,7 +925,8 @@
                 idx = group_bcast0<G>(idx);
             }
             if (idx < n) {
-                prob = ASYNC ? item : items[idx];
+                if constexpr (ASYNC) prob = item;
+                else prob = items[qmap_at(qmap, idx)];
                 const int sb = prob / p.H, i = prob - sb * p.H;
                 const size_t pi = (size_t)prob;
                 const double* th = p.theta + pi * NTH;
@@ -1068,13 +1071,14 @@
 __global__ __launch_bounds__(M::G == 16 ? CIMPC_SWEEP_THREADS : (M::WIDE ? 512 : 256), M::G == 16 ? CIMPC_SWEEP_OCC : 1) void ip_queue_kernel(IpParams p) {
     extern __shared__ __attribute__((aligned(16))) double smem[];
     __shared__ int s_knot, s_total, s_rem[PICK_MAXK];
+    static_assert(PICK_MAXK >= 2 * QS + 1, "queue map in s_rem");
     const int tid = (int)threadIdx.x;
     __builtin_amdgcn_s_setprio(CIMPC_SWEEP_PRIO);
     [[maybe_unused]] long long sp[12] = {0, 0, 0, 0, 0, 0, 0, 0, 0, 0, 0, 0};
     [[maybe_unused]] const long long sp_life = SPROF_T();
     if (p.direct) {
         const int knot = (int)blockIdx.x;
-        if (knot < p.Q.K && aload(qcount(p.Q, p.Q.par, knot)) > 0) serve_knot<M, false>(p, smem, knot, tid, sp);
+        if (knot < p.Q.K && qtotal(p.Q, p.Q.par, knot) > 0) serve_knot<M, false>(p, smem, knot, tid, s_rem, sp);
         return;
     }
     while (true) {
@@ -1088,7 +1092,7 @@
             if (tid == 0 && p.drain_count != nullptr) atomicAdd(p.drain_count, 1);
             break;
         }
-        serve_knot<M, false>(p, smem, knot, tid, sp);
+        serve_knot<M, false>(p, smem, knot, tid, s_rem, sp);
     }
 #ifdef CIMPC_SWEEP_PROF
     if ((tid & 63) == 0) {
diff --git a/contactimplicitmpc/jl_amd/csrc/newton_async_impl.h b/contactimplicitmpc/jl_amd/csrc/newton_async_impl.h
--- a/contactimplicitmpc/jl_amd/csrc/newton_async_impl.h
+++ b/contactimplicitmpc/jl_amd/csrc/newton_async_impl.h
@@ -84,7 +84,7 @@
 template <class M>
 __device__ __noinline__ void async_serve_job(unsigned long long ka, double* smem, int knot, int tid) {
     const IpParams p = uniform_arg<IpParams, offsetof(AsyncArgs, p)>(ka);
-    serve_knot<M, true>(p, smem, knot, tid);
+    serve_knot<M, true>(p, smem, knot, tid, nullptr);
 }
 
 template <class M>
diff --git a/contactimplicitmpc/jl_amd/csrc/newton_impl.h b/contactimplicitmpc/jl_amd/csrc/newton_impl.h
--- a/contactimplicitmpc/jl_amd/csrc/newton_impl.h
+++ b/contactimplicitmpc/jl_amd/csrc/newton_impl.h
@@ -30,6 +30,14 @@
 
 __device__ __forceinline__ double ls_alpha(int iter) { return ldexp(1.0, -iter); }
 
+__device__ __forceinline__ void rc_add(const NewtonDev& S, int base, int b, int n) { atomicAdd(&S.counters[(base + b % QS) * CPAD], n); }
+__device__ __forceinline__ int rc_sum(const NewtonDev& S, int base) {
+    int n = 0;
+#pragma unroll
+    for (int s = 0; s < QS; ++s) n += aload(&S.counters[(base + s) * CPAD]);
+    return n;
+}
+
 __device__ __forceinline__ void list_slot(const NewtonDev& S, size_t sb, int par, int pos = -1) {
     if (S.slot_list == nullptr) return;
     if (pos < 0) pos = atomicAdd(&S.counters[4 * CPAD], 1);
@@ -38,11 +46,10 @@
 }
 
 __device__ __forceinline__ void enqueue_eval(const NewtonDev& S, size_t sb, int b, int par, int tid, int nt, int list_pos = -1) {
-    const int H = S.dm.H, K = S.WQ.K;
+    const int H = S.dm.H;
     for (int k = tid; k < H; k += nt) {
         const int t = S.WQ.window[(size_t)b * (H + 2) + k];
-        const int pos = atomicAdd(qcount(S.WQ, par, t), 1);
-        S.WQ.items[((size_t)par * K + t) * S.WQ.cap + pos] = (int)(sb * H + k);
+        *qreserve(S.WQ, par, t, b, 1) = (int)(sb * H + k);
     }
     if (tid == 0) {
         S.WQ.done_count[sb] = 0;
@@ -52,17 +59,16 @@
 }
 
 __device__ __forceinline__ void enqueue_evals(const NewtonDev& S, size_t sb, int n, int b, int par, int tid, int nt, int mark = 1) {
-    const int H = S.dm.H, K = S.WQ.K;
+    const int H = S.dm.H;
     for (int k = tid; k < H; k += nt) {
         const int t = S.WQ.window[(size_t)b * (H + 2) + k];
-        const int pos = atomicAdd(qcount(S.WQ, par, t), n);
-        int* it = S.WQ.items + ((size_t)par * K + t) * S.WQ.cap + pos;
+        int* it = qreserve(S.WQ, par, t, b, n);
         for (int c = 0; c < n; ++c) it[c] = (int)((sb + c) * H + k);
     }
     if (tid == 0) {
         int pos = 0;
         if (S.slot_list != nullptr) pos = atomicAdd(&S.counters[4 * CPAD], n);
-        atomicAdd(&S.counters[5 * CPAD], n);
+        rc_add(S, RC_NEW, b, n);
         if (pos + n > S.dm.B * CS) __builtin_trap();
         for (int c = 0; c < n; ++c) {
             S.WQ.done_count[sb + c] = 0;
@@ -247,7 +253,7 @@
         enqueue_evals(S, sb0, n, b, par, lane, nt, S.kkt_same_round == 0 ? 2 : 1);
         if (lane == 0) {
             for (int c = n; c < CS; ++c) S.need_sweep[sb0 + c] = 0;
-            if (S.kkt_same_round == 0) atomicAdd(&S.counters[0 * CPAD], 1);
+            if (S.kkt_same_round == 0) rc_add(S, RC_SWEEP, b, 1);
         }
     }
 }
@@ -446,8 +452,9 @@
     const size_t sb0 = (size_t)b * CS;
     if (!ASYNC && blockIdx.x == 0) {
         const int K = S.WQ.K, par = S.WQ.par;
-        for (int k = tid; k < K; k += nt) { *qcount(S.WQ, par, k) = 0; *qhead(S.WQ, k) = 0; }
-        if (tid < 8) S.counters_next[tid * CPAD] = 0;
+        for (int k = tid; k < K * S.WQ.shards; k += nt) *qcount(S.WQ, par, 0, k) = 0;
+        for (int k = tid; k < K; k += nt) *qhead(S.WQ, k) = 0;
+        if (tid < RC) S.counters_next[tid * CPAD] = 0;
     }
     RPROF_BEGIN(1)
     int pre_dc = H, pre_ns = 0;
@@ -467,7 +474,7 @@
             return;
         }
         if (__syncthreads_or(mine && pre_dc < H)) {
-            if (tid == 0) atomicAdd(&S.counters[0 * CPAD], 1);
+            if (tid == 0) rc_add(S, RC_SWEEP, b, 1);
             if (mine) list_slot(S, sb0 + tid, S.WQ.par ^ 1);
             return;
         }
@@ -485,7 +492,7 @@
             int pend = 0;
             if (tid < ncand) pend = (S.WQ.done_count[sb0 + it0 + tid] < H);
             if (__syncthreads_or(pend)) {
-                if (tid == 0) atomicAdd(&S.counters[0 * CPAD], 1);
+                if (tid == 0) rc_add(S, RC_SWEEP, b, 1);
                 return;
             }
         }
@@ -595,7 +602,7 @@
         RPROF(5)
         if (tid == 0) {
             S.stage[b] = nstage;
-            atomicAdd(&S.counters[0 * CPAD], 1);
+            rc_add(S, RC_SWEEP, b, 1);
         }
         return;
     }
@@ -766,15 +773,19 @@
     __syncthreads();
     if (threadIdx.x == 0) {
         __threadfence();
+        const int sh_ = (int)blockIdx.x % QS, n_sh = ((int)gridDim.x - sh_ + QS - 1) / QS, n_shards = (int)gridDim.x < QS ? (int)gridDim.x : QS;
+        if (atomicAdd(&S.counters[(RC_TICKET + sh_) * CPAD], 1) != n_sh - 1) return;
+        __threadfence();
         const int ticket = atomicAdd(&S.counters[7 * CPAD], 1);
-        if (ticket == (int)gridDim.x - 1) {
-            const int n_sweep = atomicAdd(&S.counters[0 * CPAD], 0), n_kkt = atomicAdd(&S.counters[1 * CPAD], 0);
+        if (ticket == n_shards - 1) {
+            __threadfence();
+            const int n_sweep = rc_sum(S, RC_SWEEP), n_kkt = atomicAdd(&S.counters[1 * CPAD], 0);
             volatile int* hm = S.host_flag;
             hm[0] = n_sweep;
             hm[1] = n_kkt;
             hm[4] = atomicAdd(&S.counters[2 * CPAD], 0);
             hm[6] = atomicAdd(&S.counters[4 * CPAD], 0);
-            hm[7] = atomicAdd(&S.counters[5 * CPAD], 0);
+            hm[7] = rc_sum(S, RC_NEW);
             hm[5] = S.A.n_done != nullptr ? atomicAdd(S.A.n_done, 0) : 0;
             __threadfence_system();
             hm[2] = S.round_stamp;
diff --git a/contactimplicitmpc/jl_amd/csrc/newton_kernels.hip b/contactimplicitmpc/jl_amd/csrc/newton_kernels.hip
--- a/contactimplicitmpc/jl_amd/csrc/newton_kernels.hip
+++ b/contactimplicitmpc/jl_amd/csrc/newton_kernels.hip
@@ -252,10 +252,14 @@
 __global__ __launch_bounds__(64) void async_handoff_kernel(NewtonDev S, IpQueues LQ) {
     const int i = blockIdx.x, tid = threadIdx.x;
     if (i < S.WQ.K) {
-        const int n = *qcount(LQ, LQ.par, i);
-        const int* src = LQ.items + ((size_t)LQ.par * LQ.K + i) * LQ.cap;
         int* dst = S.WQ.items + (size_t)i * S.WQ.cap;
-        for (int k = tid; k < n; k += 64) dst[k] = src[k];
+        int n = 0;
+        for (int s = 0; s < LQ.shards; ++s) {
+            const int ns = *qcount(LQ, LQ.par, i, s);
+            const int* src = qslice(LQ, LQ.par, i, s);
+            for (int k = tid; k < ns; k += 64) dst[n + k] = src[k];
+            n += ns;
+        }
         if (tid == 0) *qcount(S.WQ, 0, i) = n;
     }
     if (i < S.dm.B && tid == 0) {
@@ -451,10 +455,11 @@
 }
 __global__ void queue_recycle_kernel(IpQueues Q, int par) {
     const int k = (int)(blockIdx.x * blockDim.x + threadIdx.x);
-    if (k < Q.K) { *qcount(Q, par, k) = 0; *qhead(Q, k) = 0; }
+    if (k < Q.K * Q.shards) *qcount(Q, par, 0, k) = 0;
+    if (k < Q.K) *qhead(Q, k) = 0;
 }
 int launch_queue_recycle(const IpQueues& Q, int par, hipStream_t s) {
-    hipLaunchKernelGGL(queue_recycle_kernel, dim3((Q.K + 255) / 256), dim3(256), 0, s, Q, par);
+    hipLaunchKernelGGL(queue_recycle_kernel, dim3((Q.K * Q.shards + 255) / 256), dim3(256), 0, s, Q, par);
     return hipGetLastError() == hipSuccess ? CIMPC_OK : CIMPC_ERR_HIP;
 }
 int launch_resid_decide(const NewtonDev& S, hipStream_t s, int n_slots, int phase) {
```

After: 74000. 2.5% lower.
